# LCAV/LenslessPiCam

Measured on AMD Instinct MI355X. Metric: ADMM iterations/sec at 4056x3040x3, 100 iters, higher is better.
Workload: dtype f32; 1 GPU; C2: one 3040x4056x3 frame per GPU, ADMM-TV 100 iterations per step; n_iter=100, frames_per_gpu=1, parallelism=frames sharded over 1 GPU(s), one all-gather per step

## Files before the change

lenslesspicam_amd/csrc/lpc_abi.cpp:

```cpp
#include "lpc_engine.h"

static thread_local std::string g_last_error;
int fail(const std::string& msg) {
  g_last_error = msg;
  return 1;
}

static std::string parse_all_opts(const char* handle_opts, EngineOpts& o) {
  std::string err = parse_engine_opts(std::getenv("LPC_OPTIONS"), o);
  return err.empty() ? parse_engine_opts(handle_opts, o) : err;
}

extern "C" {

const char* lpc_last_error(void) { return g_last_error.c_str(); }
const char* lpc_backend(void) { return rt::backend_name(); }
const char* lpc_real_name(void) { return LPC_REAL_NAME; }

int lpc_create(const lpc_config* cfg, lpc_handle* out) {
  if (!cfg || !out) return fail("lpc_create: null argument");
  *out = nullptr;
  if (cfg->height < 1 || cfg->width < 1) return fail("lpc_create: bad spatial size");
  if (cfg->channels != 1 && cfg->channels != 3) return fail("PSF must either be rgb (3) or grayscale (1)");
  if (cfg->depth < 1 || cfg->batch < 1) return fail("lpc_create: depth and batch must be >= 1");
  if (cfg->algo < LPC_ALGO_CONV || cfg->algo > LPC_ALGO_FISTA) return fail("lpc_create: unknown algo");
  if (cfg->norm < 0 || cfg->norm > 2) return fail("lpc_create: unknown norm");
  int ndev = 0;
  if (rt::device_count(&ndev) != lpcSuccess || ndev < 1)
    return fail("no HIP device: the engine has no CPU path");
  Engine* e = new Engine();
  e->cfg = *cfg;
  e->cfg.options = nullptr;
  {
    std::string err = parse_all_opts(cfg->options, e->opt);
    if (!err.empty()) { delete e; return fail("lpc_create: " + err); }
  }
  e->gd.tk = cfg->fista_tk; e->gd.nest_mu = cfg->nesterov_mu; e->gd.nest_p = cfg->nesterov_p;
  int rc = setup_geometry(e);
  if (!rc) rc = alloc_common(e);
  if (!rc && cfg->algo == LPC_ALGO_ADMM) rc = admm_alloc(e);
  if (!rc && cfg->algo >= LPC_ALGO_GD) rc = gd_alloc(e);
  if (rc) {
    lpc_destroy(e);
    return rc;
  }
  *out = e;
  return 0;
}

int lpc_plan_module(const lpc_config* cfg, int build, char* key_buf, size_t n) {
  if (!cfg) return fail("lpc_plan_module: null config");
  if (cfg->height < 1 || cfg->width < 1 || cfg->depth < 1 || cfg->batch < 1) return fail("lpc_plan_module: bad size");
  EngineOpts opt;
  std::string err = parse_all_opts(cfg->options, opt);
  if (!err.empty()) return fail("lpc_plan_module: " + err);
  ShapePlan sp;
  LPC_OK(setup_shape(*cfg, opt, plan_cu_count(), &sp));
  const bool any = sp.want_static && sp.plan.spec.any();
  if (key_buf && n) std::snprintf(key_buf, n, "%s", any ? plan_spec_key(sp.plan.spec).c_str() : "");
  if (!any || !build) return 0;
  std::string path;
  if (build_plan_module(sp.plan.spec, opt, &path) != 0) return fail(path);
  return 0;
}

int lpc_destroy(lpc_handle e) {
  if (!e) return 0;
  (void)rt::stream_sync(e->stream);
  for (auto& a : e->allocs) (void)rt::dev_free(a.first);
  release_plan_module(e->mod);
  e->mod = nullptr;
#if !defined(LPC_SIMT_EMU)
  for (auto& v : e->timer.ev)
    for (auto& pr : v) { (void)hipEventDestroy(pr.first); (void)hipEventDestroy(pr.second); }
#endif
  delete e;
  return 0;
}

int lpc_padded_shape(lpc_handle e, int* Hp, int* Wp, int* sh, int* sw) {
  if (!e) return fail("null handle");
  if (Hp) *Hp = e->g.Hp;
  if (Wp) *Wp = e->g.Wp;
  if (sh) *sh = e->g.sh;
  if (sw) *sw = e->g.sw;
  return 0;
}

int lpc_workspace_bytes(lpc_handle e, size_t* bytes) {
  if (!e || !bytes) return fail("null argument");
  *bytes = e->total_bytes;
  return 0;
}

int lpc_set_psf(lpc_handle e, const real* dev_psf, void* stream) {
  if (!e || !dev_psf) return fail("lpc_set_psf: null argument");
  e->stream = (lpcStream_t)stream;
  LPC_OK(set_psf(e, dev_psf));
  if (e->cfg.algo == LPC_ALGO_ADMM) LPC_OK(admm_setup_constants(e));
  if (e->cfg.algo >= LPC_ALGO_GD) LPC_OK(gd_setup_constants(e));
  if (e->cfg.algo != LPC_ALGO_CONV) return lpc_reset(e, stream);
  return 0;
}

static int per_frame_refusal(const Engine* e, const char* who) {
  if (!e->psf_per_frame) return 0;
  return fail(std::string(who) + ": not available with per-frame PSFs (lpc_set_psf_batch): their gradients are not implemented");
}
static int per_frame_gd_check(const Engine* e, const char* who) {
  if (e->cfg.algo < LPC_ALGO_GD || (e->gd.gx0_pinned && e->fista.sched_n > 0)) return 0;
  return fail(std::string(who) + ": per-frame PSFs need a pinned start value (lpc_set_start_value) and a schedule "
              "(lpc_set_fista_schedule) on a gradient-descent handle: plain iterations take their step and start value from one PSF");
}

int lpc_set_psf_batch(lpc_handle e, const real* dev_psfs, void* stream) {
  if (!e || !dev_psfs) return fail("lpc_set_psf_batch: null argument");
  LPC_OK(per_frame_gd_check(e, "lpc_set_psf_batch"));
  if (e->fista_tape.rec_on || e->admm_tape.rec_on)
    return fail("lpc_set_psf_batch: the handle records a tape, and gradients with per-frame PSFs are not implemented");
  e->stream = (lpcStream_t)stream;
  const bool gram = e->cfg.algo == LPC_ALGO_ADMM && !e->psf_set;
  LPC_OK(set_psf_batch(e, dev_psfs));
  e->admm.midc_valid = false;
  e->fista_tape.invalidate();
  e->admm_tape.invalidate();
  if (gram) LPC_OK(admm_setup_constants(e));
  if (e->cfg.algo != LPC_ALGO_CONV) return lpc_reset(e, stream);
  return 0;
}

int lpc_convolve(lpc_handle e, const real* dev_x, real* dev_out, int n, int x_channels, int adjoint, void* stream) {
  if (!e || !dev_x || !dev_out) return fail("lpc_convolve: null argument");
  LPC_OK(check_channels(e, x_channels, "lpc_convolve"));
  if (!e->psf_set) return fail("lpc_convolve: PSF not set");
  if (n < 1 || n > e->cfg.batch) return fail("lpc_convolve: n exceeds the configured batch");
  if (e->cfg.algo != LPC_ALGO_CONV) return fail("lpc_convolve: handle was not created with LPC_ALGO_CONV");
  e->stream = (lpcStream_t)stream;
  return convolve_hwc(e, dev_x, dev_out, n, x_channels, adjoint != 0, false);
}

int lpc_convolve_spectrum(lpc_handle e, const real* dev_x, real* dev_out, int n, int x_channels, int adjoint,
                          void* stream) {
  if (!e || !dev_x || !dev_out) return fail("lpc_convolve_spectrum: null argument");
  LPC_OK(check_channels(e, x_channels, "lpc_convolve_spectrum"));
  if (!e->psf_set) return fail("lpc_convolve_spectrum: PSF not set");
  if (n < 1 || n > e->cfg.batch) return fail("lpc_convolve_spectrum: n exceeds the configured batch");
  if (e->cfg.algo != LPC_ALGO_CONV) return fail("lpc_convolve_spectrum: handle was not created with LPC_ALGO_CONV");
  e->stream = (lpcStream_t)stream;
  return convolve_hwc(e, dev_x, dev_out, n, x_channels, adjoint != 0, true);
}

int lpc_set_data(lpc_handle e, const real* dev_data, int data_channels, void* stream) {
  if (!e || !dev_data) return fail("lpc_set_data: null argument");
  if (e->cfg.algo == LPC_ALGO_CONV) return fail("lpc_set_data: operator-only handle");
  LPC_OK(check_channels(e, data_channels, "lpc_set_data"));
  e->stream = (lpcStream_t)stream;
  const PlaneGeom& g = e->g;
  LPC_OK(hwc_to_planar(e, dev_data, e->Y, e->cfg.batch, g.H, g.W, g.W, g.uplane, data_channels));
  e->data_set = true;
  e->data_channels = data_channels;
  e->fista_tape.invalidate();
  e->admm_tape.invalidate();
  return 0;
}

int lpc_set_initial_estimate(lpc_handle e, const real* dev_est, void* stream) {
  if (!e) return fail("null handle");
  if (e->cfg.algo == LPC_ALGO_CONV) return fail("lpc_set_initial_estimate: operator-only handle");
  e->stream = (lpcStream_t)stream;
  const PlaneGeom& g = e->g;
  if (!dev_est) { e->has_init = false; return 0; }
  const bool admm = e->cfg.algo == LPC_ALGO_ADMM;
  const size_t n = (size_t)(admm ? g.rplane : g.uplane) * e->P;
  if (!e->init_est) LPC_OK(dev_alloc(e, &e->init_est, n));
  const int nimg = e->cfg.batch * e->cfg.depth;
  if (admm) LPC_OK(hwc_to_planar(e, dev_est, e->init_est, nimg, g.Hp, g.Wp, g.rpitch, g.rplane));
  else LPC_OK(hwc_to_planar(e, dev_est, e->init_est, nimg, g.H, g.W, g.W, g.uplane));
  e->has_init = true;
  return 0;
}

int lpc_reset(lpc_handle e, void* stream) {
  if (!e) return fail("null handle");
  if (!e->psf_set) return fail("lpc_reset: PSF not set");
  e->stream = (lpcStream_t)stream;
  if (e->cfg.algo == LPC_ALGO_ADMM) return admm_reset(e);
  if (e->cfg.algo >= LPC_ALGO_GD) return gd_reset(e);
  return 0;
}

int lpc_set_momentum(lpc_handle e, double p, double mu, double tk) {
  if (!e) return fail("null handle");
  e->gd.nest_p = p; e->gd.nest_mu = mu;
  if (tk > 0) e->gd.tk = tk;
  return gd_apply_momentum_reset(e);
}

int lpc_set_start_value(lpc_handle e, const real* dev_start, void* stream) {
  if (!e) return fail("null handle");
  if (e->cfg.algo < LPC_ALGO_GD) return fail("lpc_set_start_value: gradient-descent family only");
  e->stream = (lpcStream_t)stream;
  e->gd.gx0_pinned = dev_start != nullptr;
  if (dev_start) LPC_RT(rt::copy_d2d_async(e->gd.gx0, dev_start, e->cfg.channels * sizeof(real), e->stream));
  return 0;
}

int lpc_set_admm_schedule(lpc_handle e, int n, const double* mu1, const double* mu2, const double* mu3,
                          const double* tau) {
  if (!e) return fail("null handle");
  if (e->cfg.algo != LPC_ALGO_ADMM) return fail("lpc_set_admm_schedule: not an ADMM handle");
  for (auto& v : e->admm.sched) v.clear();
  e->admm_tape.invalidate();
  if (n <= 0) return 0;
  if (!mu1 || !mu2 || !mu3 || !tau) return fail("lpc_set_admm_schedule: null array");
  for (int i = 0; i < n; ++i) {
    if (!(mu1[i] > 0) || !(mu2[i] > 0) || !(mu3[i] > 0)) return fail("lpc_set_admm_schedule: step sizes must be > 0");
    e->admm.sched[0].push_back(mu1[i]); e->admm.sched[1].push_back(mu2[i]);
    e->admm.sched[2].push_back(mu3[i]); e->admm.sched[3].push_back(tau[i]);
  }
  return 0;
}

int lpc_set_fista_schedule(lpc_handle e, int n, const real* alpha, const real* coef, void* stream) {
  if (!e) return fail("null handle");
  if (e->cfg.algo != LPC_ALGO_FISTA) return fail("lpc_set_fista_schedule: not a FISTA handle");
  e->stream = (lpcStream_t)stream;
  return gd_set_schedule(e, n, alpha, coef);
}

int lpc_fista_record(lpc_handle e, int on) {
  if (!e) return fail("null handle");
  if (e->cfg.algo != LPC_ALGO_FISTA) return fail("lpc_fista_record: not a FISTA handle");
  if (on) LPC_OK(per_frame_refusal(e, "lpc_fista_record"));
  return tape_record(e, e->fista_tape, on, gd_tape_alloc);
}

static int tape_refusal(const Engine* e, const Tape& t, long n, const std::string& who, bool counted) {
  if (!counted && (!t.rec_on || !t.buf || t.iters < 0))
    return fail("lpc_" + who + "_backward: nothing recorded (lpc_" + who + "_record(h, 1), then lpc_reset and lpc_iterate)");
  if (counted && !t.complete(n, e->iters_done))
    return fail("lpc_" + who + "_backward: " + std::to_string(e->iters_done) + " iterations since the reset, the schedule has " +
                std::to_string(n));
  return 0;
}

static int fista_backward(lpc_handle e, const real* dev_grad_out, real* dev_grad_data, real* dev_grad_alpha,
                          real* dev_grad_coef, real* dev_grad_init, real* dev_grad_psf, void* stream) {
  if (!e || !dev_grad_out || !dev_grad_alpha || !dev_grad_coef) return fail("lpc_fista_backward: null argument");
  if (e->cfg.algo != LPC_ALGO_FISTA) return fail("lpc_fista_backward: not a FISTA handle");
  LPC_OK(per_frame_refusal(e, "lpc_fista_backward"));
  if (e->fista.sched_n <= 0) return fail("lpc_fista_backward: the handle has no schedule (lpc_set_fista_schedule)");
  LPC_OK(tape_refusal(e, e->fista_tape, e->fista.sched_n, "fista", false));
  if (e->gd.split_pending) return fail("lpc_fista_backward: a split iteration is in flight (lpc_iterate_end missing)");
  LPC_OK(tape_refusal(e, e->fista_tape, e->fista.sched_n, "fista", true));
  if ((e->g.Hp | e->g.Wp) & 1)
    return fail("lpc_fista_backward: padded frame " + std::to_string(e->g.Hp) + " x " + std::to_string(e->g.Wp) +
                " has an odd length: convolve and deconvolve are not each other's adjoints there (not implemented)");
  if (e->cfg.depth > 1) return fail("lpc_fista_backward: depth > 1 is not implemented");
  for (real a : e->fista.alpha)
    if (a == (real)0.) return fail("lpc_fista_backward: a step alpha of the schedule is 0");
  if (dev_grad_data && !e->data_set) return fail("lpc_fista_backward: no data set");
  e->stream = (lpcStream_t)stream;
  return gd_backward(e, dev_grad_out, dev_grad_data, dev_grad_alpha, dev_grad_coef, dev_grad_init, dev_grad_psf);
}
int lpc_fista_backward(lpc_handle e, const real* dev_grad_out, real* dev_grad_data, real* dev_grad_alpha,
                       real* dev_grad_coef, real* dev_grad_init, void* stream) {
  return fista_backward(e, dev_grad_out, dev_grad_data, dev_grad_alpha, dev_grad_coef, dev_grad_init, nullptr, stream);
}
int lpc_fista_backward_psf(lpc_handle e, const real* dev_grad_out, real* dev_grad_data, real* dev_grad_alpha,
                           real* dev_grad_coef, real* dev_grad_init, real* dev_grad_psf, void* stream) {
  return fista_backward(e, dev_grad_out, dev_grad_data, dev_grad_alpha, dev_grad_coef, dev_grad_init, dev_grad_psf, stream);
}

int lpc_admm_record(lpc_handle e, int on) {
  if (!e) return fail("null handle");
  if (e->cfg.algo != LPC_ALGO_ADMM) return fail("lpc_admm_record: not an ADMM handle");
  if (on) LPC_OK(per_frame_refusal(e, "lpc_admm_record"));
  return tape_record(e, e->admm_tape, on, admm_tape_alloc);
}

static int admm_backward_checked(lpc_handle e, const real* dev_grad_out, real* dev_grad_data, real* dev_grad_mu1,
                                 real* dev_grad_mu2, real* dev_grad_mu3, real* dev_grad_tau, real* dev_grad_psf, void* stream) {
  if (!e || !dev_grad_out || !dev_grad_mu1 || !dev_grad_mu2 || !dev_grad_mu3 || !dev_grad_tau)
    return fail("lpc_admm_backward: null argument");
  if (e->cfg.algo != LPC_ALGO_ADMM) return fail("lpc_admm_backward: not an ADMM handle");
  LPC_OK(per_frame_refusal(e, "lpc_admm_backward"));
  const long n = (long)e->admm.sched[0].size();
  if (n <= 0) return fail("lpc_admm_backward: the handle has no schedule (lpc_set_admm_schedule)");
  if (e->cfg.depth > 1) return fail("lpc_admm_backward: depth > 1 is not implemented");
  if ((e->g.Hp | e->g.Wp) & 1)
    return fail("lpc_admm_backward: padded frame " + std::to_string(e->g.Hp) + " x " + std::to_string(e->g.Wp) +
                " has an odd length: the spectral step and the convolve / deconvolve pair are not self-adjoint there "
                "(not implemented)");
  if (e->admm.custom_gram || e->admm.pnp_mode)
    return fail("lpc_admm_backward: a caller's psi and plug-and-play iterations are not differentiated");
  if (e->has_init) return fail("lpc_admm_backward: an initial estimate is set (its gradient is not implemented)");
  LPC_OK(tape_refusal(e, e->admm_tape, n, "admm", false));
  LPC_OK(tape_refusal(e, e->admm_tape, n, "admm", true));
  if (dev_grad_data && !e->data_set) return fail("lpc_admm_backward: no data set");
  if (dev_grad_psf && e->cfg.norm != LPC_NORM_BACKWARD)
    return fail("lpc_admm_backward_psf: the gradient with respect to the PSF is implemented for norm \"backward\" only");
  e->stream = (lpcStream_t)stream;
  return admm_backward(e, dev_grad_out, dev_grad_data, dev_grad_mu1, dev_grad_mu2, dev_grad_mu3, dev_grad_tau, dev_grad_psf);
}
int lpc_admm_backward(lpc_handle e, const real* dev_grad_out, real* dev_grad_data, real* dev_grad_mu1, real* dev_grad_mu2,
                      real* dev_grad_mu3, real* dev_grad_tau, void* stream) {
  return admm_backward_checked(e, dev_grad_out, dev_grad_data, dev_grad_mu1, dev_grad_mu2, dev_grad_mu3, dev_grad_tau, nullptr,
                               stream);
}
int lpc_admm_backward_psf(lpc_handle e, const real* dev_grad_out, real* dev_grad_data, real* dev_grad_mu1, real* dev_grad_mu2,
                          real* dev_grad_mu3, real* dev_grad_tau, real* dev_grad_psf, void* stream) {
  return admm_backward_checked(e, dev_grad_out, dev_grad_data, dev_grad_mu1, dev_grad_mu2, dev_grad_mu3, dev_grad_tau,
                               dev_grad_psf, stream);
}

int lpc_iterate(lpc_handle e, int n_iter, void* stream) {
  if (!e) return fail("null handle");
  if (n_iter < 0) return fail("lpc_iterate: negative iteration count");
  if (!e->psf_set) return fail("lpc_iterate: PSF not set");
  if (!e->data_set) return fail("Must set data with `set_data()`");
  e->stream = (lpcStream_t)stream;
  if (e->gd.split_pending) return fail("lpc_iterate: a split iteration is in flight (lpc_iterate_end missing)");
  if (e->admm.pnp_mode) return fail("lpc_iterate: the handle runs plug-and-play iterations since the last reset");
  if (e->psf_per_frame) LPC_OK(per_frame_gd_check(e, "lpc_iterate"));
  if (e->cfg.algo == LPC_ALGO_ADMM) return admm_iterate(e, n_iter);
  if (e->cfg.algo >= LPC_ALGO_GD) return gd_iterate(e, n_iter);
  return fail("lpc_iterate: operator-only handle");
}

int lpc_iterate_begin(lpc_handle e, void* stream) {
  if (!e) return fail("null handle");
  if (e->cfg.algo < LPC_ALGO_GD) return fail("lpc_iterate_begin: gradient-descent family only");
  if (!e->psf_set) return fail("lpc_iterate_begin: PSF not set");
  if (!e->data_set) return fail("Must set data with `set_data()`");
  if (e->gd.split_pending) return fail("lpc_iterate_begin: the previous split iteration was not finished");
  if (e->psf_per_frame) LPC_OK(per_frame_gd_check(e, "lpc_iterate_begin"));
  if (e->fista_tape.rec_on)
    return fail("lpc_iterate_begin: not available while the handle records a tape (lpc_fista_record)");
  e->stream = (lpcStream_t)stream;
  return gd_iterate(e, 1, 1);
}

int lpc_iterate_end(lpc_handle e, const real* dev_projected, void* stream) {
  if (!e || !dev_projected) return fail("lpc_iterate_end: null argument");
  if (e->cfg.algo < LPC_ALGO_GD) return fail("lpc_iterate_end: gradient-descent family only");
  if (!e->gd.split_pending) return fail("lpc_iterate_end: no split iteration in flight");
  e->stream = (lpcStream_t)stream;
  return gd_finish_split(e, dev_projected);
}

static int pnp_check(lpc_handle e, const char* who) {
  if (!e) return fail("null handle");
  if (e->cfg.algo != LPC_ALGO_ADMM) return fail(std::string(who) + ": ADMM handles only");
  if (!e->psf_set) return fail(std::string(who) + ": PSF not set");
  if (!e->data_set) return fail("Must set data with `set_data()`");
  if (!e->admm.sched[0].empty()) return fail(std::string(who) + ": not available with an unrolled schedule");
  return 0;
}

int lpc_admm_pnp_begin(lpc_handle e, int use_dual, real* dev_denoiser_in, void* stream) {
  LPC_OK(pnp_check(e, "lpc_admm_pnp_begin"));
  if (!dev_denoiser_in) return fail("lpc_admm_pnp_begin: null argument");
  if (e->admm.pnp_pending) return fail("lpc_admm_pnp_begin: the previous split iteration was not finished");
  if (!e->admm.pnp_mode && e->iters_done != 0)
    return fail("lpc_admm_pnp_begin: fused iterations already ran since the last reset");
  e->stream = (lpcStream_t)stream;
  return admm_pnp_begin(e, use_dual, dev_denoiser_in);
}

int lpc_admm_pnp_end(lpc_handle e, int use_dual, const real* dev_U, void* stream) {
  LPC_OK(pnp_check(e, "lpc_admm_pnp_end"));
  if (!dev_U) return fail("lpc_admm_pnp_end: null argument");
  if (!e->admm.pnp_pending) return fail("lpc_admm_pnp_end: no split iteration in flight");
  e->stream = (lpcStream_t)stream;
  return admm_pnp_end(e, use_dual, dev_U);
}

int lpc_set_psi_gram(lpc_handle e, const real* dev_gabs, void* stream) {
  if (!e || !dev_gabs) return fail("lpc_set_psi_gram: null argument");
  if (e->cfg.algo != LPC_ALGO_ADMM) return fail("lpc_set_psi_gram: ADMM handles only");
  e->stream = (lpcStream_t)stream;
  return admm_set_psi_gram(e, dev_gabs);
}

int lpc_admm_psi_step(lpc_handle e, const real* dev_psit, void* stream) {
  LPC_OK(pnp_check(e, "lpc_admm_psi_step"));
  if (!dev_psit) return fail("lpc_admm_psi_step: null argument");
  if (e->admm.pnp_pending) return fail("lpc_admm_psi_step: a plug-and-play iteration is in flight");
  if (!e->admm.pnp_mode && e->iters_done != 0)
    return fail("lpc_admm_psi_step: fused iterations already ran since the last reset");
  e->stream = (lpcStream_t)stream;
  return admm_psi_step(e, dev_psit);
}

int lpc_form_image(lpc_handle e, real* dev_out, void* stream) {
  if (!e || !dev_out) return fail("lpc_form_image: null argument");
  e->stream = (lpcStream_t)stream;
  if (e->cfg.algo == LPC_ALGO_ADMM) return admm_form_image(e, dev_out);
  if (e->cfg.algo >= LPC_ALGO_GD) return gd_form_image(e, dev_out);
  return fail("lpc_form_image: operator-only handle");
}

int lpc_get_state(lpc_handle e, const char* name, real* dev_out, void* stream) {
  if (!e || !name || !dev_out) return fail("lpc_get_state: null argument");
  e->stream = (lpcStream_t)stream;
  if (e->cfg.algo >= LPC_ALGO_GD) return gd_get_state(e, name, dev_out);
  if (e->cfg.algo == LPC_ALGO_ADMM) return admm_get_state(e, name, dev_out);
  return fail("lpc_get_state: operator-only handle");
}

int lpc_profile_enable(lpc_handle e, int on) {
  if (!e) return fail("null handle");
#if !defined(LPC_SIMT_EMU)
  for (int k = 0; k < LPC_K_COUNT; ++k) e->timer.used[k] = 0;
#endif
  e->timer.on = on != 0;
  e->timer.mask = on > 1 ? (unsigned)on >> 1 : ~0u;
  return 0;
}

int lpc_profile_read(lpc_handle e, double* avg_ms, long* launches) {
  if (!e || !avg_ms || !launches) return fail("null argument");
  for (int k = 0; k < LPC_K_COUNT; ++k) { avg_ms[k] = 0.0; launches[k] = 0; }
#if !defined(LPC_SIMT_EMU)
  LPC_RT(hipStreamSynchronize(e->stream));
  for (int k = 0; k < LPC_K_COUNT; ++k) {
    double tot = 0.0;
    for (size_t i = 0; i < e->timer.used[k]; ++i) {
      float ms = 0.f;
      LPC_RT(hipEventElapsedTime(&ms, e->timer.ev[k][i].first, e->timer.ev[k][i].second));
      tot += ms;
    }
    launches[k] = (long)e->timer.used[k];
    avg_ms[k] = e->timer.used[k] ? tot / (double)e->timer.used[k] : 0.0;
  }
#endif
  return 0;
}

int lpc_kernel_bytes(lpc_handle e, int kid, double* bytes) {
  if (!e || !bytes) return fail("null argument");
  if (e->cfg.algo == LPC_ALGO_ADMM) return admm_kernel_bytes(e, kid, bytes);
  if (e->cfg.algo >= LPC_ALGO_GD) return gd_kernel_bytes(e, kid, bytes);
  return fail("lpc_kernel_bytes: operator-only handle");
}

int lpc_plan_info(lpc_handle e, char* buf, size_t n) {
  if (!e || !buf || n == 0) return fail("null argument");
  const PlaneGeom& g = e->g;
  const LaunchPlan& pl = e->plan;
  const PlanSpec& sp = pl.spec;
  std::string s = "padded " + std::to_string(g.Hp) + "x" + std::to_string(g.Wp);
  s += pl.rows_half ? "; rows: half-length " + std::to_string(g.Wp / 2) : "; rows: paired " + std::to_string(g.Wp);
  const bool rows_static = e->mod && sp.row_kind && (pl.rows_half || e->cfg.algo == LPC_ALGO_ADMM);
  if (rows_static) s += " [static " + rad_list(sp.row, ".") + ", " + std::to_string(sp.row.nt) + " threads]";
  if (pl.gd_v2) s += " (fused rows: second form, " + std::to_string(sp.row.n / sp.row.rad[0]) + " lanes)";
  if (pl.admm_rows_v2)
    s += std::string(" (ADMM rows: second form, ") + (pl.admm_rows_v2 == 3 ? "forward + inverse, " : pl.admm_rows_v2 == 2 ? "inverse, " : "forward, ") +
         std::to_string(sp.row.n / sp.row.rad[0]) + " lanes)";
  s += "; columns: " + (pl.N1 > 1 ? std::to_string(pl.N1) + " x " + std::to_string(pl.N2) + " split" : std::string("single pass ") + std::to_string(pl.N2));
  s += ", T = " + std::to_string(pl.T);
  if (e->mod && sp.passA.n) s += ", pass A [static " + rad_list(sp.passA, ".") + ", T = " + std::to_string(sp.passA.T) + "]";
  if (e->cfg.algo == LPC_ALGO_ADMM) {
    s += pl.admm_mid == ADMM_MID_REG24 ? ", middle in registers"
         : pl.admm_mid == ADMM_MID_MODULE ? ", LDS middle [static " + rad_list(sp.mid, ".") + (sp.mid_kind == LPC_MID_SEQ ? ", one spectrum at a time" : "") + (g.slay ? ", pair-line spectra]" : "]")
                                          : ", LDS middle";
    s += pl.k1 == ADMM_K1_ROWS ? "; TV / W half and X half inside the forward rows (three launches per iteration)"
         : pl.k1 == ADMM_K1_TV_W ? "; tiled TV / W kernel + X half inside the forward rows" : "; stand-alone image-domain kernel";
    if (pl.xi_window) s += pl.hv_skip ? " (xi inside the sensor window only, H V row transforms skipped outside it)"
                                      : " (xi inside the sensor window only)";
    if (pl.rho_rsp || pl.xi_half)
      s += std::string("; inside a call: ") + (pl.rho_rsp ? "rho read back from r_sp" : "") +
           (pl.rho_rsp && pl.xi_half ? ", " : "") + (pl.xi_half ? "xi half-applied" : "");
  }
  if (e->cfg.algo == LPC_ALGO_ADMM && e->admm.g_sep) s += "; gram as row + column terms";
  if (e->cfg.algo == LPC_ALGO_FISTA)
    s += e->mod && e->mod->gd_bwd_head ? "; reverse rows: plan module" : pl.rows_half ? "; reverse rows: half-length, run-time plan"
                                                                                     : "; reverse rows: paired, run-time plan";
  s += e->mod ? "; plan module " + plan_spec_key(sp) : "; run-time plans (" + e->mod_note + ")";
  std::snprintf(buf, n, "%s", s.c_str());
  return 0;
}

int lpc_model_bytes(lpc_handle e, double* bytes) {
  if (!e || !bytes) return fail("null argument");
  if (e->cfg.algo == LPC_ALGO_ADMM) *bytes = admm_model_bytes(e);
  else if (e->cfg.algo >= LPC_ALGO_GD) *bytes = gd_model_bytes(e);
  else return fail("lpc_model_bytes: operator-only handle");
  return 0;
}

}
```

lenslesspicam_amd/csrc/lpc_admm.cpp:

```cpp
#include "lpc_engine.h"
#include "lpc_admm_kernels.h"
#include "lpc_layout_kernels.h"
#include "lpc_reduce_kernels.h"

static void admm_params(const Engine* e, long it, double out[4]) {
  const lpc_config& c = e->cfg;
  const double dflt[4] = {c.mu1, c.mu2, c.mu3, c.tau};
  for (int k = 0; k < 4; ++k) {
    const std::vector<double>& v = e->admm.sched[k];
    out[k] = v.empty() ? dflt[k] : v[(size_t)std::min<long>(it, (long)v.size() - 1)];
  }
}

static AdmmScalars admm_scalars(const Engine* e, const double cur[4]) {
  AdmmScalars p;
  p.mu1 = (real)cur[0]; p.mu2 = (real)cur[1]; p.mu3 = (real)cur[2];
  p.thr = (real)(cur[3] / cur[1]);
  p.m_in = (real)1.0 / ((real)1.0 + p.mu1);
  p.m_out = (real)1.0 / ((real)0.0 + p.mu1);
  p.first = e->first ? 1 : 0;
  const double* prev = e->first ? cur : e->admm.last_par;
  p.mu1p = (real)prev[0]; p.mu2p = (real)prev[1]; p.mu3p = (real)prev[2];
  p.thrp = (real)(prev[3] / prev[1]);
  p.m_in_p = (real)1.0 / ((real)1.0 + p.mu1p);
  p.m_out_p = (real)1.0 / ((real)0.0 + p.mu1p);
  p.r_mu2 = (real)(1.0 / (double)p.mu2); p.r_mu3 = (real)(1.0 / (double)p.mu3);
  p.r_mu2p = (real)(1.0 / (double)p.mu2p); p.r_mu3p = (real)(1.0 / (double)p.mu3p);
  p.clamp_cur = e->admm.vw_cur ? 1 : 0;
  p.clamp_old = e->admm.vw_old ? 1 : 0;
  p.xiw = e->plan.xi_window ? 1 : 0;
  p.xi_store = 1;
  p.skipa = p.skiphv = 0;
  p.rev = e->plan.rev_k1 ? 1 : 0;
  p.half_in = p.half_out = 0;
  p.rho_rsp = p.xi_in = p.xi_out = 0;
  return p;
}

int admm_alloc_psf(Engine* e, int nplanes) {
  const PlaneGeom& g = e->g;
  dev_free(e, e->admm.Hs_t); dev_free(e, e->admm.midc); dev_free(e, e->admm.midrd);
  e->admm.Hs_t = nullptr; e->admm.midc = nullptr; e->admm.midrd = nullptr;
  e->admm.midc_valid = false;
  if (!g.slay) return 0;
  LPC_OK(dev_alloc(e, &e->admm.Hs_t, (size_t)g.cplane * nplanes));
  if (e->mod && e->mod->mid_pc) {
    real2* c = nullptr;
    LPC_OK(dev_alloc(e, &c, (size_t)g.cplane * nplanes * (e->mod->mid_pc == 1 ? 2 : 1)));
    e->admm.midc = c;
    LPC_OK(dev_alloc(e, &e->admm.midrd, (size_t)g.cplane * nplanes));
  }
  return 0;
}

static const int kGsepBlocks = 512;
int admm_alloc(Engine* e) {
  const PlaneGeom& g = e->g;
  const size_t rp = (size_t)g.rplane * e->P;
  real* zeroed = nullptr;
  LPC_OK(dev_alloc(e, &zeroed, 8 * rp));
  real** zb[] = {&e->admm.V[0], &e->admm.V[1], &e->admm.HVb[0], &e->admm.HVb[1], &e->admm.xi, &e->admm.eta0[0], &e->admm.eta1[0], &e->admm.rho};
  for (int k = 0; k < 8; ++k) *zb[k] = zeroed + (size_t)k * rp;
  real** bufs[] = {&e->admm.eta0[1], &e->admm.eta1[1], &e->admm.Rsp, &e->admm.Aarr};
  for (real** b : bufs) LPC_OK(dev_alloc(e, b, rp));
  LPC_OK(dev_alloc(e, &e->admm.Gabs, (size_t)g.cplane));
  if (g.slay) LPC_OK(dev_alloc(e, &e->admm.Gabs_t, (size_t)g.cplane));
  LPC_OK(admm_alloc_psf(e, e->Ppsf));
  LPC_OK(dev_alloc(e, &e->admm.Ga, (size_t)g.Hp));
  LPC_OK(dev_alloc(e, &e->admm.Gb, (size_t)g.cpitch));
  LPC_OK(dev_alloc(e, &e->admm.Gpart, (size_t)2 * kGsepBlocks));
  return 0;
}

static int admm_split_gram(Engine* e) {
  const PlaneGeom& g = e->g;
  e->admm.g_sep = 0;
  e->admm.midc_valid = false;
  if (g.slay)
    LPC_OK(launch_k(e, -1, k_to_pair_lines<256, real>, grid1d((long)g.Hp * g.cpitch, 256), 256, 0, (const real*)e->admm.Gabs,
                    e->admm.Gabs_t, g.Hp, g.cpitch, g.cplane));
  if (!e->plan.g_terms) return 0;
  const int n = (int)std::max<long>(g.Hp, g.cpitch);
  LPC_OK(launch_k(e, -1, k_gsep_extract, grid1d((long)n, 256), 256, 0, (const real*)e->admm.Gabs, g.Hp, g.Wc,
                  (long)g.cpitch, e->admm.Ga, e->admm.Gb));
  LPC_OK(launch_k(e, -1, k_gsep_check<256>, dim3(kGsepBlocks), 256, 2 * 256 * sizeof(real), (const real*)e->admm.Gabs, g.Hp,
                  g.Wc, (long)g.cpitch, (const real*)e->admm.Ga, (const real*)e->admm.Gb, e->admm.Gpart));
  std::vector<real> part((size_t)2 * kGsepBlocks);
  LPC_RT(rt::copy_d2h_async(part.data(), e->admm.Gpart, part.size() * sizeof(real), e->stream));
  LPC_RT(rt::stream_sync(e->stream));
  double err = 0., top = 0.;
  for (int b = 0; b < kGsepBlocks; ++b) { err = std::max(err, (double)part[2 * b]); top = std::max(top, -(double)part[2 * b + 1]); }
  const double eps = sizeof(real) == 4 ? 1e-6 : 1e-13;
  e->admm.g_sep = (top > 0. && err <= eps * top) ? 1 : 0;
  return 0;
}

int admm_setup_constants(Engine* e) {
  const PlaneGeom& g = e->g;
  real* stencil = e->admm.Rsp;
  LPC_RT(rt::memset_async(stencil, 0, (size_t)g.rplane * sizeof(real), e->stream));
  std::vector<real> host((size_t)g.rplane, (real)0.);
  host[0] = (real)4.;
  host[(size_t)(1 % g.Wp)] = -(real)1.;
  host[(size_t)(g.Wp - 1)] = -(real)1.;
  host[(size_t)(1 % g.Hp) * g.rpitch] = -(real)1.;
  host[(size_t)(g.Hp - 1) * g.rpitch] = -(real)1.;
  LPC_OK(upload(e, stencil, host.data(), host.size() * sizeof(real)));
  real2* Gs = e->S;
  LPC_OK(fft2_forward_setup(e, src_padded(e, stencil), Gs, 1));
  LPC_OK(launch_k(e, -1, k_abs_complex<256>, grid1d((long)g.cplane, 256), 256, 0, (const real2*)Gs, e->admm.Gabs,
                  (long)g.cplane));
  e->admm.custom_gram = false;
  return admm_split_gram(e);
}

int admm_reset(Engine* e) {
  const PlaneGeom& g = e->g;
  const size_t rb = (size_t)g.rplane * e->P * sizeof(real);
  if (e->has_init) LPC_RT(rt::memset_async(e->admm.V[1], 0, 7 * rb, e->stream));
  else LPC_RT(rt::memset_async(e->admm.V[0], 0, 8 * rb, e->stream));
  e->admm.vcur = 0;
  e->admm.ecur = 0;
  e->admm.hcur = 0;
  e->admm.vw_cur = e->admm.vw_old = false;
  if (e->has_init) {
    LPC_RT(rt::copy_d2d_async(e->admm.V[0], e->init_est, rb, e->stream));
    LPC_OK(convolve_planar(e, e->admm.V[0], e->admm.HVb[0], e->P, true, false));
  }
  e->first = true;
  e->admm.pnp_mode = e->admm.pnp_pending = false;
  e->iters_done = 0;
  return admm_tape_reset(e);
}

static int admm_spectral_step(Engine* e, const AdmmScalars& sc, real* Vout, real* HVout, bool xhalf = false,
                              const K1Rows* k1 = nullptr) {
  if (xhalf) LPC_OK(e->mod->admm_rows_fwd_x(e, &sc, k1));
  else LPC_OK(admm_rows_fwd(e));
  LPC_OK(admm_cols(e, sc));
  return admm_rows_inv(e, Vout, HVout, sc.skiphv != 0);
}
int admm_spectral_plain(Engine* e, const double par[4], real* Vout, real* HVout) {
  return admm_spectral_step(e, admm_scalars(e, par), Vout, HVout);
}


typedef void (*K1Kernel)(PlaneGeom, AdmmScalars, const real*, const real*, const real*, const real*, real*, const real*,
                         const real*, real*, real*, real*, const real*, real*, real*, unsigned);
struct K1Launch { K1Kernel fn; int th, tw; size_t smem; };
static K1Launch k1_launch(AdmmK1 form, bool half_in) {
  constexpr int NT = 256, TW4 = 256;
  auto smem4 = [](int th) { return (size_t)2 * (th + 2) * (TW4 + 8) * sizeof(real); };
  switch (form) {
    case ADMM_K1_TV_W:
      return half_in ? K1Launch{k_admm_spatial_v4<4, NT, false, true>, 4, TW4, smem4(4) / 2}
                     : K1Launch{k_admm_spatial_v4<4, NT, false>, 4, TW4, smem4(4)};
    case ADMM_K1_TILED: return {k_admm_spatial_v4<8, NT>, 8, TW4, smem4(8)};
    default: return {k_admm_spatial<16, 64, NT>, 16, 64, (size_t)(2 * 18 * 66 + 17 * 64 + 16 * 65) * sizeof(real)};
  }
}

int admm_iterate(Engine* e, int n_iter) {
  const PlaneGeom& g = e->g;
  const LaunchPlan& pl = e->plan;
  bool sb_rows_valid = false;
  for (int it = 0; it < n_iter; ++it) {
    real* Vc = e->admm.V[e->admm.vcur];
    real* Vo = e->admm.V[e->admm.vcur ^ 1];
    double par[4];
    admm_params(e, e->iters_done, par);
    AdmmScalars sc = admm_scalars(e, par);
    sc.xi_store = (it + 1 == n_iter || !sc.xiw) ? 1 : 0;
    sc.skipa = (pl.hv_skip && sb_rows_valid && !sc.xi_store) ? 1 : 0;
    sc.skiphv = (pl.hv_skip && it + 3 < n_iter) ? 1 : 0;
    sc.half_in = (pl.k1_half && it > 0) ? 1 : 0;
    sc.half_out = (pl.k1_half && it + 1 < n_iter) ? 1 : 0;
    sc.rho_rsp = (pl.rho_rsp && sc.half_in) ? 1 : 0;
    sc.xi_in = (pl.xi_half && it > 0) ? 1 : 0;
    sc.xi_out = (pl.xi_half && it + 1 < n_iter) ? 1 : 0;
    AdmmState& a = e->admm;
    const K1Rows k1 = {Vc, Vo, a.eta0[a.ecur], a.eta1[a.ecur], a.eta0[a.ecur ^ 1], a.eta1[a.ecur ^ 1], a.rho, pl.k1_xcd_order};
    if (pl.k1 != ADMM_K1_ROWS) {
      const K1Launch k = k1_launch(pl.k1, sc.half_in != 0);
      const unsigned tiles_x = (g.Wp + k.tw - 1) / k.tw, tiles_y = (g.Hp + k.th - 1) / k.th;
      LPC_OK(launch_k(e, LPC_K_SPATIAL, k.fn, dim3(tiles_x * tiles_y, e->P, 1), 256, k.smem, g, sc, (const real*)Vc,
                      (const real*)Vo, (const real*)a.HVb[a.hcur], (const real*)a.HVb[a.hcur ^ 1], a.xi,
                      (const real*)a.eta0[a.ecur], (const real*)a.eta1[a.ecur], a.eta0[a.ecur ^ 1], a.eta1[a.ecur ^ 1],
                      a.rho, (const real*)e->Y, a.Rsp, a.Aarr, tiles_x));
    }
    e->admm.vw_old = e->admm.vw_cur;
    e->admm.vw_cur = false;
    e->admm.ecur ^= 1;
    e->first = false;
    LPC_OK(admm_spectral_step(e, sc, Vo, e->admm.HVb[e->admm.hcur ^ 1], pl.xhalf_rows, pl.k1 == ADMM_K1_ROWS ? &k1 : nullptr));
    e->admm.vcur ^= 1;
    e->admm.hcur ^= 1;
    sb_rows_valid = true;
    for (int k = 0; k < 4; ++k) e->admm.last_par[k] = par[k];
    LPC_OK(admm_tape_push(e, Vo));
    ++e->iters_done;
  }
  return 0;
}

int admm_pnp_begin(Engine* e, int use_dual, real* dev_denoiser_in) {
  e->admm.pnp_mode = true;
  const PlaneGeom& g = e->g;
  const int nimg = e->cfg.batch * e->cfg.depth;
  real* src = e->admm.V[e->admm.vcur];
  if (use_dual) {
    const long n = (long)g.rplane * e->P;
    LPC_OK(launch_k(e, -1, k_pnp_input<256>, grid1d(n, 256), 256, 0, e->admm.Rsp, (const real*)e->admm.eta1[0],
                    (const real*)e->admm.eta0[0], (real)e->cfg.mu2, n));
    src = e->admm.Rsp;
  }
  LPC_OK(planar_to_hwc(e, src, dev_denoiser_in, nimg, g.Hp, g.Wp, g.rpitch, g.rplane, 0, 0, 0));
  e->admm.pnp_pending = true;
  return 0;
}

int admm_pnp_end(Engine* e, int use_dual, const real* dev_U) {
  const PlaneGeom& g = e->g;
  const int nimg = e->cfg.batch * e->cfg.depth;
  real *eta = e->admm.eta0[0], *U = e->admm.eta1[0], *X = e->admm.eta0[1], *W = e->admm.eta1[1];
  LPC_OK(hwc_to_planar(e, dev_U, U, nimg, g.Hp, g.Wp, g.rpitch, g.rplane));
  double par[4];
  admm_params(e, e->iters_done, par);
  const AdmmScalars sc = admm_scalars(e, par);
  const dim3 grid = grid1d((long)g.Hp * g.Wp, 256, e->P);
  real* Vc = e->admm.V[e->admm.vcur];
  real* Vn = e->admm.V[e->admm.vcur ^ 1];
  real* HVn = e->admm.HVb[e->admm.hcur ^ 1];
  LPC_OK(launch_k(e, LPC_K_SPATIAL, k_pnp_pre<256>, grid, 256, 0, g, sc, use_dual ? 1 : 0, (const real*)Vc,
                  (const real*)e->admm.HVb[e->admm.hcur], (const real*)e->admm.xi, (const real*)e->admm.rho, (const real*)U,
                  (const real*)eta, (const real*)e->Y, X, W, e->admm.Rsp, e->admm.Aarr));
  LPC_OK(admm_spectral_step(e, sc, Vn, HVn));
  LPC_OK(launch_k(e, LPC_K_SPATIAL, k_pnp_post<256>, grid, 256, 0, g, sc, use_dual ? 1 : 0, (const real*)Vn,
                  (const real*)HVn, (const real*)X, (const real*)W, (const real*)U, e->admm.xi, eta, e->admm.rho));
  e->admm.vcur ^= 1;
  e->admm.hcur ^= 1;
  e->admm.pnp_pending = false;
  e->first = false;
  ++e->iters_done;
  return 0;
}

int admm_set_psi_gram(Engine* e, const real* dev_gabs) {
  const PlaneGeom& g = e->g;
  LPC_RT(rt::memset_async(e->admm.Gabs, 0, (size_t)g.cplane * sizeof(real), e->stream));
  LPC_OK(launch_k(e, -1, k_permute_spectrum_rows<256>, grid1d((long)g.Hp * g.Wc, 256), 256, 0, dev_gabs, e->admm.Gabs, g.Hp,
                  g.Wc, g.cpitch, e->plan.N1, e->plan.N2));
  e->admm.custom_gram = true;
  return admm_split_gram(e);
}

int admm_psi_step(Engine* e, const real* dev_psit) {
  e->admm.pnp_mode = true;
  const PlaneGeom& g = e->g;
  const int nimg = e->cfg.batch * e->cfg.depth;
  real *T = e->admm.eta1[0], *X = e->admm.eta0[1], *W = e->admm.eta1[1];
  LPC_OK(hwc_to_planar(e, dev_psit, T, nimg, g.Hp, g.Wp, g.rpitch, g.rplane));
  double par[4];
  admm_params(e, e->iters_done, par);
  const AdmmScalars sc = admm_scalars(e, par);
  const dim3 grid = grid1d((long)g.Hp * g.Wp, 256, e->P);
  real* Vc = e->admm.V[e->admm.vcur];
  real* Vn = e->admm.V[e->admm.vcur ^ 1];
  real* HVn = e->admm.HVb[e->admm.hcur ^ 1];
  LPC_OK(launch_k(e, LPC_K_SPATIAL, k_pnp_pre<256>, grid, 256, 0, g, sc, 2, (const real*)Vc,
                  (const real*)e->admm.HVb[e->admm.hcur], (const real*)e->admm.xi, (const real*)e->admm.rho, (const real*)T,
                  (const real*)e->admm.eta0[0], (const real*)e->Y, X, W, e->admm.Rsp, e->admm.Aarr));
  LPC_OK(admm_spectral_step(e, sc, Vn, HVn));
  LPC_OK(launch_k(e, LPC_K_SPATIAL, k_pnp_post<256>, grid, 256, 0, g, sc, 0, (const real*)Vn, (const real*)HVn,
                  (const real*)X, (const real*)W, (const real*)T, e->admm.xi, e->admm.eta0[0], e->admm.rho));
  e->admm.vcur ^= 1;
  e->admm.hcur ^= 1;
  e->first = false;
  ++e->iters_done;
  return 0;
}

int admm_form_image(Engine* e, real* dev_out) {
  const PlaneGeom& g = e->g;
  const int nimg = e->cfg.batch * e->cfg.depth;
  if (e->has_init && e->iters_done == 0 && e->init_est) {
    LPC_OK(launch_k(e, -1, k_clamp_window_inplace<256>, grid1d((long)g.H * g.W, 256, e->P), 256, 0, g, e->init_est));
  }
  if (e->admm.pnp_mode) {
    LPC_OK(planar_to_hwc(e, e->admm.V[e->admm.vcur], dev_out, nimg, g.H, g.W, g.rpitch, g.rplane, g.sh, g.sw, 1));
    return launch_k(e, -1, k_clamp_window_inplace<256>, grid1d((long)g.H * g.W, 256, e->P), 256, 0, g,
                    e->admm.V[e->admm.vcur]);
  }
  LPC_OK(planar_to_hwc(e, e->admm.V[e->admm.vcur], dev_out, nimg, g.H, g.W, g.rpitch, g.rplane, g.sh, g.sw, 1));
  e->admm.vw_cur = true;
  return 0;
}

int admm_get_state(Engine* e, const std::string& nm, real* dev_out) {
  const PlaneGeom& g = e->g;
  const int nimg = e->cfg.batch * e->cfg.depth;
  auto out_padded = [&](real* src) {
    return planar_to_hwc(e, src, dev_out, nimg, g.Hp, g.Wp, g.rpitch, g.rplane, 0, 0, 0);
  };
  if (e->admm.pnp_mode) {
    if (nm == "image_est") return out_padded(e->admm.V[e->admm.vcur]);
    if (nm == "forward_out") return out_padded(e->admm.HVb[e->admm.hcur]);
    if (nm == "xi") return out_padded(e->admm.xi);
    if (nm == "rho") return out_padded(e->admm.rho);
    if (nm == "eta") return out_padded(e->admm.eta0[0]);
    if (nm == "U") return out_padded(e->admm.eta1[0]);
    if (nm == "X") return out_padded(e->admm.eta0[1]);
    if (nm == "W") return out_padded(e->admm.eta1[1]);
    return fail("lpc_get_state: unknown name '" + nm + "'");
  }
  if (nm == "image_est")
    return planar_to_hwc(e, e->admm.V[e->admm.vcur], dev_out, nimg, g.Hp, g.Wp, g.rpitch, g.rplane, 0, 0,
                         e->admm.vw_cur ? 2 : 0);
  if (nm == "forward_out") return out_padded(e->admm.HVb[e->admm.hcur]);
  int w0 = -1, w1 = -1;
  if (nm == "xi") w0 = 0;
  else if (nm == "rho") w0 = 3;
  else if (nm == "W") w0 = 6;
  else if (nm == "X") w0 = 7;
  else if (nm == "eta") { w0 = 1; w1 = 2; }
  else if (nm == "U") { w0 = 4; w1 = 5; }
  else return fail("lpc_get_state: unknown name '" + nm + "'");
  double par[4];
  admm_params(e, e->iters_done, par);
  AdmmScalars sc = admm_scalars(e, par);
  sc.clamp_old = e->admm.vw_old ? 1 : 0;
  const AdmmState& a = e->admm;
  LPC_OK(launch_k(e, -1, k_admm_flush<256>, grid1d((long)g.Hp * g.Wp, 256, e->P), 256, 0, g, sc,
                  (const real*)a.V[a.vcur], (const real*)a.V[a.vcur ^ 1], (const real*)a.HVb[a.hcur],
                  (const real*)a.HVb[a.hcur ^ 1], (const real*)e->Y, (const real*)a.xi, (const real*)a.eta0[a.ecur],
                  (const real*)a.eta1[a.ecur], (const real*)a.rho, a.Rsp, w1 >= 0 ? a.Aarr : (real*)nullptr, w0,
                  w1 >= 0 ? w1 : 0));
  if (w1 < 0) return out_padded(e->admm.Rsp);
  return planar2_to_hwc2(e, e->admm.Rsp, e->admm.Aarr, dev_out, nimg);
}

int admm_kernel_bytes(Engine* e, int kid, double* bytes) {
  const PlaneGeom& g = e->g;
  const LaunchPlan& pl = e->plan;
  const double eb = (double)sizeof(real);
  const double R = eb * g.Hp * g.Wp * e->P;
  const double S = 2 * eb * g.Hp * g.Wc * e->P;
  const double R0 = eb * g.H * g.W * e->Pdata;
  const double Sc = 2 * eb * g.Hp * g.Wc * e->Ppsf;
  const bool split = pl.N1 > 1, k1_rows = pl.k1 == ADMM_K1_ROWS;
  const double fr = (double)g.H / (double)g.Hp;
  const double nxw = pl.xi_half ? 2.0 : 3.0;
  double b = 0.0;
  switch (kid) {
    case LPC_K_SPATIAL: b = k1_rows ? 0.0 : pl.xhalf_rows ? (pl.rho_rsp ? 7.0 : pl.k1_half ? 8.0 : 9.0) * R : 15.0 * R + R0; break;
    case LPC_K_ROW_FWD: b = (pl.hv_skip ? (1.0 + fr) * R + nxw * eb * g.H * g.W * e->P + R0 + (1.0 + fr) * S
                                : pl.xi_window ? 2.0 * R + nxw * eb * g.H * g.W * e->P + R0 + 2.0 * S
                                : pl.xhalf_rows ? (2.0 + nxw) * R + R0 + 2.0 * S : 2.0 * R + 2.0 * S)
                               + (k1_rows ? (pl.k1_half ? 6.0 : 7.0) * R : 0.0); break;
    case LPC_K_COL_A_FWD: b = split ? 4.0 * S : 0.0; break;
    case LPC_K_COL_MID: b = 4.0 * S + Sc + (e->admm.g_sep ? 0. : eb * g.Hp * g.Wc); break;
    case LPC_K_COL_A_INV: b = split ? 4.0 * S : 0.0; break;
    case LPC_K_ROW_INV: b = pl.hv_skip ? (1.0 + fr) * (S + R) : 2.0 * S + 2.0 * R; break;
    default: return fail("bad kernel id");
  }
  *bytes = b;
  return 0;
}

double admm_model_bytes(const Engine* e) {
  const PlaneGeom& g = e->g;
  const double eb = (double)sizeof(real);
  const double R = eb * g.Hp * g.Wp * e->P, S = 2 * eb * g.Hp * g.Wc * e->P;
  const double Sc = e->psf_per_frame ? 2 * eb * g.Hp * g.Wc * e->Ppsf : 0.0;
  return 19.0 * R + eb * g.H * g.W * e->Pdata + 13.5 * S + Sc;
}
```

lenslesspicam_amd/csrc/lpc_admm_v2_kernels.h:

```cpp
#pragma once
#include "lpc_gd_v2_kernels.h"
#include "lpc_admm_kernels.h"

#ifndef LPC_DOUBLE

template <int NT, int SK, class PL>
__global__ __launch_bounds__(NT, 4) void k_rinv_half_v2(PlaneGeom g, PL plan, const real2* LPC_RESTRICT twW,
                                                        const real2* LPC_RESTRICT SA, const real2* LPC_RESTRICT SB,
                                                        real* LPC_RESTRICT A, real* LPC_RESTRICT B, int skip_b_outside) {
  using P = typename PL::plan;
  constexpr int R = GdV2<P>::R, NB = GdV2<P>::NB, L = GdV2<P>::L;
  static_assert(GdV2<P>::ok && NT == NB, "k_rinv_half_v2: one butterfly per lane and stage");
  LPC_DYN_SMEM(smem);
  real2* s = (real2*)smem;
  const int j = LPC_TID(NT);
  const unsigned bx = LPC_BX(g);
  int row = bx >> 1, arr = (bx ^ (bx >> 3)) & 1;
  const long pl = LPC_BY(g);
  if (skip_b_outside) {
    if ((int)bx < 2 * g.H) row += g.sh;
    else {
      const int q = (int)bx - 2 * g.H;
      row = q < g.sh ? q : q + g.H;
      arr = 0;
    }
  }
  real2 wb[4];
  v2_tw_load<P, 1>(plan.tws, j, wb);
  v2_load_tangle_first<P, SK, false>(s, (arr ? SB : SA) + pl * g.cplane + (long)row * g.cpitch, twW, j);
  v2_barrier();
  v2_mid_chain<P, SK, true>(s, plan.tws, j, wb, std::make_integer_sequence<int, L - 2>{});
  real2 v[R];
  v2_final_stage<P, SK, true, false>(s, plan.tws, j, wb, v);
  real2* o2 = (real2*)((arr ? B : A) + pl * g.rplane + (long)row * g.rpitch);
#pragma unroll
  for (int m = 0; m < R; ++m) o2[j + NB * m] = v[m];
}

template <int NT, int SK, class PL>
__global__ __launch_bounds__(NT, 4) void k_rfwd_half_x_v2(PlaneGeom g, AdmmScalars pin, PL plan, const real2* LPC_RESTRICT twW,
                                                          const real* LPC_RESTRICT Rsp, const real* LPC_RESTRICT HV,
                                                          real* LPC_RESTRICT xi, const real* LPC_RESTRICT Y,
                                                          real2* LPC_RESTRICT SA, real2* LPC_RESTRICT SB, FastDiv fdc,
                                                          FastDiv fc) {
  using P = typename PL::plan;
  constexpr int R = GdV2<P>::R, NB = GdV2<P>::NB, L = GdV2<P>::L, H = R / 2;
  static_assert(GdV2<P>::ok && NT == NB, "k_rfwd_half_x_v2: one butterfly per lane and stage");
  LPC_DYN_SMEM(smem);
  real2* s = (real2*)smem;
  const int j = LPC_TID(NT);
  const unsigned bx = LPC_BX(g);
  const int gr = (int)(bx >> 1), arr = (int)(bx & 1);
  const unsigned pl = LPC_BY(g);
  const long o_row = (long)pl * g.rplane + (long)gr * g.rpitch;
  const bool row_in = (gr >= g.sh) && (gr < g.sh + g.H);
  if (arr == 1 && pin.skipa && !row_in) return;
  real2 r[R], v[R];
  if (arr == 0) {
    const real2* a2 = (const real2*)(Rsp + o_row);
#pragma unroll
    for (int m = 0; m < R; ++m) r[m] = a2[j + NB * m];
  } else {
    AdmmScalars p = pin;
    p.first = 0; p.xi_in = 1; p.xi_out = 1;
    const int x0 = p.xiw ? g.sw & ~3 : 0, x1 = p.xiw ? (g.sw + g.W + 3) & ~3 : g.Wp;
    const lpc_rsrc xr = lpc_make_rsrc(xi + o_row + x0, (p.xiw && !row_in) ? 0u : (unsigned)(x1 - x0) * (unsigned)sizeof(real));
    const lpc_rsrc yr = lpc_make_rsrc(Y + (long)v2_data_plane(pl, fdc, fc, g.C) * g.uplane + (long)(gr - g.sh) * g.W,
                                      row_in ? (unsigned)g.W * (unsigned)sizeof(real) : 0u);
    const real2* hv2 = (const real2*)(HV + o_row);
    const real ho = lpc_opaque_f((real)0.);
    auto xoff = [&](int m) { return lpc_opaque((2 * (j + NB * m) - x0) * (int)sizeof(real)); };
    auto yoff = [&](int m) { return lpc_opaque((2 * (j + NB * m) - g.sw) * (int)sizeof(real)); };
    auto loads = [&](int m0, real2* hh, real2* xx, real2* yy) {
#pragma unroll
      for (int m = 0; m < H; ++m) hh[m] = hv2[j + NB * (m0 + m)];
#pragma unroll
      for (int m = 0; m < H; ++m) xx[m] = lpc_buf_load2(xr, xoff(m0 + m));
#pragma unroll
      for (int m = 0; m < H; ++m) yy[m] = lpc_buf_load2(yr, yoff(m0 + m));
    };
    auto apply = [&](int m0, const real2* hh, const real2* xx, const real2* yy) {
#pragma unroll
      for (int m = 0; m < H; ++m) {
        const bool in = row_in && (unsigned)(2 * (j + NB * (m0 + m)) - g.sw) < (unsigned)g.W;
        real2 xn;
        xhalf_apply2(p, hh[m], xx[m], yy[m], in, ho, xn, r[m0 + m]);
        lpc_buf_store2(xr, xoff(m0 + m), xn);
      }
    };
    real2 h0[H], x0v[H], y0[H], h1[H], x1v[H], y1[H];
    loads(0, h0, x0v, y0);
    loads(H, h1, x1v, y1);
    LPC_SCHED_FENCE();
    apply(0, h0, x0v, y0);
    apply(H, h1, x1v, y1);
  }
  real2 wb[4];
  v2_tw_load<P, 1>(plan.tws, j, wb);
  v2_first_fwd<P, SK>(s, j, r);
  v2_mid_chain<P, SK, false>(s, plan.tws, j, wb, std::make_integer_sequence<int, L - 2>{});
  v2_final_stage<P, SK, false, false>(s, plan.tws, j, wb, v);
  v2_barrier();
  v2_untangle_store<P, SK, false>(s, twW, j, v, (arr ? SB : SA) + (long)pl * g.cplane + (long)gr * g.cpitch);
}

#endif
```

lenslesspicam_amd/csrc/lpc_engine.h:

```cpp
#pragma once
#include "lpc_args.h"
#include "lpc.h"
#include "lpc_plan.h"

#ifndef LPC_SRC_FP
#define LPC_SRC_FP "dev"
#endif

#include <algorithm>
#include <climits>
#include <string>
#include <type_traits>
#include <unordered_set>
#include <vector>

int fail(const std::string& msg);
#define LPC_RT(expr)                                                                      \
  do {                                                                                    \
    lpcError_t e_ = (expr);                                                               \
    if (e_ != lpcSuccess)                                                                 \
      return fail(std::string(#expr) + " failed: " + rt::err_string(e_));                 \
  } while (0)
#define LPC_OK(expr)          \
  do {                        \
    int r_ = (expr);          \
    if (r_) return r_;        \
  } while (0)


static constexpr int kMaxTilePoints = (int)(131072 / sizeof(real2));
template <class F>
static inline int dispatch_cfg(int nelem, F&& f) {
  using std::integral_constant;
  if (nelem <= 1024) return f(integral_constant<int, 256>{}, integral_constant<int, 4>{});
  if (nelem <= 2048) return f(integral_constant<int, 256>{}, integral_constant<int, 8>{});
  if (nelem <= 4096) return f(integral_constant<int, 256>{}, integral_constant<int, 16>{});
  if (nelem <= 8192) return f(integral_constant<int, 512>{}, integral_constant<int, 16>{});
  if (nelem <= kMaxTilePoints) return f(integral_constant<int, 1024>{}, integral_constant<int, 16>{});
  return fail("FFT tile of " + std::to_string(nelem) + " points exceeds the LDS budget (" +
              std::to_string(kMaxTilePoints) + ")");
}

template <class F>
static inline int dispatch_row(int Wp, int skew, bool r2, F&& f) {
  using std::integral_constant;
  return dispatch_cfg(Wp, [&](auto NT, auto EM) {
    if (skew && r2) return f(NT, EM, integral_constant<bool, true>{}, integral_constant<bool, true>{});
    if (skew) return f(NT, EM, integral_constant<bool, true>{}, integral_constant<bool, false>{});
    if (r2) return f(NT, EM, integral_constant<bool, false>{}, integral_constant<bool, true>{});
    return f(NT, EM, integral_constant<bool, false>{}, integral_constant<bool, false>{});
  });
}

struct KernelTimer {
#if !defined(LPC_SIMT_EMU)
  std::vector<std::pair<hipEvent_t, hipEvent_t>> ev[LPC_K_COUNT];
  size_t used[LPC_K_COUNT] = {0};
#endif
  bool on = false;
  unsigned mask = ~0u;
};

enum AdmmK1 { ADMM_K1_ROWS, ADMM_K1_TV_W, ADMM_K1_TILED, ADMM_K1_SCALAR };
enum AdmmMid { ADMM_MID_REG24, ADMM_MID_MODULE, ADMM_MID_RT_512X18, ADMM_MID_RT_LDS };

struct LaunchPlan {
  PlanSpec spec;
  int N1 = 1, N2 = 1;
  int T = 16;
  bool rows_half = false;
  bool xhalf_rows = false;
  bool xi_window = false;
  bool hv_skip = false;
  AdmmK1 k1 = ADMM_K1_SCALAR;
  bool k1_half = false;
  bool rho_rsp = false;
  bool xi_half = false;
  int admm_rows_v2 = 0;
  int k1_xcd_order = 0;
  AdmmMid admm_mid = ADMM_MID_RT_LDS;
  int conv_mid_reg = 0;
  bool gd_fuse_fwd = false;
  bool gd_v2 = false;
  bool rev_k1 = false, rev_passa_fwd = false, rev_passa_inv = false, rev_mid = false;
  bool gd_rev_resid = false, gd_rev_update = false, gd_rev_mid = false;
  int mid_swz = 0;
  bool g_terms = false;
};

struct LaunchCtx {
  KernelTimer timer;
  lpcStream_t stream = nullptr;
};

struct AdmmState {
  real2* Hs_t = nullptr;
  real* Gabs_t = nullptr;
  void* midc = nullptr;
  real* midrd = nullptr;
  double midc_par[3] = {0, 0, 0};
  bool midc_valid = false;
  real* Gabs = nullptr;
  real* Ga = nullptr;
  real* Gb = nullptr;
  real* Gpart = nullptr;
  int g_sep = 0;
  std::vector<double> sched[4];
  double last_par[4] = {0, 0, 0, 0};
  real *V[2] = {nullptr, nullptr}, *HVb[2] = {nullptr, nullptr}, *xi = nullptr, *rho = nullptr,
        *Rsp = nullptr, *Aarr = nullptr;
  real *eta0[2] = {nullptr, nullptr}, *eta1[2] = {nullptr, nullptr};
  int vcur = 0, ecur = 0, hcur = 0;
  bool vw_cur = false, vw_old = false;
  bool pnp_mode = false, pnp_pending = false;
  bool custom_gram = false;
};

struct GdState {
  real *gx = nullptr, *gaux = nullptr;
  real* galpha = nullptr;
  real* gx0 = nullptr;
  bool gx0_pinned = false;
  real2* S2 = nullptr;
  double tk = 1.0, nest_mu = 0.9, nest_p = 0.0;
  bool fwd_done = false;
  bool split_pending = false;
};

struct FistaSchedule {
  std::vector<real> coef;
  real* galpha_sched = nullptr;
  size_t sched_cap = 0;
  int sched_n = 0;
  std::vector<real> alpha;
};

struct Tape {
  bool rec_on = false;
  real* buf = nullptr;
  size_t slot = 0;
  double* part = nullptr;
  int n = 0;
  long iters = -1;
  real* psf_ws = nullptr;
  real* at(long k) const { return buf + (size_t)k * slot; }
  void begin() { iters = 0; }
  void invalidate() { iters = -1; }
  bool wants(long iters_done) const { return iters >= 0 && iters == iters_done && iters_done < n; }
  void advance() { ++iters; }
  bool complete(long sched_n, long iters_done) const { return iters_done == sched_n && iters == sched_n && n == sched_n; }
};

struct lpc_engine : LaunchCtx {
  lpc_config cfg{};
  PlaneGeom g{};
  Fft1dPlan planW{}, planA{}, planB{};
  Fft1dPlan planWi{};
  Fft1dPlan planWh{};
  EngineOpts opt;
  LaunchPlan plan;
  const struct LpcModule* mod = nullptr;
  std::string mod_note;
  bool rows_r2 = false;
  ColPass passA{}, passB{};
  int P = 0, Ppsf = 0, Pdata = 0;
  int psf_cap = 0;
  bool psf_per_frame = false;
  std::vector<std::pair<void*, size_t>> allocs;
  size_t total_bytes = 0;

  real2* Hs = nullptr;
  real2* phr = nullptr;
  real2* phc = nullptr;
  real2* twH = nullptr;
  real2* tws_row = nullptr;
  real2* S = nullptr;
  real* Y = nullptr;
  int data_channels = 0;
  real* init_est = nullptr;
  real* psf_planar = nullptr;
  real *conv_in = nullptr, *conv_out = nullptr;
  bool has_init = false, psf_set = false, data_set = false, first = true;
  long iters_done = 0;
  AdmmState admm;
  GdState gd;
  FistaSchedule fista;
  Tape fista_tape, admm_tape;
};
typedef lpc_engine Engine;

template <class Tp>
static inline int dev_alloc(Engine* e, Tp** out, size_t count) {
  void* p = nullptr;
  size_t bytes = count * sizeof(Tp);
  LPC_RT(rt::dev_malloc(&p, bytes));
  e->allocs.push_back({p, bytes});
  e->total_bytes += bytes;
  *out = (Tp*)p;
  return 0;
}
static inline void dev_free(Engine* e, void* p) {
  if (!p) return;
  (void)rt::stream_sync(e->stream);
  for (auto it = e->allocs.begin(); it != e->allocs.end(); ++it)
    if (it->first == p) {
      e->total_bytes -= it->second;
      e->allocs.erase(it);
      break;
    }
  (void)rt::dev_free(p);
}

static inline void tape_free(Engine* e, Tape& t) {
  dev_free(e, t.psf_ws);
  dev_free(e, t.buf);
  dev_free(e, t.part);
  t.psf_ws = nullptr; t.buf = nullptr; t.part = nullptr; t.n = 0;
  t.invalidate();
}
static inline int tape_alloc(Engine* e, Tape& t, int n, size_t nslots, size_t slot, size_t nparts) {
  if (t.buf && t.n == n) return 0;
  tape_free(e, t);
  LPC_OK(dev_alloc(e, &t.buf, nslots * slot));
  if (dev_alloc(e, &t.part, nparts)) {
    tape_free(e, t);
    return 1;
  }
  t.n = n; t.slot = slot;
  return 0;
}
static inline int tape_record(Engine* e, Tape& t, int on, int (*alloc)(Engine*)) {
  t.rec_on = on > 0;
  t.invalidate();
  if (on < 0) return 0;
  if (!t.rec_on) { tape_free(e, t); return 0; }
  return alloc(e);
}

int big_smem_once(const void* fn, size_t smem);

template <class K, class... A>
static inline int launch_k(LaunchCtx* e, int kid, K kernel, dim3 grid, int nt, size_t smem, A... args) {
  if (smem > 48 * 1024) LPC_OK(big_smem_once((const void*)kernel, smem));
#if !defined(LPC_SIMT_EMU)
  const bool timed = e->timer.on && kid >= 0 && ((e->timer.mask >> kid) & 1u);
  size_t slot = 0;
  if (timed) {
    auto& v = e->timer.ev[kid];
    slot = e->timer.used[kid]++;
    if (slot >= v.size()) {
      hipEvent_t a, b;
      LPC_RT(hipEventCreate(&a));
      LPC_RT(hipEventCreate(&b));
      v.push_back({a, b});
    }
    LPC_RT(hipEventRecord(v[slot].first, e->stream));
  }
  hipLaunchKernelGGL(kernel, grid, dim3(nt), smem, e->stream, args...);
  if (timed) LPC_RT(hipEventRecord(e->timer.ev[kid][slot].second, e->stream));
#else
  (void)kid;
  lpc_emu::launch(grid, dim3(nt), smem, [=]() { kernel(args...); });
#endif
  LPC_RT(rt::last_error());
  return 0;
}

static inline dim3 grid1d(long n, int nt, long planes = 1) {
  long b = (n + nt - 1) / nt;
  if (b > 4096) b = 4096;
  if (b < 1) b = 1;
  return dim3((unsigned)b, (unsigned)planes, 1);
}

static inline RealSrc src_unpadded(const Engine* e, const real* base) {
  const PlaneGeom& g = e->g;
  RealSrc s;
  s.base = base; s.plane_stride = g.uplane; s.pitch = g.W; s.nrows = g.H; s.ncols = g.W; s.col0 = g.sw;
  s.out_row0 = g.sh;
  return s;
}
static inline RealSrc src_padded(const Engine* e, const real* base) {
  const PlaneGeom& g = e->g;
  RealSrc s;
  s.base = base; s.plane_stride = g.rplane; s.pitch = g.rpitch; s.nrows = g.Hp; s.ncols = g.Wp; s.col0 = 0;
  s.out_row0 = 0;
  return s;
}
static inline RealDst dst_padded(const Engine* e, real* base) {
  const PlaneGeom& g = e->g;
  RealDst d;
  d.base = base; d.plane_stride = g.rplane; d.pitch = g.rpitch; d.nrows = g.Hp; d.row0 = 0; d.col0 = 0;
  d.ncols = g.Wp;
  return d;
}
static inline RealDst dst_cropped(const Engine* e, real* base) {
  const PlaneGeom& g = e->g;
  RealDst d;
  d.base = base; d.plane_stride = g.uplane; d.pitch = g.W; d.nrows = g.H; d.row0 = g.sh; d.col0 = g.sw;
  d.ncols = g.W;
  return d;
}

struct GdScalars;
struct GdBwd;
struct LpcModule {
  int (*rows_fwd_single)(Engine*, const RealSrc*, real2* S, int nplanes, int kid);
  int (*rows_inv_single)(Engine*, const real2* S, const RealDst*, int nplanes, int kid);
  int (*admm_rows_fwd)(Engine*);
  int (*admm_rows_fwd_x)(Engine*, const AdmmScalars*, const K1Rows* k1);
  int (*admm_rows_inv)(Engine*, real* Vout, real* HVout, int skip_hv_outside);
  int (*gd_rows_mid)(Engine*, const real2* Sin, real2* Sout);
  int (*gd_rows_update)(Engine*, const GdScalars*, const real* alpha);
  int (*gd_rows_update_fwd)(Engine*, const GdScalars*, const real* alpha);
  int (*gd_bwd_head)(Engine*, const GdBwd*);
  int (*gd_bwd_mid)(Engine*, const GdBwd*);
  int (*gd_bwd_update)(Engine*, const GdBwd*);
  int (*gd_bwd_acc)(Engine*, const GdBwd*, const real2* Sin);
  int (*cols_passA)(Engine*, const ColPass*, real2* S, int nplanes, int inverse, int kid);
  int (*admm_mid)(Engine*, const ColPass*, const AdmmScalars*, real sb_outside_scale);
  int k1_rows;
  int mid_pc;
  int slay;
  int gd_v2;
  int admm_rows_v2;
};
const LpcModule* get_plan_module(const PlanSpec& spec, const EngineOpts& opt, bool allow_compile, std::string* why);
void release_plan_module(const LpcModule* mod);
int build_plan_module(const PlanSpec& spec, const EngineOpts& opt, std::string* path_or_error);

struct ShapePlan {
  PlaneGeom g{};
  int P = 0, Ppsf = 0, Pdata = 0;
  LaunchPlan plan;
  bool want_static = false;
};
int plan_cu_count();
bool plan_radices(int n, std::vector<int>& rad);
int setup_shape(const lpc_config& c, const EngineOpts& o, int cu, ShapePlan* out);
void choose_plan(const lpc_config& c, const EngineOpts& o, const PlaneGeom& g, int P, bool allow_static, int cu, LaunchPlan* pl);
void finish_plan(const lpc_config& c, const EngineOpts& o, const PlaneGeom& g, int P, const LpcModule* mod, bool lane_twiddles,
                 int cu, LaunchPlan* pl);
int upload(Engine* e, void* dst, const void* src, size_t bytes);
int setup_geometry(Engine* e);
int alloc_common(Engine* e);
int set_psf(Engine* e, const real* dev_psf);
int set_psf_batch(Engine* e, const real* dev_psfs);
int fft2_forward_setup(Engine* e, const RealSrc& src, real2* S, int nplanes);
int cols_fwd_full(Engine* e, real2* S, int nplanes, int zr0, int zr1);
int convolve_planar(Engine* e, const real* xin, real* xout, int nplanes, bool padded_io, bool adjoint);
int convolve_hwc(Engine* e, const real* dev_x, real* dev_out, int n, int x_channels, bool adjoint, bool spectrum);
int hwc_to_planar(Engine* e, const real* src, real* dst, int nimg, int rows, int cols, int pitch, long dplane,
                  int src_channels = 0);
int planar_to_hwc(Engine* e, real* src, real* dst, int nimg, int rows, int cols, int pitch, long splane, int row0, int col0,
                  int clamp);
int planar2_to_hwc2(Engine* e, const real* a0, const real* a1, real* dst, int nimg);
int check_channels(const Engine* e, int ch, const char* who);
int fill_planar(Engine* e, real* p, long n, real v);
int plane_minmax(Engine* e, const real2* Hs, const real* plane, int nblk, int nplanes, real* partial);
int admm_alloc(Engine* e);
int admm_alloc_psf(Engine* e, int nplanes);
int admm_setup_constants(Engine* e);
int admm_reset(Engine* e);
int admm_iterate(Engine* e, int n_iter);
int admm_pnp_begin(Engine* e, int use_dual, real* dev_denoiser_in);
int admm_pnp_end(Engine* e, int use_dual, const real* dev_U);
int admm_set_psi_gram(Engine* e, const real* dev_gabs);
int admm_psi_step(Engine* e, const real* dev_psit);
int admm_form_image(Engine* e, real* dev_out);
int admm_get_state(Engine* e, const std::string& nm, real* dev_out);
int admm_kernel_bytes(Engine* e, int kid, double* bytes);
double admm_model_bytes(const Engine* e);
int admm_spectral_plain(Engine* e, const double par[4], real* Vout, real* HVout);
int admm_tape_alloc(Engine* e);
int admm_tape_reset(Engine* e);
int admm_tape_push(Engine* e, const real* Vnew);
int admm_backward(Engine* e, const real* grad_out, real* grad_data, real* grad_mu1, real* grad_mu2, real* grad_mu3,
                  real* grad_tau, real* grad_psf = nullptr);
int gd_alloc(Engine* e);
int gd_setup_constants(Engine* e);
int gd_apply_momentum_reset(Engine* e);
int gd_set_schedule(Engine* e, int n, const real* alpha, const real* coef);
int gd_reset(Engine* e);
int gd_iterate(Engine* e, int n_iter, int split = 0);
int gd_finish_split(Engine* e, const real* dev_projected);
int gd_form_image(Engine* e, real* dev_out);
int gd_get_state(Engine* e, const std::string& nm, real* dev_out);
int gd_kernel_bytes(Engine* e, int kid, double* bytes);
double gd_model_bytes(const Engine* e);
int rows_fwd_single(Engine* e, const RealSrc& src, real2* S, int nplanes, int kid);
int rows_inv_single(Engine* e, const real2* S, const RealDst& dst, int nplanes, int kid);
int admm_rows_fwd(Engine* e);
int admm_rows_inv(Engine* e, real* Vout, real* HVout, bool skip_hv_outside = false);
int cols_passA(Engine* e, real2* S, int nplanes, bool inverse, int zr0, int zr1, int kid, bool crop_rows_only = false,
               real sb_outside_scale = (real)0.);
int cols_passB_fwd(Engine* e, real2* S, int nplanes, int zr0, int zr1);
int conv_middle(Engine* e, real2* S, int nplanes, bool adjoint, int zr0, int zr1, bool crop_rows_only = false,
                const real2* mult = nullptr, int mult_planes = 0);
int admm_cols(Engine* e, const AdmmScalars& sc);
int gd_rows_mid(Engine* e, const real2* Sin, real2* Sout);
int gd_rows_update(Engine* e, const GdScalars& sc, const real* alpha);
int gd_tape_alloc(Engine* e);
int gd_tape_reset(Engine* e);
int gd_tape_push(Engine* e);
int gd_backward(Engine* e, const real* grad_out, real* grad_data, real* grad_alpha, real* grad_coef, real* grad_init,
                real* grad_psf = nullptr);
int gd_bwd_rows(Engine* e, int mode, const GdBwd& a, const real2* Sin = nullptr);
int gd_bwd_psf_sum(Engine* e, const real* acc, real* grad_psf);
int gd_bwd_gdata(Engine* e, const real* gb, real* grad_data);
```

lenslesspicam_amd/csrc/lpc_launch.h:

```cpp
#pragma once
#include "lpc_engine.h"
#include "lpc_row_kernels.h"
#include "lpc_col_kernels.h"

static inline real2* spec_b(const Engine* e) { return e->S + (size_t)e->P * e->g.cplane; }
static inline real inv_points(const PlaneGeom& g) { return (real)1.0 / ((real)g.Hp * (real)g.Wp); }
static inline PlaneGeom geom_rev(const Engine* e, bool rev) {
  PlaneGeom g = e->g;
  g.rev = rev ? 1 : 0;
  return g;
}

template <int NT, int EM, int SK, class PA>
static inline int launch_rows_fwd_half(Engine* e, const PA& pa, const RealSrc& src, real2* S, int nplanes, int kid) {
  return launch_k(e, kid, k_rfwd_rows_half<NT, EM, SK, PA>, dim3(src.nrows, nplanes), NT,
                  LPC_ROW_SMEM_BYTES(e->g.Wp / 2, SK), e->g, pa, e->planW.tw, src, S);
}
template <int NT, int EM, int SK, class PA>
static inline int launch_rows_inv_half(Engine* e, const PA& pa, const real2* S, const RealDst& dst, int nplanes, int kid) {
  return launch_k(e, kid, k_rinv_rows_half<NT, EM, SK, PA>, dim3(dst.nrows, nplanes), NT,
                  LPC_ROW_SMEM_BYTES(e->g.Wp / 2, SK), e->g, pa, e->planW.tw, S, dst);
}
template <int NT, int EM, int SK, class PA>
static inline int launch_admm_rows_fwd_half(Engine* e, const PA& pa) {
  return launch_k(e, LPC_K_ROW_FWD, k_rfwd_half<NT, EM, SK, PA>, dim3(2 * e->g.Hp, e->P), NT,
                  LPC_ROW_SMEM_BYTES(e->g.Wp / 2, SK), e->g, pa, e->planW.tw, (const real*)e->admm.Rsp, (const real*)e->admm.Aarr,
                  e->S, spec_b(e));
}
template <int NT, int EM, int SK, class PA>
static inline int launch_admm_rows_inv_half(Engine* e, const PA& pa, real* Vout, real* HVout, bool skip_hv) {
  const PlaneGeom& g = e->g;
  return launch_k(e, LPC_K_ROW_INV, k_rinv_half<NT, EM, SK, PA>, dim3(skip_hv ? g.Hp + g.H : 2 * g.Hp, e->P), NT,
                  LPC_ROW_SMEM_BYTES(g.Wp / 2, SK), g, pa, e->planW.tw, (const real2*)e->S, (const real2*)spec_b(e),
                  Vout, HVout, skip_hv ? 1 : 0);
}

template <int NT, int EM, int SK, bool R2, int SL, class PA>
static inline int launch_admm_rows_fwd_paired(Engine* e, const PA& pa) {
  return launch_k(e, LPC_K_ROW_FWD, k_rfwd_arrays<NT, EM, SK, R2, PA, SL>, dim3(paired_rows_grid(e->g, false), e->P), NT,
                  LPC_ROW_SMEM_BYTES(e->g.Wp, SK), e->g, pa, (const real*)e->admm.Rsp, (const real*)e->admm.Aarr, e->S, spec_b(e));
}
template <int NT, int EM, int SK, bool R2, int SL, class PA>
static inline int launch_admm_rows_inv_paired(Engine* e, const PA& pa, real* Vout, real* HVout, bool skip_hv) {
  return launch_k(e, LPC_K_ROW_INV, k_rinv_arrays<NT, EM, SK, R2, PA, SL>, dim3(paired_rows_grid(e->g, skip_hv), e->P), NT,
                  LPC_ROW_SMEM_BYTES(e->g.Wp, SK), e->g, pa, (const real2*)e->S, (const real2*)spec_b(e), Vout, HVout,
                  skip_hv ? 1 : 0);
}

template <int NT, int EM, int SBT, bool TWLDS, class PA>
static inline int launch_cols(Engine* e, const PA& pa, const ColPass& cp, real2* S, int nplanes, bool inverse, int kid) {
  const dim3 grid(cp.G * cp.ntile_c, nplanes);
  const size_t smem = (size_t)cp.N * (cp.T + (TWLDS ? 2 : 0)) * sizeof(real2);
  if (inverse) return launch_k(e, kid, k_cols<NT, EM, true, PA, SBT, TWLDS>, grid, NT, smem, e->g, pa, cp, S);
  return launch_k(e, kid, k_cols<NT, EM, false, PA, SBT, TWLDS>, grid, NT, smem, e->g, pa, cp, S);
}
template <int NT, int EM, int SBT2, bool TWLDS, int SL, class PA>
static inline int launch_admm_mid(Engine* e, const PA& pa, const ColPass& cp, const AdmmScalars& sc, real sb_outside_scale) {
  return launch_k(e, LPC_K_COL_MID, k_cols_mid_admm<NT, EM, PA, SBT2, TWLDS, SL>, dim3(cp.G * cp.ntile_c, e->P), NT,
                  (size_t)cp.N * (2 * cp.T + (TWLDS ? 1 : 0)) * sizeof(real2), e->g, pa, cp, e->S, spec_b(e),
                  (const real2*)(SL ? e->admm.Hs_t : e->Hs), (const real*)(SL ? e->admm.Gabs_t : e->admm.Gabs), (const real2*)e->phr,
                  (const real2*)e->phc, make_fastdiv((unsigned)(2 * cp.T)), sc.mu1, sc.mu2, sc.mu3, inv_points(e->g),
                  sb_outside_scale);
}
```

lenslesspicam_amd/csrc/lpc_module.cpp:

```cpp
#include "lpc_gd_launch.h"
#include "lpc_gd_bwd_launch.h"
#include "lpc_admm_row_kernels.h"
#include "lpc_gd_v2_kernels.h"
#include "lpc_admm_v2_kernels.h"

#ifndef LPC_MOD_MID_PRE
#define LPC_MOD_MID_PRE 0
#endif
#ifndef LPC_MOD_SLAY
#define LPC_MOD_SLAY 0
#endif
#ifndef LPC_MOD_MID_PC
#define LPC_MOD_MID_PC 0
#endif
#ifndef LPC_MOD_FAMILY
#error "lpc_module.cpp is compiled with the flags of plan_spec_defines() (lpc_plan.h)"
#endif

#if LPC_MOD_ROW_KIND != 0
typedef SPlan<LPC_MOD_ROW_RAD> RowP;
#ifndef LPC_MOD_TW_LANE
#define LPC_MOD_TW_LANE 1
#endif
typedef SPlanArg<RowP, LPC_MOD_TW_LANE != 0> RowPA;
static constexpr int RNT = LPC_MOD_ROW_NT, REM = LPC_MOD_ROW_EM;
static constexpr int RSK = LPC_MOD_ROW_SK;
static_assert(RSK != LPC_LAY_SKEW8 || RowP::skew_ok(), "this row plan does not keep the LDS skew affine");
static const size_t kRowSmem = LPC_ROW_SMEM_BYTES(RowP::n, RSK);
#endif

#if LPC_MOD_ROW_KIND == LPC_ROWS_HALF
static RowPA row_arg(const Engine* e) { return splan_arg<RowP, LPC_MOD_TW_LANE != 0>(e->planWh, e->tws_row); }

static int m_rows_fwd_single(Engine* e, const RealSrc* src, real2* S, int nplanes, int kid) {
  return launch_rows_fwd_half<RNT, REM, RSK>(e, row_arg(e), *src, S, nplanes, kid);
}
static int m_rows_inv_single(Engine* e, const real2* S, const RealDst* dst, int nplanes, int kid) {
  return launch_rows_inv_half<RNT, REM, RSK>(e, row_arg(e), S, *dst, nplanes, kid);
}
#if LPC_MOD_FAMILY == LPC_FAM_ADMM
#ifndef LPC_MOD_V2_SK
#define LPC_MOD_V2_SK LPC_LAY_NONE
#endif
static constexpr int V2SK = LPC_MOD_V2_SK;
static const size_t kV2Smem = LPC_ROW_SMEM_BYTES(RowP::n, V2SK);
static int m_admm_rows_fwd(Engine* e) { return launch_admm_rows_fwd_half<RNT, REM, RSK>(e, row_arg(e)); }
static int m_admm_rows_inv(Engine* e, real* Vout, real* HVout, int skip_hv_outside) {
#ifndef LPC_DOUBLE
  if constexpr (GdV2<RowP>::ok) {
    if (e->plan.admm_rows_v2 & 2) {
      const PlaneGeom& g = e->g;
      constexpr int NB = GdV2<RowP>::NB;
      return launch_k(e, LPC_K_ROW_INV, k_rinv_half_v2<NB, V2SK, RowPA>, dim3(skip_hv_outside ? g.Hp + g.H : 2 * g.Hp, e->P), NB,
                      kV2Smem, g, row_arg(e), (const real2*)e->planW.tw, (const real2*)e->S, (const real2*)spec_b(e), Vout,
                      HVout, skip_hv_outside ? 1 : 0);
    }
  }
#endif
  return launch_admm_rows_inv_half<RNT, REM, RSK>(e, row_arg(e), Vout, HVout, skip_hv_outside != 0);
}
#if LPC_MOD_ROW_X
static int m_admm_rows_fwd_x(Engine* e, const AdmmScalars* sc, const K1Rows* k1) {
  if (k1) return fail("internal: half-length rows do not hold the TV / W half");
#ifndef LPC_DOUBLE
  if constexpr (GdV2<RowP>::ok) {
    if ((e->plan.admm_rows_v2 & 1) && !sc->first && sc->xi_in && sc->xi_out && !(sc->xiw && sc->xi_store)) {
      constexpr int NB = GdV2<RowP>::NB;
      return launch_k(e, LPC_K_ROW_FWD, k_rfwd_half_x_v2<NB, V2SK, RowPA>, dim3(2 * e->g.Hp, e->P), NB, kV2Smem, e->g, *sc,
                      row_arg(e), (const real2*)e->planW.tw, (const real*)e->admm.Rsp, (const real*)e->admm.HVb[e->admm.hcur],
                      e->admm.xi, (const real*)e->Y, e->S, spec_b(e), make_fastdiv((unsigned)e->g.DC),
                      make_fastdiv((unsigned)e->g.C));
    }
  }
#endif
  return launch_k(e, LPC_K_ROW_FWD, k_rfwd_half_x<RNT, REM, RSK, RowPA>, dim3(2 * e->g.Hp, e->P), RNT, kRowSmem,
                  e->g, *sc,
                  row_arg(e), (const real2*)e->planW.tw, (const real*)e->admm.Rsp, (const real*)e->admm.HVb[e->admm.hcur],
                  (const real*)e->admm.HVb[e->admm.hcur ^ 1], e->admm.xi, (const real*)e->Y, e->S, spec_b(e));
}
#endif
#else
#ifndef LPC_MOD_V2_SK
#define LPC_MOD_V2_SK LPC_LAY_NONE
#endif
static constexpr int V2SK = LPC_MOD_V2_SK;
static const size_t kV2Smem = LPC_ROW_SMEM_BYTES(RowP::n, V2SK);
static int m_gd_rows_mid(Engine* e, const real2* Sin, real2* Sout) {
  const PlaneGeom& g = e->g;
#ifndef LPC_DOUBLE
  if constexpr (GdV2<RowP>::ok) {
    if (e->plan.gd_v2)
      return launch_k(e, LPC_K_ROW_INV, k_gd_resid_v2<GdV2<RowP>::NB, V2SK, RowPA>, dim3(g.H, e->P), GdV2<RowP>::NB, kV2Smem,
                      geom_rev(e, e->plan.gd_rev_resid), row_arg(e), e->planW.tw, Sin, Sout,
                      (const real*)e->Y, make_fastdiv((unsigned)g.DC), make_fastdiv((unsigned)g.C));
  }
#endif
  return launch_gd_rows_mid_half<RNT, REM, RSK>(e, row_arg(e), Sin, Sout);
}
static int m_gd_rows_update(Engine* e, const GdScalars* sc, const real* alpha) {
  return launch_gd_rows_update_half<RNT, REM, RSK>(e, row_arg(e), *sc, alpha);
}
static int m_gd_rows_update_fwd(Engine* e, const GdScalars* sc, const real* alpha) {
  const PlaneGeom& g = e->g;
#ifndef LPC_DOUBLE
  if constexpr (GdV2<RowP>::ok) {
    if (e->plan.gd_v2) {
      auto go = [&](auto kernel) {
        return launch_k(e, LPC_K_SPATIAL, kernel, dim3(g.H, e->P), GdV2<RowP>::NB, kV2Smem, geom_rev(e, e->plan.gd_rev_update),
                        row_arg(e), e->planW.tw, (const real2*)e->gd.S2, e->S, e->gd.gx, e->gd.gaux, alpha, *sc,
                        make_fastdiv((unsigned)g.C));
      };
      constexpr int NB = GdV2<RowP>::NB;
      if (sc->kind == 2) return sc->first ? go(k_gd_update_fwd_v2<NB, V2SK, RowPA, 2, 1>) : go(k_gd_update_fwd_v2<NB, V2SK, RowPA, 2, 0>);
      if (sc->kind == 1) return go(k_gd_update_fwd_v2<NB, V2SK, RowPA, 1, 0>);
      return go(k_gd_update_fwd_v2<NB, V2SK, RowPA, 0, 0>);
    }
  }
#endif
  return launch_k(e, LPC_K_SPATIAL, k_rinv_gd_update_fwd_half<RNT, REM, RSK, RowPA>, dim3(g.H, e->P), RNT, kRowSmem,
                  geom_rev(e, e->plan.gd_rev_update),
                  row_arg(e), e->planW.tw, (const real2*)e->gd.S2, e->S, e->gd.gx, e->gd.gaux, alpha, *sc);
}
static int m_gd_bwd_head(Engine* e, const GdBwd* a) { return launch_gd_bwd_half<0, RNT, REM, RSK>(e, row_arg(e), *a); }
static int m_gd_bwd_mid(Engine* e, const GdBwd* a) { return launch_gd_bwd_half<1, RNT, REM, RSK>(e, row_arg(e), *a); }
static int m_gd_bwd_update(Engine* e, const GdBwd* a) { return launch_gd_bwd_half<2, RNT, REM, RSK>(e, row_arg(e), *a); }
static int m_gd_bwd_acc(Engine* e, const GdBwd* a, const real2* Sin) {
  return launch_gd_bwd_half<3, RNT, REM, RSK>(e, row_arg(e), *a, Sin);
}
#endif
#endif

#if LPC_MOD_ROW_KIND == LPC_ROWS_PAIRED
static RowPA row_arg(const Engine* e) { return splan_arg<RowP, LPC_MOD_TW_LANE != 0>(e->planW, e->tws_row); }

static int m_admm_rows_fwd(Engine* e) {
  return launch_admm_rows_fwd_paired<RNT, REM, RSK, false, LPC_MOD_SLAY>(e, row_arg(e));
}
static int m_admm_rows_inv(Engine* e, real* Vout, real* HVout, int skip_hv_outside) {
  return launch_admm_rows_inv_paired<RNT, REM, RSK, false, LPC_MOD_SLAY>(e, row_arg(e), Vout, HVout, skip_hv_outside != 0);
}
#if LPC_MOD_ROW_X
constexpr int kK1Quads = (RowP::n >> 2) <= RNT ? 1 : ((RowP::n >> 2) <= 2 * RNT ? 2 : 0);
constexpr bool kK1Rows = kK1Quads != 0;
static int m_admm_rows_fwd_x(Engine* e, const AdmmScalars* sc, const K1Rows* k1) {
  real2 *SA = e->S, *SB = spec_b(e);
  const int xrows = paired_rows_grid(e->g, sc->skipa != 0);
  if (k1) {
    if constexpr (kK1Rows)
      return launch_k(e, LPC_K_ROW_FWD, k_rfwd_arrays_x<RNT, REM, RSK, RowPA, true, LPC_MOD_SLAY>, dim3(xrows, e->P), RNT, kRowSmem,
                      e->g, *sc,
                      row_arg(e), (const real*)e->admm.Rsp, (const real*)e->admm.HVb[e->admm.hcur], (const real*)e->admm.HVb[e->admm.hcur ^ 1],
                      e->admm.xi, (const real*)e->Y, SA, SB, *k1);
    return fail("internal: this module's rows do not hold the TV / W half");
  }
  return launch_k(e, LPC_K_ROW_FWD, k_rfwd_arrays_x<RNT, REM, RSK, RowPA, false, LPC_MOD_SLAY>, dim3(xrows, e->P), RNT, kRowSmem,
                  e->g, *sc,
                  row_arg(e), (const real*)e->admm.Rsp, (const real*)e->admm.HVb[e->admm.hcur], (const real*)e->admm.HVb[e->admm.hcur ^ 1],
                  e->admm.xi, (const real*)e->Y, SA, SB, K1Rows{});
}
#endif
#endif

#if LPC_MOD_PASSA
typedef SPlan<LPC_MOD_PASSA_RAD> PassAP;
static int m_cols_passA(Engine* e, const ColPass* cp, real2* S, int nplanes, int inverse, int kid) {
  return launch_cols<LPC_MOD_PASSA_NT, LPC_MOD_PASSA_EM, LPC_MOD_PASSA_T, true>(e, splan_arg<PassAP>(e->planA), *cp, S,
                                                                                nplanes, inverse != 0, kid);
}
#endif

#if LPC_MOD_MID_KIND != 0
typedef SPlan<LPC_MOD_MID_RAD> MidP;
typedef SPlanArg<MidP> MidPA;
static int m_admm_mid(Engine* e, const ColPass* cp, const AdmmScalars* sc, real sb_outside_scale) {
  constexpr int NT = LPC_MOD_MID_NT, EM = LPC_MOD_MID_EM, T = LPC_MOD_MID_T;
  const MidPA pa = splan_arg<MidP>(e->planB);
#if LPC_MOD_MID_KIND == LPC_MID_SEQ
  constexpr int PC = LPC_MOD_SLAY != 0 ? LPC_MOD_MID_PC : 0;
  return launch_k(e, LPC_K_COL_MID, k_cols_mid_admm_seq<NT, EM, MidPA, T, LPC_MOD_MID_MINW, LPC_MOD_MID_PRE != 0, LPC_MOD_SLAY, PC>,
                  dim3(cp->ntile_c * e->P), NT, (size_t)MidP::n * (T + 1) * sizeof(real2), e->g, pa, *cp, e->S, spec_b(e),
                  PC ? (const real2*)e->admm.midc : (const real2*)(LPC_MOD_SLAY ? e->admm.Hs_t : e->Hs),
                  PC ? (const real*)e->admm.midrd : (const real*)(LPC_MOD_SLAY ? e->admm.Gabs_t : e->admm.Gabs), (const real2*)e->phr, (const real2*)e->phc, sc->mu1,
                  sc->mu2, sc->mu3, inv_points(e->g), sb_outside_scale);
#else
  return launch_admm_mid<NT, EM, 2 * T, true, LPC_MOD_SLAY>(e, pa, *cp, *sc, sb_outside_scale);
#endif
}
#endif

#if defined(LPC_STAMP)
extern "C" int lpc_module_stamps(unsigned long long* dst, size_t bytes) {
  if (bytes > sizeof(lpc_stamp_buf)) bytes = sizeof(lpc_stamp_buf);
  if (hipDeviceSynchronize() != hipSuccess) return 1;
  return hipMemcpyFromSymbol(dst, HIP_SYMBOL(lpc_stamp_buf), bytes, 0, hipMemcpyDeviceToHost) == hipSuccess ? 0 : 1;
}
#endif
extern "C" int lpc_module_init(LpcModule* m, size_t engine_size, const char* src_fp) {
  if (!m || engine_size != sizeof(Engine) || !src_fp || std::strcmp(src_fp, LPC_SRC_FP) != 0) return 1;
  std::memset((void*)m, 0, sizeof(*m));
#if LPC_MOD_ROW_KIND == LPC_ROWS_HALF
  m->rows_fwd_single = m_rows_fwd_single;
  m->rows_inv_single = m_rows_inv_single;
#endif
#if LPC_MOD_ROW_KIND != 0 && LPC_MOD_FAMILY == LPC_FAM_ADMM
  m->admm_rows_fwd = m_admm_rows_fwd;
  m->admm_rows_inv = m_admm_rows_inv;
#if LPC_MOD_ROW_KIND == LPC_ROWS_HALF && !defined(LPC_DOUBLE)
  m->admm_rows_v2 = GdV2<RowP>::ok ? 1 : 0;
#endif
#if LPC_MOD_ROW_X
  m->admm_rows_fwd_x = m_admm_rows_fwd_x;
#if LPC_MOD_ROW_KIND == LPC_ROWS_PAIRED
  m->k1_rows = kK1Quads;
#endif
#endif
#endif
#if LPC_MOD_ROW_KIND == LPC_ROWS_HALF && LPC_MOD_FAMILY == LPC_FAM_GD
#ifndef LPC_DOUBLE
  m->gd_v2 = GdV2<RowP>::ok ? 1 : 0;
#endif
  m->gd_rows_mid = m_gd_rows_mid;
  m->gd_rows_update = m_gd_rows_update;
  m->gd_rows_update_fwd = m_gd_rows_update_fwd;
  m->gd_bwd_head = m_gd_bwd_head;
  m->gd_bwd_mid = m_gd_bwd_mid;
  m->gd_bwd_update = m_gd_bwd_update;
  m->gd_bwd_acc = m_gd_bwd_acc;
#endif
#if LPC_MOD_PASSA
  m->cols_passA = m_cols_passA;
#endif
#if LPC_MOD_MID_KIND != 0
  m->admm_mid = m_admm_mid;
#endif
  m->slay = LPC_MOD_SLAY;
#if LPC_MOD_MID_KIND == LPC_MID_SEQ
  m->mid_pc = LPC_MOD_SLAY != 0 ? LPC_MOD_MID_PC : 0;
#endif
  return 0;
}
```

lenslesspicam_amd/csrc/lpc_plan.h:

```cpp
#pragma once
#include <cctype>
#include <cstdio>
#include <cstdlib>
#include <cstring>
#include <string>
#include <vector>

#define LPC_SPEC_MAX_ST 8

struct StaticFft {
  int n = 0;
  int nst = 0;
  int rad[LPC_SPEC_MAX_ST] = {0};
  int nt = 0, em = 0;
  int T = 1;
};

#define LPC_FAM_ADMM 1
#define LPC_FAM_GD 2
#define LPC_ROWS_RUNTIME 0
#define LPC_ROWS_HALF 1
#define LPC_ROWS_PAIRED 2
#define LPC_MID_RUNTIME 0
#define LPC_MID_PAIR 1
#define LPC_MID_SEQ 2

struct PlanSpec {
  int family = 0;
  int f64 = 0;
  int row_kind = LPC_ROWS_RUNTIME;
  StaticFft row;
  int row_sk = 0;
  int row_x = 0;
  StaticFft passA;
  int mid_kind = LPC_MID_RUNTIME;
  StaticFft mid;
  int mid_minw = 1;
  int mid_pre = 0;
  int mid_pc = 0;
  int slay = 0;
  bool any() const { return row_kind != LPC_ROWS_RUNTIME || passA.n || mid_kind != LPC_MID_RUNTIME; }
};

static inline std::string fft_key(const StaticFft& f) {
  std::string s = std::to_string(f.n) + "r";
  for (int i = 0; i < f.nst; ++i) s += (i ? "." : "") + std::to_string(f.rad[i]);
  s += "t" + std::to_string(f.T) + "w" + std::to_string(f.nt) + "x" + std::to_string(f.em);
  return s;
}
static inline std::string plan_spec_key(const PlanSpec& s) {
  std::string k = s.f64 ? "f64" : "f32";
  k += s.family == LPC_FAM_ADMM ? "_admm" : "_gd";
  if (s.row_kind) k += std::string(s.row_kind == LPC_ROWS_HALF ? "_rh" : "_rp") + fft_key(s.row) + (s.row_sk == 1 ? "s" : "") + (s.row_x ? "x" : "");
  if (s.passA.n) k += "_a" + fft_key(s.passA);
  if (s.mid_kind) k += std::string(s.mid_kind == LPC_MID_PAIR ? "_mp" : "_ms") + fft_key(s.mid) + "m" + std::to_string(s.mid_minw) + (s.mid_pre ? "p" : "") + (s.slay ? "L" : "") + (s.mid_pc == 1 ? "c" : (s.mid_pc == 2 ? "r" : ""));
  return k;
}
static inline std::string rad_list(const StaticFft& f, const char* sep = ",") {
  std::string s;
  for (int i = 0; i < f.nst; ++i) s += (i ? sep : "") + std::to_string(f.rad[i]);
  return s;
}
static inline std::vector<std::string> plan_spec_defines(const PlanSpec& s) {
  std::vector<std::string> d;
  auto def = [&](const std::string& k, const std::string& v) { d.push_back("-D" + k + "=" + v); };
  auto defi = [&](const std::string& k, int v) { def(k, std::to_string(v)); };
  if (s.f64) d.push_back("-DLPC_DOUBLE");
  defi("LPC_MOD_FAMILY", s.family);
  defi("LPC_MOD_ROW_KIND", s.row_kind);
  if (s.row_kind) {
    def("LPC_MOD_ROW_RAD", rad_list(s.row));
    defi("LPC_MOD_ROW_NT", s.row.nt); defi("LPC_MOD_ROW_EM", s.row.em);
    defi("LPC_MOD_ROW_SK", s.row_sk); defi("LPC_MOD_ROW_X", s.row_x);
  }
  defi("LPC_MOD_PASSA", s.passA.n ? 1 : 0);
  if (s.passA.n) {
    def("LPC_MOD_PASSA_RAD", rad_list(s.passA));
    defi("LPC_MOD_PASSA_NT", s.passA.nt); defi("LPC_MOD_PASSA_EM", s.passA.em); defi("LPC_MOD_PASSA_T", s.passA.T);
  }
  defi("LPC_MOD_MID_KIND", s.mid_kind);
  if (s.mid_kind) {
    def("LPC_MOD_MID_RAD", rad_list(s.mid));
    defi("LPC_MOD_MID_NT", s.mid.nt); defi("LPC_MOD_MID_EM", s.mid.em); defi("LPC_MOD_MID_T", s.mid.T);
    defi("LPC_MOD_MID_MINW", s.mid_minw);
    defi("LPC_MOD_MID_PRE", s.mid_pre);
  }
  defi("LPC_MOD_SLAY", s.slay);
  defi("LPC_MOD_MID_PC", s.mid_pc);
  return d;
}

struct EngineOpts {
  int no_static = 0;
  int jit = 1;
  long jit_min_points = 1L << 16;
  std::string module_dir;
  std::string compiler;
  int module_max = 256;
  int module_loaded_max = 64;
  int rows_half = -1;
  int tile_budget = 0;
  int split_n2 = 0;
  int col_t = 0;
  int passa_t = 0;
  int mid_seq = -1;
  int mid_pre = -1;
  int prow_nt128 = -1;
  int g_plane = -1;
  int mid_swz = -1;
  int spec_lay = -1;
  std::string row_rad;
  int hv_full = 0;
  int xi_full = 0;
  int k1_rows = 1;
  int k1_group = 16;
  int mid_pc = 1;
  int k1_half = 1;
  int rho_rsp = 1;
  int xi_half = 1;
  int admm_rows_v2 = 1;
  int rev_order = 9;
  int gd_rev = -1;
  int gd_no_fuse_fwd = 0;
  int gd_v2 = 1;
};

static inline std::string unescape_opt_path(const std::string& v) {
  std::string r;
  for (size_t i = 0; i < v.size(); ++i) {
    if (v[i] == '%' && i + 2 < v.size() && std::isxdigit((unsigned char)v[i + 1]) && std::isxdigit((unsigned char)v[i + 2])) {
      r += (char)std::strtol(v.substr(i + 1, 2).c_str(), nullptr, 16);
      i += 2;
    } else {
      r += v[i];
    }
  }
  return r;
}

static inline std::string parse_engine_opts(const char* str, EngineOpts& o) {
  if (!str) return "";
  std::string s(str);
  size_t i = 0;
  while (i < s.size()) {
    size_t j = s.find_first_of(",; \t\n", i);
    if (j == std::string::npos) j = s.size();
    if (j > i) {
      const std::string tok = s.substr(i, j - i);
      const size_t eq = tok.find('=');
      const std::string k = tok.substr(0, eq), v = eq == std::string::npos ? "1" : tok.substr(eq + 1);
      const long iv = std::atol(v.c_str());
      if (k == "no_static") o.no_static = (int)iv;
      else if (k == "jit") o.jit = (int)iv;
      else if (k == "jit_min_points") o.jit_min_points = iv;
      else if (k == "module_dir") o.module_dir = unescape_opt_path(v);
      else if (k == "compiler") o.compiler = unescape_opt_path(v);
      else if (k == "module_max") o.module_max = (int)iv;
      else if (k == "module_loaded_max") o.module_loaded_max = (int)iv;
      else if (k == "rows_half") o.rows_half = (int)iv;
      else if (k == "tile_budget") o.tile_budget = (int)iv;
      else if (k == "split_n2") o.split_n2 = (int)iv;
      else if (k == "col_t") o.col_t = (int)iv;
      else if (k == "passa_t") o.passa_t = (int)iv;
      else if (k == "mid_seq") o.mid_seq = (int)iv;
      else if (k == "mid_pre") o.mid_pre = (int)iv;
      else if (k == "prow_nt128") o.prow_nt128 = (int)iv;
      else if (k == "g_plane") o.g_plane = (int)iv;
      else if (k == "mid_swz") o.mid_swz = (int)iv;
      else if (k == "spec_lay") o.spec_lay = (int)iv;
      else if (k == "row_rad") o.row_rad = v;
      else if (k == "hv_full") o.hv_full = (int)iv;
      else if (k == "xi_full") o.xi_full = (int)iv;
      else if (k == "k1_rows") o.k1_rows = (int)iv;
      else if (k == "k1_group") o.k1_group = (int)iv;
      else if (k == "k1_half") o.k1_half = (int)iv;
      else if (k == "rho_rsp") o.rho_rsp = (int)iv;
      else if (k == "xi_half") o.xi_half = (int)iv;
      else if (k == "admm_rows_v2") o.admm_rows_v2 = (int)iv;
      else if (k == "mid_pc") o.mid_pc = (int)iv;
      else if (k == "rev_order") o.rev_order = (int)iv;
      else if (k == "gd_rev") o.gd_rev = (int)iv;
      else if (k == "gd_no_fuse_fwd") o.gd_no_fuse_fwd = (int)iv;
      else if (k == "gd_v2") o.gd_v2 = (int)iv;
      else return "unknown engine option '" + k + "'";
    }
    i = j + 1;
  }
  return "";
}
```

lenslesspicam_amd/csrc/lpc_planner.cpp:

```cpp
#include "lpc_engine.h"

static int next_5smooth(int n) {
  int m = n < 1 ? 1 : n;
  for (;; ++m) {
    int r = m;
    while (r % 2 == 0) r /= 2;
    while (r % 3 == 0) r /= 3;
    while (r % 5 == 0) r /= 5;
    if (r == 1) return m;
  }
}
bool plan_radices(int n, std::vector<int>& rad) {
  rad.clear();
  int r = n, a = 0, b3 = 0;
  while (r % 2 == 0) { r /= 2; ++a; }
  while (r % 3 == 0) { r /= 3; ++b3; }
  int c5 = 0;
  { int t = r; while (t % 5 == 0) { t /= 5; ++c5; } }
  int best_k6 = 0, best_cnt = 1 << 30;
  for (int k6 = 0; k6 <= std::min(a, b3); ++k6) {
    const int a2 = a - k6;
    const int cnt = k6 + a2 / 3 + (a2 % 3 ? 1 : 0) + (b3 - k6) + c5;
    if (cnt < best_cnt) { best_cnt = cnt; best_k6 = k6; }
  }
  a -= best_k6;
  for (int i = 0; i < a / 3; ++i) rad.push_back(8);
  a %= 3;
  for (int i = 0; i < best_k6; ++i) rad.push_back(6);
  b3 -= best_k6;
  if (a == 2) rad.push_back(4);
  if (a == 1) rad.push_back(2);
  while (r % 5 == 0) { r /= 5; rad.push_back(5); }
  for (int i = 0; i < b3; ++i) rad.push_back(3);
  return r == 1;
}
static bool radices_skew_ok(int n, const std::vector<int>& rad) {
  int ns = 1;
  for (int r : rad) {
    if ((n / r) % 8 != 0) return false;
    if (!(ns % 8 == 0 || (ns == 1 && r % 8 == 0))) return false;
    ns *= r;
  }
  return true;
}

static int row_layout(int n, const std::vector<int>& rad) { return radices_skew_ok(n, rad) ? 1 : 0; }

static void choose_split(const EngineOpts& opt, int Hp, int Wc, int* N1, int* N2, int* T, bool prefer24 = false,
                         bool admm_f32 = false) {
  int t = 16;
  if (opt.col_t > 0) t = opt.col_t;
  while (t > 1 && t / 2 >= Wc) t /= 2;
  int budget = kMaxTilePoints;
  if (opt.tile_budget > 0) budget = std::max(64, opt.tile_budget);
  for (int tt = t; tt >= (t >= 8 ? 8 : t); tt /= 2) {
    if ((long)Hp * 2 * tt <= budget) { *N1 = 1; *N2 = Hp; *T = tt; return; }
    if (tt == 1) break;
  }
  int best1 = 1, best2 = Hp, bestcost = 1 << 30;
  for (int d = 1; d <= Hp; ++d) {
    if (Hp % d) continue;
    const int n2 = d, n1 = Hp / d;
    if ((long)n2 * 2 * t > budget / 2 || (long)n1 * t > budget / 2) continue;
    const int cost = std::max(n1, 2 * n2);
    if (cost < bestcost || (admm_f32 && cost == bestcost && n2 > best2)) { bestcost = cost; best1 = n1; best2 = n2; }
  }
  if (prefer24 && Hp % 24 == 0 && Hp / 24 <= (admm_f32 ? 96 : 128) && Hp / 24 >= 2 && (long)(Hp / 24) * t <= budget / 2) {
    best2 = 24; best1 = Hp / 24;
  }
  if (opt.split_n2 > 0) {
    const int n2 = opt.split_n2;
    if (n2 > 0 && Hp % n2 == 0 && (long)n2 * 2 * t <= budget && (long)(Hp / n2) * t <= budget) { best2 = n2; best1 = Hp / n2; }
  }
  *N1 = best1; *N2 = best2; *T = t;
}
static void set_static_fft(StaticFft& f, int n, const std::vector<int>& rad, int T, int nt, int em) {
  f = StaticFft{};
  if ((int)rad.size() > LPC_SPEC_MAX_ST) return;
  f.n = n; f.nst = (int)rad.size();
  for (int i = 0; i < f.nst; ++i) f.rad[i] = rad[(size_t)i];
  f.T = T; f.nt = nt; f.em = em;
}
static inline int round_up64(int v) { return (v + 63) / 64 * 64; }
static void override_radices(const std::string& opt, int n, std::vector<int>& rad) {
  if (opt.empty()) return;
  std::vector<int> r;
  long prod = 1;
  size_t i = 0;
  while (i < opt.size()) {
    size_t j = opt.find('.', i);
    if (j == std::string::npos) j = opt.size();
    const int v = std::atoi(opt.substr(i, j - i).c_str());
    static const int ok[] = {2, 3, 4, 5, 6, 8, 9, 10, 12, 15, 16, 18, 20, 24, 30};
    if (std::find(std::begin(ok), std::end(ok), v) == std::end(ok)) return;
    r.push_back(v);
    prod *= v;
    i = j + 1;
  }
  if (prod == n && (int)r.size() <= LPC_SPEC_MAX_ST) rad = r;
}

int plan_cu_count() {
#if defined(LPC_SIMT_EMU)
  return 256;
#endif
  int n = 0;
  if (rt::device_count(&n) != lpcSuccess || n <= 0) return 256;
  return rt::cu_count();
}

void choose_plan(const lpc_config& c, const EngineOpts& o, const PlaneGeom& g, int P, bool allow_static, int cu, LaunchPlan* out) {
  const bool admm = c.algo == LPC_ALGO_ADMM, f32 = sizeof(real) == 4;
  LaunchPlan& pl = *out;
  pl = LaunchPlan{};
  pl.spec.family = admm ? LPC_FAM_ADMM : LPC_FAM_GD;
  pl.spec.f64 = f32 ? 0 : 1;
  choose_split(o, g.Hp, g.Wc, &pl.N1, &pl.N2, &pl.T, !admm || f32, admm && f32);
  const long col_step = (long)(pl.N1 > 1 ? pl.N2 : 1) * g.cpitch * (long)sizeof(real2);
  const bool st_cols = allow_static && col_step < (1L << 24) && g.Hp < (1 << 24) &&
                       (unsigned long long)g.Hp * g.cpitch * sizeof(real2) < (1ULL << 32);
  const bool seq = admm && f32 && st_cols && pl.N1 == 1 && pl.T == 8 && g.Wc > 8 && (long)g.Hp * 16 <= kMaxTilePoints &&
                   o.col_t == 0 && o.mid_seq != 0 && ((long)P * ((g.Wc + 15) / 16) >= 512 || o.mid_seq == 1);
  const bool half_ok = g.Wp % 2 == 0 && g.Wp >= 4;
  const bool admm_wide = (allow_static && g.Wp % 4 == 0 && o.k1_rows != 0) ? g.Wp > 4096
                                                                            : 5 * LPC_ROW_SMEM_BYTES(g.Wp, 1) > 160 * 1024;
  const bool wide = admm ? admm_wide : (g.Wp >= 2048 || (allow_static && g.Wp >= 128));
  pl.rows_half = half_ok && wide;
  if (o.rows_half == 0) pl.rows_half = false;
  if (o.rows_half == 1 && half_ok) pl.rows_half = true;
  if (!allow_static) return;

  PlanSpec& sp = pl.spec;
  std::vector<int> rad;
  const bool xhalf = admm && g.Wp % 4 == 0;
  if (pl.rows_half) {
    const int n = g.Wp / 2;
    plan_radices(n, rad);
    if (n == 4096) rad = {16, 16, 16};
    if (n == 2048 && admm) rad = {16, 16, 8};
    if (n == 1920 && admm) rad = {16, 8, 15};
    override_radices(o.row_rad, n, rad);
    int nt = std::min(1024, std::max(64, round_up64(n / rad[0])));
    if (n == 2048 && admm && rad[0] == 16) nt = 256;
    if (n == 4096 && rad[0] == 16) nt = 512;
    if (n == 1024 && !admm) nt = 256;
    set_static_fft(sp.row, n, rad, 1, nt, (n + nt - 1) / nt);
    if (sp.row.n && sp.row.em <= 16) {
      sp.row_kind = LPC_ROWS_HALF;
      sp.row_sk = row_layout(n, rad);
      sp.row_x = xhalf;
    }
  } else if (admm) {
    const int n = g.Wp;
    plan_radices(n, rad);
    if (rad.size() >= 2 && rad.back() == 2) {
      for (size_t i = rad.size() - 1; i-- > 0;)
        if (rad[i] == 8) { rad[i] = 4; rad.back() = 4; std::stable_sort(rad.begin(), rad.end(), [](int a, int b) { return (a == 8) > (b == 8); }); break; }
    }
    override_radices(o.row_rad, n, rad);
    int nt = std::min(1024, std::max(64, round_up64(n / rad[0])));
    if (nt < 256 && n >= 512) {
      const bool batch = (long)P * g.Hp >= 8192;
      const bool k1r = xhalf && o.k1_rows != 0 && n % 4 == 0 && n / 4 <= 256;
      if (o.prow_nt128 == 0 || (o.prow_nt128 < 0 && (!batch || k1r))) nt = 256;
    }
    set_static_fft(sp.row, n, rad, 1, nt, (n + nt - 1) / nt);
    if (sp.row.n && sp.row.em <= 16) {
      sp.row_kind = LPC_ROWS_PAIRED;
      sp.row_sk = row_layout(n, rad);
      sp.row_x = xhalf;
    }
  }
  if (st_cols && pl.N1 > 1) {
    int T = pl.T;
    if (pl.T == 16 && g.Wc >= 256 && o.col_t == 0) T = 32;
    if (o.passa_t > 0) T = o.passa_t;
    while (T > 1 && (long)pl.N1 * T > kMaxTilePoints) T /= 2;
    plan_radices(pl.N1, rad);
    if (pl.N1 == 90) rad = {10, 9};
    const int pts = pl.N1 * T;
    int nt = T >= 32 ? 512 : 256;
    while (nt < 1024 && (pts + nt - 1) / nt > 16) nt *= 2;
    set_static_fft(sp.passA, pl.N1, rad, T, nt, (pts + nt - 1) / nt);
    if (sp.passA.em > 16) sp.passA = StaticFft{};
  }
  const bool reg_mid = pl.N1 > 1 && f32 && pl.N2 == 24;
  if (admm && st_cols && !reg_mid) {
    const int n = pl.N2, T = pl.T;
    plan_radices(n, rad);
    if (n == 540) rad = seq ? std::vector<int>{10, 6, 9} : std::vector<int>{30, 18};
    const bool one_wave_of_tiles = !seq && pl.N1 == 1 && (long)P * ((g.Wc + T - 1) / T) <= cu && n * 2 * T > 8192;
    if (one_wave_of_tiles && n == 540) rad = {6, 10, 9};
    const int pts = n * (seq ? T : 2 * T);
    int nt = pts <= 4096 ? 256 : (pts <= 9216 ? 512 : 1024);
    if (seq) nt = pts <= 9 * 256 ? 256 : (pts <= 18 * 512 ? 512 : 1024);
    if (one_wave_of_tiles) nt = 1024;
    set_static_fft(sp.mid, n, rad, T, nt, (pts + nt - 1) / nt);
    if (sp.mid.n && sp.mid.em <= 18) {
      sp.mid_kind = seq ? LPC_MID_SEQ : LPC_MID_PAIR;
      if (seq) {
        sp.mid_pre = o.mid_pre >= 0 ? (o.mid_pre ? 1 : 0) : 1;
        const size_t lds = (size_t)n * (T + 1) * sizeof(real2);
        const int wgs = (int)std::max<size_t>(1, std::min<size_t>(8, (160 * 1024) / lds));
        sp.mid_minw = std::min(8, std::max(1, (wgs * nt + 255) / 256));
      }
    } else {
      sp.mid = StaticFft{};
    }
  }
  sp.slay = (admm && f32 && sp.row_kind == LPC_ROWS_PAIRED && sp.mid_kind != LPC_MID_RUNTIME && pl.N1 == 1 && sp.mid.T == 8 &&
             o.spec_lay != 0) ? 1 : 0;
  sp.mid_pc = (sp.slay && sp.mid_kind == LPC_MID_SEQ && o.mid_pc != 0) ? ((g.Hp % 2 == 0 && g.Wp % 2 == 0) ? 2 : 1) : 0;
}

void finish_plan(const lpc_config& c, const EngineOpts& o, const PlaneGeom& g, int P, const LpcModule* mod, bool lane_twiddles,
                 int cu, LaunchPlan* out) {
  LaunchPlan& pl = *out;
  const bool admm = c.algo == LPC_ALGO_ADMM, gd = c.algo >= LPC_ALGO_GD, split = pl.N1 > 1;
  pl.xhalf_rows = admm && mod && mod->admm_rows_fwd_x;
  const bool k1_rows = pl.xhalf_rows && g.Wp % 4 == 0 && mod->k1_rows != 0 && o.k1_rows != 0;
  pl.k1 = k1_rows ? ADMM_K1_ROWS : pl.xhalf_rows ? ADMM_K1_TV_W : g.Wp % 4 == 0 ? ADMM_K1_TILED : ADMM_K1_SCALAR;
  pl.k1_half = pl.xhalf_rows && o.k1_half != 0;
  pl.rho_rsp = pl.k1_half && pl.k1 == ADMM_K1_TV_W && o.rho_rsp != 0;
  pl.xi_half = pl.k1_half && o.xi_half != 0;
  pl.admm_rows_v2 = (admm && pl.rows_half && mod && mod->admm_rows_v2 && lane_twiddles && ((g.sw | g.W) & 1) == 0 && g.W >= 2)
                        ? (o.admm_rows_v2 & 3) : 0;
  pl.k1_xcd_order = cu != 256 ? 0 : (long)paired_rows_grid(g, false) * P <= 8192 ? -1 : std::max(0, o.k1_group);
  pl.xi_window = pl.xhalf_rows && !o.xi_full;
  pl.hv_skip = pl.xi_window && !o.hv_full && mod->admm_rows_inv && (split || mod->admm_mid);
  const long mid_pts = (long)pl.N2 * pl.T * 2;
  pl.admm_mid = split && sizeof(real) == 4 && pl.N2 == 24 ? ADMM_MID_REG24
                : mod && mod->admm_mid ? ADMM_MID_MODULE
                : mid_pts > 8192 && mid_pts <= 9216 ? ADMM_MID_RT_512X18 : ADMM_MID_RT_LDS;
  static const int kRegMid[] = {48, 40, 36, 32, 30, 24};
  pl.conv_mid_reg = split && std::find(std::begin(kRegMid), std::end(kRegMid), pl.N2) != std::end(kRegMid) ? pl.N2 : 0;
  pl.gd_fuse_fwd = gd && mod && mod->gd_rows_update_fwd && !o.gd_no_fuse_fwd;
  pl.gd_v2 = gd && mod && mod->gd_v2 && lane_twiddles && o.gd_v2 != 0 && ((g.sw | g.W) & 1) == 0 && g.W >= 2;
  pl.rev_k1 = o.rev_order & 1;
  pl.rev_passa_fwd = o.rev_order & 2;
  pl.rev_passa_inv = o.rev_order & 4;
  pl.rev_mid = o.rev_order & 8;
  const int gd_rev = o.gd_rev >= 0 ? o.gd_rev : ((size_t)g.cplane * P * sizeof(real2) > ((size_t)200 << 20)) ? 7 : 0;
  const bool mod_gd_rows = mod && mod->gd_rows_mid;
  pl.gd_rev_resid = mod_gd_rows && (gd_rev & 1);
  pl.gd_rev_update = mod_gd_rows && (gd_rev & 2);
  pl.gd_rev_mid = gd_rev & 4;
  pl.mid_swz = o.mid_swz >= 0 ? o.mid_swz : ((size_t)pl.T * sizeof(real2) < 128 && !g.slay ? 1 : 0);
  pl.g_terms = o.g_plane >= 0 ? !o.g_plane : ((size_t)g.cplane * sizeof(real) > ((size_t)8 << 20));
}

int setup_shape(const lpc_config& c, const EngineOpts& o, int cu, ShapePlan* out) {
  PlaneGeom& g = out->g;
  g.H = c.height; g.W = c.width;
  g.Hp = next_5smooth(2 * g.H - 1);
  g.Wp = next_5smooth(2 * g.W - 1);
  g.Wc = g.Wp / 2 + 1;
  g.sh = (g.Hp - g.H) / 2;
  g.sw = (g.Wp - g.W) / 2;
  g.rpitch = (g.Wp + 3) / 4 * 4;
  g.cpitch = (g.Wc + 15) / 16 * 16;
  g.rplane = (long)g.Hp * g.rpitch;
  g.cplane = (long)((g.Hp + 1) & ~1) * g.cpitch;
  g.slay = 0;
  g.uplane = (long)g.H * g.W;
  g.DC = c.depth * c.channels;
  g.C = c.channels;
  g.PM = g.DC;
  g.rev = 0;
  out->Ppsf = g.DC;
  out->P = c.batch * g.DC;
  out->Pdata = c.batch * c.channels;
  if (g.Wp > kMaxTilePoints)
    return fail("padded width " + std::to_string(g.Wp) + " > " + std::to_string(kMaxTilePoints) + " is not supported");
  out->want_static = !o.no_static && (long)g.Hp * g.Wp >= o.jit_min_points;
  choose_plan(c, o, g, out->P, out->want_static, cu, &out->plan);
  return 0;
}
```

lenslesspicam_amd/csrc/lpc_row_kernels.h:

```cpp
#pragma once
#include "lpc_args.h"

template <int NT, int SK, int SL = 0>
static __device__ __forceinline__ void untangle_store(const real2* s, int Wp, int Wc, real2* outA,
                                                       real2* outB, bool validB, int tid, bool validA = true) {
  for (int k = tid; k < Wc; k += NT) {
    real2 zk = s[lds_slot<SK>(k)];
    real2 zn = s[lds_slot<SK>(k == 0 ? 0 : Wp - k)];
    if (validA) outA[spec_col<SL>(k)] = make_real2((real)0.5 * (zk.x + zn.x), (real)0.5 * (zk.y - zn.y));
    if (validB) outB[spec_col<SL>(k)] = make_real2((real)0.5 * (zk.y + zn.y), -(real)0.5 * (zk.x - zn.x));
  }
}

template <int NT, int EMAX, int SK, int SL = 0>
static __device__ __forceinline__ void tangle_load(real2* s, int Wp, int Wc, const real2* inA,
                                                    const real2* inB, bool validB, int tid, bool validA = true) {
  constexpr int EH = EMAX / 2 + 1;
  if constexpr (SL == 1) {
    constexpr int EP = (EH + 1) / 2;
    real4 a4[EP], b4[EP];
    const real4 z4 = make_real4((real)0., (real)0., (real)0., (real)0.);
#pragma unroll
    for (int q = 0; q < EP; ++q) {
      const int k = 2 * (tid + q * NT);
      a4[q] = b4[q] = z4;
      if (k < Wc) {
        if (validA) a4[q] = ld4((const real*)(inA + spec_col<SL>(k)));
        if (validB) b4[q] = ld4((const real*)(inB + spec_col<SL>(k)));
      }
    }
#pragma unroll
    for (int q = 0; q < EP; ++q) {
#pragma unroll
      for (int u = 0; u < 2; ++u) {
        const int k = 2 * (tid + q * NT) + u;
        if (k < Wc) {
          real2 av = u ? make_real2(a4[q].z, a4[q].w) : make_real2(a4[q].x, a4[q].y);
          real2 bv = u ? make_real2(b4[q].z, b4[q].w) : make_real2(b4[q].x, b4[q].y);
          const bool selfconj = (k == 0) || (2 * k == Wp);
          if (selfconj) { av.y = (real)0.; bv.y = (real)0.; }
          s[lds_slot<SK>(k)] = make_real2(av.x - bv.y, av.y + bv.x);
          if (!selfconj) s[lds_slot<SK>(Wp - k)] = make_real2(av.x + bv.y, bv.x - av.y);
        }
      }
    }
    return;
  }
  real2 a[EH], b[EH];
#pragma unroll
  for (int q = 0; q < EH; ++q) {
    const int k = tid + q * NT;
    a[q] = make_real2((real)0., (real)0.);
    b[q] = make_real2((real)0., (real)0.);
    if (k < Wc) {
      if (validA) a[q] = inA[spec_col<SL>(k)];
      if (validB) b[q] = inB[spec_col<SL>(k)];
    }
  }
#pragma unroll
  for (int q = 0; q < EH; ++q) {
    const int k = tid + q * NT;
    if (k < Wc) {
      real2 av = a[q], bv = b[q];
      const bool selfconj = (k == 0) || (2 * k == Wp);
      if (selfconj) { av.y = (real)0.; bv.y = (real)0.; }
      s[lds_slot<SK>(k)] = make_real2(av.x - bv.y, av.y + bv.x);
      if (!selfconj) s[lds_slot<SK>(Wp - k)] = make_real2(av.x + bv.y, bv.x - av.y);
    }
  }
}

template <int NT, int SK>
static __device__ __forceinline__ void untangle_r2_store(const real2* s, int Wp, const real2* LPC_RESTRICT tw,
                                                          real2* outA, real2* outB, bool validB, int tid) {
  const int nb = Wp >> 1;
  auto emit = [&](int k, real2 zk, real2 zn) {
    outA[k] = make_real2((real)0.5 * (zk.x + zn.x), (real)0.5 * (zk.y - zn.y));
    if (validB) outB[k] = make_real2((real)0.5 * (zk.y + zn.y), (real)-0.5 * (zk.x - zn.x));
  };
  for (int j = tid; j <= nb / 2; j += NT) {
    const int jm = nb - j;
    const real2 u0 = s[lds_slot<SK>(j)];
    const real2 v0 = j ? cmul(s[lds_slot<SK>(j + nb)], tw[j]) : s[lds_slot<SK>(nb)];
    const real2 zj = cadd(u0, v0), zjn = csub(u0, v0);
    if (j == 0) {
      emit(0, zj, zj);
      emit(nb, zjn, zjn);
    } else if (j == jm) {
      emit(j, zj, zjn);
    } else {
      const real2 u1 = s[lds_slot<SK>(jm)];
      const real2 v1 = cmul(s[lds_slot<SK>(jm + nb)], tw[jm]);
      const real2 zm = cadd(u1, v1), zmn = csub(u1, v1);
      emit(j, zj, zmn);
      emit(jm, zm, zjn);
    }
  }
}

template <int NT>
static __device__ __forceinline__ void tangle_r2_load(real2* s, int Wp, const real2* inA, const real2* inB,
                                                       bool validB, int tid) {
  const int nb = Wp >> 1;
  const real2 zero = make_real2((real)0, (real)0);
  for (int j = tid; j <= nb / 2; j += NT) {
    const int jm = nb - j;
    real2 a0 = inA[j], b0 = validB ? inB[j] : zero;
    real2 a1 = inA[jm], b1 = validB ? inB[jm] : zero;
    if (j == 0) { a0.y = (real)0; b0.y = (real)0; a1.y = (real)0; b1.y = (real)0; }
    const real2 zj = make_real2(a0.x - b0.y, a0.y + b0.x);
    const real2 zm = make_real2(a1.x - b1.y, a1.y + b1.x);
    const real2 zjn = make_real2(a1.x + b1.y, b1.x - a1.y);
    const real2 zmn = make_real2(a0.x + b0.y, b0.x - a0.y);
    if (j == 0) {
      s[0] = cadd(zj, zm);
      s[1] = csub(zj, zm);
    } else {
      s[2 * j] = cadd(zj, zjn);
      s[2 * j + 1] = csub(zj, zjn);
      if (j != jm) {
        s[2 * jm] = cadd(zm, zmn);
        s[2 * jm + 1] = csub(zm, zmn);
      }
    }
  }
}

static __device__ __forceinline__ PairedRows paired_rows_of(const PlaneGeom& g, unsigned bx, bool window_b) {
  const int nB = window_b ? paired_rows_window(g) : (g.Hp + 1) >> 1;
  PairedRows r;
  int idx;
  if ((int)bx < 2 * nB) { r.arr = (int)((bx ^ (bx >> 3)) & 1u); idx = (int)(bx >> 1); }
  else { r.arr = 0; idx = (int)bx - nB; }
  r.first = true;
  if (r.arr == 1 && window_b) {
    r.r0 = (g.slay ? g.sh & ~1 : g.sh) + 2 * idx;
    r.first = r.r0 >= g.sh;
    r.second = r.r0 + 1 < g.sh + g.H;
  }
  else { r.r0 = 2 * idx; r.second = r.r0 + 1 < g.Hp; }
  return r;
}

template <int NT, int EMAX, int SK, bool R2, class PL = Fft1dPlan, int SL = 0>
__global__ __launch_bounds__(NT) void k_rfwd_arrays(PlaneGeom g, PL plan,
                                                     const real* LPC_RESTRICT A,
                                                     const real* LPC_RESTRICT B,
                                                     real2* LPC_RESTRICT SA,
                                                     real2* LPC_RESTRICT SB) {
  LPC_DYN_SMEM(smem);
  real2* s = (real2*)smem;
  const int tid = LPC_TID(NT);
  const long pl = blockIdx.y;
  const PairedRows pr = paired_rows_of(g, blockIdx.x, false);
  const real* a = (pr.arr ? B : A) + pl * g.rplane + (long)pr.r0 * g.rpitch;
  const real* b = a + g.rpitch;
  const bool v1 = pr.second;
  auto src = [&](int i, int) { return make_real2(a[i], v1 ? b[i] : (real)0.); };
  if constexpr (is_static_plan<PL>::value)
    fft_tile<NT, EMAX, false, SK, false, true>(s, plan, 1, make_fastdiv_dev1(), tid, src, LdsNatural{});
  else
    fft_tile<NT, EMAX, false, SK, false, true>(s, plan, 1, make_fastdiv_dev1(), tid, src, LdsNatural{}, NoFix{}, 0,
                                               R2 ? 1 : 0);
  real2* oa = (pr.arr ? SB : SA) + pl * g.cplane + (long)pr.r0 * g.cpitch;
  real2* ob = oa + (SL ? 8 : g.cpitch);
  static_assert(!(R2 && SL), "pair-line spectra: compile-time plans only");
  if (R2) untangle_r2_store<NT, SK>(s, g.Wp, plan.tw, oa, ob, v1, tid);
  else untangle_store<NT, SK, SL>(s, g.Wp, g.Wc, oa, ob, v1, tid);
}

template <int NT, int SK>
static __device__ __forceinline__ void untangle_half_store(const real2* s, int M, const real2* LPC_RESTRICT twW,
                                                            real2* LPC_RESTRICT o, int tid) {
  for (int k = tid; k <= M / 2; k += NT) {
    const int km = M - k;
    const real2 zk = s[lds_slot<SK>(k)];
    const real2 zm = s[lds_slot<SK>(k == 0 ? 0 : km)];
    const real ex = (real)0.5 * (zk.x + zm.x), ey = (real)0.5 * (zk.y - zm.y);
    const real2 od = make_real2((real)0.5 * (zk.y + zm.y), (real)-0.5 * (zk.x - zm.x));
    const real2 wo = cmul(twW[k], od);
    o[k] = make_real2(ex + wo.x, ey + wo.y);
    if (k != km) o[km] = make_real2(ex - wo.x, wo.y - ey);
  }
}

template <int NT, int EMAX, int SK, class PL = Fft1dPlan>
__global__ __launch_bounds__(NT) void k_rfwd_half(PlaneGeom g, PL plan, const real2* LPC_RESTRICT twW,
                                                   const real* LPC_RESTRICT A, const real* LPC_RESTRICT B,
                                                   real2* LPC_RESTRICT SA, real2* LPC_RESTRICT SB) {
  LPC_DYN_SMEM(smem);
  real2* s = (real2*)smem;
  const int tid = LPC_TID(NT), row = blockIdx.x >> 1, arr = blockIdx.x & 1;
  const long pl = blockIdx.y;
  const real2* a2 = (const real2*)((arr ? B : A) + pl * g.rplane + (long)row * g.rpitch);
  auto src = [&](int i, int) { return a2[i]; };
  fft_tile<NT, EMAX, false, SK, false, true>(s, plan, 1, make_fastdiv_dev1(), tid, src, LdsNatural{});
  untangle_half_store<NT, SK>(s, g.Wp >> 1, twW, (arr ? SB : SA) + pl * g.cplane + (long)row * g.cpitch, tid);
}

template <int NT, int EMAX, int SK>
static __device__ __forceinline__ void tangle_half_load(real2* s, int M, const real2* LPC_RESTRICT twW,
                                                         const real2* LPC_RESTRICT in, int tid) {
  constexpr int EH = EMAX / 2 + 1;
  real2 xk[EH], xm[EH];
#pragma unroll
  for (int q = 0; q < EH; ++q) {
    const int k = tid + q * NT;
    xk[q] = make_real2((real)0., (real)0.);
    xm[q] = xk[q];
    if (k <= M / 2) { xk[q] = in[k]; xm[q] = in[M - k]; }
  }
#pragma unroll
  for (int q = 0; q < EH; ++q) {
    const int k = tid + q * NT;
    if (k <= M / 2) {
      real2 a = xk[q], b = xm[q];
      if (k == 0) { a.y = (real)0.; b.y = (real)0.; }
      const real2 e = make_real2(a.x + b.x, a.y - b.y);
      const real2 d = make_real2(a.x - b.x, a.y + b.y);
      const real2 od = cmul_conj(d, twW[k]);
      s[lds_slot<SK>(k)] = make_real2(e.x - od.y, e.y + od.x);
      if (k != 0 && k != M - k) s[lds_slot<SK>(M - k)] = make_real2(e.x + od.y, od.x - e.y);
    }
  }
}

template <int NT, int EMAX, int SK, class PL = Fft1dPlan>
__global__ __launch_bounds__(NT) void k_rinv_half(PlaneGeom g, PL plan, const real2* LPC_RESTRICT twW,
                                                   const real2* LPC_RESTRICT SA, const real2* LPC_RESTRICT SB,
                                                   real* LPC_RESTRICT A, real* LPC_RESTRICT B, int skip_b_outside) {
  LPC_DYN_SMEM(smem);
  real2* s = (real2*)smem;
  const int tid = LPC_TID(NT);
  const unsigned bx = LPC_BX(g);
  int row = bx >> 1, arr = (bx ^ (bx >> 3)) & 1;
  const long pl = LPC_BY(g);
  if (skip_b_outside) {
    if ((int)bx < 2 * g.H) row += g.sh;
    else {
      const int q = (int)bx - 2 * g.H;
      row = q < g.sh ? q : q + g.H;
      arr = 0;
    }
  }
  tangle_half_load<NT, EMAX, SK>(s, g.Wp >> 1, twW, (arr ? SB : SA) + pl * g.cplane + (long)row * g.cpitch, tid);
  __syncthreads();
  real2* o2 = (real2*)((arr ? B : A) + pl * g.rplane + (long)row * g.rpitch);
  auto out = [&](int i, int, real2 v) { o2[i] = v; };
  fft_tile<NT, EMAX, true, SK, true, false, true>(s, plan, 1, make_fastdiv_dev1(), tid, LdsNatural{}, out);
}

template <int NT, int EMAX, int SK, bool R2>
__global__ __launch_bounds__(NT) void k_rfwd_rows(PlaneGeom g, Fft1dPlan plan, RealSrc src,
                                                   real2* LPC_RESTRICT S) {
  LPC_DYN_SMEM(smem);
  real2* s = (real2*)smem;
  const int tid = LPC_TID(NT);
  const int r0 = 2 * blockIdx.x, r1 = r0 + 1;
  const long pl = blockIdx.y;
  const bool v1 = r1 < src.nrows;
  const real* a = src.base + pl * src.plane_stride + (long)r0 * src.pitch;
  const real* b = src.base + pl * src.plane_stride + (long)r1 * src.pitch;
  auto in = [&](int i, int) {
    const int c = i - src.col0;
    const bool ok = (c >= 0) && (c < src.ncols);
    return make_real2(ok ? a[c] : (real)0., (ok && v1) ? b[c] : (real)0.);
  };
  fft_tile<NT, EMAX, false, SK, false, true>(s, plan, 1, make_fastdiv_dev1(), tid, in, LdsNatural{}, NoFix{}, 0,
                                             R2 ? 1 : 0);
  real2* o = S + pl * g.cplane + (long)(src.out_row0 + r0) * g.cpitch;
  if (R2) untangle_r2_store<NT, SK>(s, g.Wp, plan.tw, o, o + g.cpitch, v1, tid);
  else untangle_store<NT, SK>(s, g.Wp, g.Wc, o, o + g.cpitch, v1, tid);
}

template <int NT, int EMAX, int SK, class PL = Fft1dPlan>
__global__ __launch_bounds__(NT) void k_rfwd_rows_half(PlaneGeom g, PL plan, const real2* LPC_RESTRICT twW,
                                                        RealSrc src, real2* LPC_RESTRICT S) {
  LPC_DYN_SMEM(smem);
  real2* s = (real2*)smem;
  const int tid = LPC_TID(NT), r = blockIdx.x;
  const long pl = blockIdx.y;
  const real* a = src.base + pl * src.plane_stride + (long)r * src.pitch;
  auto in = [&](int i, int) {
    const int c = 2 * i - src.col0;
    return make_real2((c >= 0 && c < src.ncols) ? a[c] : (real)0.,
                      (c + 1 >= 0 && c + 1 < src.ncols) ? a[c + 1] : (real)0.);
  };
  fft_tile<NT, EMAX, false, SK, false, true>(s, plan, 1, make_fastdiv_dev1(), tid, in, LdsNatural{});
  untangle_half_store<NT, SK>(s, g.Wp >> 1, twW, S + pl * g.cplane + (long)(src.out_row0 + r) * g.cpitch, tid);
}

template <int NT, int EMAX, int SK, bool R2, class PL = Fft1dPlan, int SL = 0>
__global__ __launch_bounds__(NT) void k_rinv_arrays(PlaneGeom g, PL plan,
                                                     const real2* LPC_RESTRICT SA,
                                                     const real2* LPC_RESTRICT SB,
                                                     real* LPC_RESTRICT A, real* LPC_RESTRICT B, int window_only) {
  LPC_DYN_SMEM(smem);
  real2* s = (real2*)smem;
  const int tid = LPC_TID(NT);
  LPC_STAMP_BEGIN(3);
  const long pl = LPC_BY(g);
  const PairedRows pr = paired_rows_of(g, LPC_BX(g), window_only != 0);
  const bool va = pr.first, vb = pr.second;
  const real2* ia = (pr.arr ? SB : SA) + pl * g.cplane + (long)pr.r0 * g.cpitch;
  const real2* ib = ia + (SL ? 8 : g.cpitch);
  static_assert(!(R2 && SL), "pair-line spectra: compile-time plans only");
  if (R2) tangle_r2_load<NT>(s, g.Wp, ia, ib, vb, tid);
  else tangle_load<NT, EMAX, SK, SL>(s, g.Wp, g.Wc, ia, ib, vb, tid, va);
  __syncthreads();
  real* a = (pr.arr ? B : A) + pl * g.rplane + (long)pr.r0 * g.rpitch;
  real* b = a + g.rpitch;
  auto out = [&](int i, int, real2 v) { if (va) a[i] = v.x; if (vb) b[i] = v.y; };
  if constexpr (is_static_plan<PL>::value)
    fft_tile<NT, EMAX, true, SK, true, false, true>(s, plan, 1, make_fastdiv_dev1(), tid, LdsNatural{}, out);
  else
    fft_tile<NT, EMAX, true, SK, true, false, true>(s, plan, 1, make_fastdiv_dev1(), tid, LdsNatural{}, out, NoFix{},
                                                    R2 ? 1 : 0, 0);
  LPC_STAMP_END();
}

static __device__ __forceinline__ int shifted_col(int i, int hw, int col0, int Wp) {
  int c = i - hw - col0;
  if (c < 0) c += Wp;
  if (c < 0) c += Wp;
  return c;
}

template <int NT, int EMAX, int SK, bool R2>
__global__ __launch_bounds__(NT) void k_rinv_rows(PlaneGeom g, Fft1dPlan plan,
                                                   const real2* LPC_RESTRICT S, RealDst dst) {
  LPC_DYN_SMEM(smem);
  real2* s = (real2*)smem;
  const int tid = LPC_TID(NT);
  const int r0 = 2 * blockIdx.x, r1 = r0 + 1;
  const long pl = blockIdx.y;
  const bool v1 = r1 < dst.nrows;
  const int hh = g.Hp / 2, hw = g.Wp / 2;
  const int sr0 = wrap_add(dst.row0 + r0, hh, g.Hp);
  const int sr1 = wrap_add(dst.row0 + (v1 ? r1 : r0), hh, g.Hp);
  if (R2) tangle_r2_load<NT>(s, g.Wp, S + pl * g.cplane + (long)sr0 * g.cpitch,
                             S + pl * g.cplane + (long)sr1 * g.cpitch, v1, tid);
  else tangle_load<NT, EMAX, SK>(s, g.Wp, g.Wc, S + pl * g.cplane + (long)sr0 * g.cpitch,
                                 S + pl * g.cplane + (long)sr1 * g.cpitch, v1, tid);
  __syncthreads();
  real* a = dst.base + pl * dst.plane_stride + (long)r0 * dst.pitch;
  real* b = dst.base + pl * dst.plane_stride + (long)r1 * dst.pitch;
  auto out = [&](int i, int, real2 v) {
    const int c = shifted_col(i, hw, dst.col0, g.Wp);
    if (c < dst.ncols) {
      a[c] = v.x;
      if (v1) b[c] = v.y;
    }
  };
  fft_tile<NT, EMAX, true, SK, true, false, true>(s, plan, 1, make_fastdiv_dev1(), tid, LdsNatural{}, out, NoFix{},
                                                  R2 ? 1 : 0, 0);
}

template <int NT, int EMAX, int SK, class PL = Fft1dPlan>
__global__ __launch_bounds__(NT) void k_rinv_rows_half(PlaneGeom g, PL plan, const real2* LPC_RESTRICT twW,
                                                        const real2* LPC_RESTRICT S, RealDst dst) {
  LPC_DYN_SMEM(smem);
  real2* s = (real2*)smem;
  const int tid = LPC_TID(NT), r = blockIdx.x;
  const long pl = blockIdx.y;
  const int hh = g.Hp / 2, hw = g.Wp / 2;
  const int sr = wrap_add(dst.row0 + r, hh, g.Hp);
  tangle_half_load<NT, EMAX, SK>(s, g.Wp >> 1, twW, S + pl * g.cplane + (long)sr * g.cpitch, tid);
  __syncthreads();
  real* a = dst.base + pl * dst.plane_stride + (long)r * dst.pitch;
  auto out = [&](int i, int, real2 v) {
    const int c0 = shifted_col(2 * i, hw, dst.col0, g.Wp);
    if (c0 < dst.ncols) a[c0] = v.x;
    const int c1 = shifted_col(2 * i + 1, hw, dst.col0, g.Wp);
    if (c1 < dst.ncols) a[c1] = v.y;
  };
  fft_tile<NT, EMAX, true, SK, true, false, true>(s, plan, 1, make_fastdiv_dev1(), tid, LdsNatural{}, out);
}
```

lenslesspicam_amd/csrc/lpc_rows.cpp:

```cpp
#include "lpc_launch.h"

int rows_fwd_single(Engine* e, const RealSrc& src, real2* S, int nplanes, int kid) {
  const PlaneGeom& g = e->g;
  if (e->mod && e->mod->rows_fwd_single) return e->mod->rows_fwd_single(e, &src, S, nplanes, kid);
  if (e->plan.rows_half)
    return dispatch_row(g.Wp / 2, e->planWh.skew_ok, false, [&](auto NT, auto EM, auto SK, auto) {
      return launch_rows_fwd_half<NT.value, EM.value, SK.value>(e, e->planWh, src, S, nplanes, kid);
    });
  const int nblk = (src.nrows + 1) / 2;
  return dispatch_row(g.Wp, e->planW.skew_ok, e->rows_r2, [&](auto NT, auto EM, auto SK, auto R2) {
    constexpr int nt = decltype(NT)::value, em = decltype(EM)::value;
    constexpr bool sk = decltype(SK)::value, r2 = decltype(R2)::value;
    return launch_k(e, kid, k_rfwd_rows<nt, em, sk, r2>, dim3(nblk, nplanes), nt, LPC_ROW_SMEM_BYTES(g.Wp, sk), g,
                    e->planW, src, S);
  });
}

int rows_inv_single(Engine* e, const real2* S, const RealDst& dst, int nplanes, int kid) {
  const PlaneGeom& g = e->g;
  if (e->mod && e->mod->rows_inv_single) return e->mod->rows_inv_single(e, S, &dst, nplanes, kid);
  if (e->plan.rows_half)
    return dispatch_row(g.Wp / 2, e->planWh.skew_ok, false, [&](auto NT, auto EM, auto SK, auto) {
      return launch_rows_inv_half<NT.value, EM.value, SK.value>(e, e->planWh, S, dst, nplanes, kid);
    });
  const int nblk = (dst.nrows + 1) / 2;
  const Fft1dPlan& pinv = e->rows_r2 ? e->planWi : e->planW;
  return dispatch_row(g.Wp, pinv.skew_ok, e->rows_r2, [&](auto NT, auto EM, auto SK, auto R2) {
    constexpr int nt = decltype(NT)::value, em = decltype(EM)::value;
    constexpr bool sk = decltype(SK)::value, r2 = decltype(R2)::value;
    return launch_k(e, kid, k_rinv_rows<nt, em, sk, r2>, dim3(nblk, nplanes), nt, LPC_ROW_SMEM_BYTES(g.Wp, sk), g,
                    pinv, S, dst);
  });
}

int admm_rows_fwd(Engine* e) {
  const PlaneGeom& g = e->g;
  if (e->mod && e->mod->admm_rows_fwd) return e->mod->admm_rows_fwd(e);
  if (e->plan.rows_half)
    return dispatch_row(g.Wp / 2, e->planWh.skew_ok, false, [&](auto NT, auto EM, auto SK, auto) {
      return launch_admm_rows_fwd_half<NT.value, EM.value, SK.value>(e, e->planWh);
    });
  return dispatch_row(g.Wp, e->planW.skew_ok, e->rows_r2, [&](auto NT, auto EM, auto SK, auto R2) {
    return launch_admm_rows_fwd_paired<NT.value, EM.value, SK.value, R2.value, 0>(e, e->planW);
  });
}

int admm_rows_inv(Engine* e, real* Vout, real* HVout, bool skip_hv_outside) {
  if (e->mod && e->mod->admm_rows_inv) return e->mod->admm_rows_inv(e, Vout, HVout, skip_hv_outside ? 1 : 0);
  if (skip_hv_outside) return fail("internal: skipping H V rows needs the plan module's row kernels");
  const PlaneGeom& g = e->g;
  const Fft1dPlan& pinv = e->rows_r2 ? e->planWi : e->planW;
  if (e->plan.rows_half)
    return dispatch_row(g.Wp / 2, e->planWh.skew_ok, false, [&](auto NT, auto EM, auto SK, auto) {
      return launch_admm_rows_inv_half<NT.value, EM.value, SK.value>(e, e->planWh, Vout, HVout, false);
    });
  return dispatch_row(g.Wp, pinv.skew_ok, e->rows_r2, [&](auto NT, auto EM, auto SK, auto R2) {
    return launch_admm_rows_inv_paired<NT.value, EM.value, SK.value, R2.value, 0>(e, pinv, Vout, HVout, false);
  });
}
```

lenslesspicam_amd/csrc/lpc_rt.h:

```cpp
#pragma once

#include <cstddef>
#include <cstdint>
#include <cstdio>
#include <cstdlib>
#include <cstring>
#include <cmath>

#if defined(LPC_SIMT_EMU)

#include <functional>

struct dim3 {
  unsigned x, y, z;
  dim3(unsigned x_ = 1, unsigned y_ = 1, unsigned z_ = 1) : x(x_), y(y_), z(z_) {}
};
struct float2 { float x, y; };
struct float4 { float x, y, z, w; };
struct double2 { double x, y; };
static inline double2 make_double2(double x, double y) { double2 r; r.x = x; r.y = y; return r; }
static inline float2 make_float2(float x, float y) { float2 r; r.x = x; r.y = y; return r; }
static inline float4 make_float4(float x, float y, float z, float w) { float4 r; r.x = x; r.y = y; r.z = z; r.w = w; return r; }

namespace lpc_emu {
struct ThreadCtx { dim3 tid, bid, bdim, gdim; char* smem; };
ThreadCtx& ctx();
void barrier();
void launch(dim3 grid, dim3 block, size_t smem_bytes, const std::function<void()>& body);
}

#define __global__
#define __device__
#define __host__
#define __forceinline__ inline
#define __launch_bounds__(...)
#define LPC_RESTRICT
#define threadIdx (lpc_emu::ctx().tid)
#define blockIdx (lpc_emu::ctx().bid)
#define blockDim (lpc_emu::ctx().bdim)
#define gridDim (lpc_emu::ctx().gdim)
#define __syncthreads() lpc_emu::barrier()
#define LPC_DYN_SMEM(name) char* name = lpc_emu::ctx().smem
#define LPC_TID(nt) ((int)threadIdx.x)
static inline unsigned __umulhi(unsigned a, unsigned b) { return (unsigned)(((uint64_t)a * (uint64_t)b) >> 32); }
struct lpc_rsrc { char* base; unsigned bytes; };
static inline lpc_rsrc lpc_make_rsrc(const void* base, unsigned bytes) { lpc_rsrc r; r.base = (char*)base; r.bytes = bytes; return r; }
static inline int lpc_opaque(int x) { return x; }
static inline float lpc_opaque_f(float x) { return x; }
#define LPC_SCHED_FENCE() ((void)0)

typedef void* lpcStream_t;
typedef int lpcError_t;
#define lpcSuccess 0

namespace rt {
static inline const char* err_string(lpcError_t) { return "emu"; }
static inline lpcError_t dev_malloc(void** p, size_t n) { *p = std::malloc(n ? n : 1); return *p ? 0 : 1; }
static inline lpcError_t dev_free(void* p) { std::free(p); return 0; }
static inline lpcError_t dev_malloc_async(void** p, size_t n, lpcStream_t) { return dev_malloc(p, n); }
static inline lpcError_t dev_free_async(void* p, lpcStream_t) { std::free(p); return 0; }
static inline lpcError_t memset_async(void* p, int v, size_t n, lpcStream_t) { std::memset(p, v, n); return 0; }
static inline lpcError_t copy_d2d_async(void* d, const void* s, size_t n, lpcStream_t) { std::memmove(d, s, n); return 0; }
static inline lpcError_t copy_h2d_async(void* d, const void* s, size_t n, lpcStream_t) { std::memcpy(d, s, n); return 0; }
static inline lpcError_t copy_d2h_async(void* d, const void* s, size_t n, lpcStream_t) { std::memcpy(d, s, n); return 0; }
static inline lpcError_t stream_sync(lpcStream_t) { return 0; }
static inline lpcError_t last_error() { return 0; }
static inline lpcError_t device_count(int* n) { *n = 1; return 0; }
static inline lpcError_t current_device(int* d) { *d = 0; return 0; }
static inline lpcError_t set_max_dyn_smem(const void*, size_t) { return 0; }
static inline const char* backend_name() { return "simt-emu(test-only)"; }
static inline int cu_count() { return 2; }
}

#define LPC_LAUNCH(kernel, grid, block, smem, stream, ...) \
  lpc_emu::launch((grid), (block), (smem), [=]() { kernel(__VA_ARGS__); })

#else

#include <hip/hip_runtime.h>

#define LPC_RESTRICT __restrict__
#define LPC_DYN_SMEM(name)                                              \
  extern __shared__ __attribute__((aligned(16))) char lpc_dyn_smem_[];  \
  char* name = lpc_dyn_smem_
static __device__ __forceinline__ int lpc_tid_below(unsigned nt) {
  const unsigned t = threadIdx.x;
  __builtin_assume(t < nt);
  return (int)t;
}
#define LPC_TID(nt) lpc_tid_below((unsigned)(nt))

#if defined(LPC_STAMP)
#define LPC_STAMP_KERNELS 4
#define LPC_STAMP_WGS 4096
#define LPC_STAMP_SLOTS 32
static __device__ unsigned long long lpc_stamp_buf[LPC_STAMP_KERNELS * LPC_STAMP_WGS * LPC_STAMP_SLOTS];
__shared__ unsigned lpc_stamp_lds[2];
static __device__ __forceinline__ void lpc_stamp_put() {
  if (threadIdx.x == 0) {
    const unsigned wg = blockIdx.x + gridDim.x * blockIdx.y, n = lpc_stamp_lds[1];
    if (wg < LPC_STAMP_WGS && n < LPC_STAMP_SLOTS - 1)
      lpc_stamp_buf[((size_t)lpc_stamp_lds[0] * LPC_STAMP_WGS + wg) * LPC_STAMP_SLOTS + 1 + n] = __builtin_amdgcn_s_memrealtime();
    lpc_stamp_lds[1] = n + 1;
  }
}
static __device__ __forceinline__ void lpc_stamp_begin(unsigned kid) {
  if (threadIdx.x == 0) { lpc_stamp_lds[0] = kid; lpc_stamp_lds[1] = 0; }
  lpc_stamp_put();
}
static __device__ __forceinline__ void lpc_stamp_end() {
  asm volatile("s_waitcnt vmcnt(0) lgkmcnt(0)" ::: "memory");
  lpc_stamp_put();
  if (threadIdx.x == 0) {
    const unsigned wg = blockIdx.x + gridDim.x * blockIdx.y;
    if (wg < LPC_STAMP_WGS) lpc_stamp_buf[((size_t)lpc_stamp_lds[0] * LPC_STAMP_WGS + wg) * LPC_STAMP_SLOTS] = lpc_stamp_lds[1];
  }
}
static __device__ __forceinline__ void lpc_sync_stamped() { __syncthreads(); lpc_stamp_put(); }
#define __syncthreads() lpc_sync_stamped()
#define LPC_STAMP_BEGIN(kid) lpc_stamp_begin(kid)
#define LPC_STAMP_END() lpc_stamp_end()
#endif

typedef __amdgpu_buffer_rsrc_t lpc_rsrc;
static __device__ __forceinline__ lpc_rsrc lpc_make_rsrc(const void* base, unsigned bytes) {
  return __builtin_amdgcn_make_buffer_rsrc((void*)base, 0, (int)bytes, 0x00020000);
}
static __device__ __forceinline__ int lpc_opaque(int x) { asm volatile("" : "+v"(x)); return x; }
static __device__ __forceinline__ float lpc_opaque_f(float x) { asm volatile("" : "+s"(x)); return x; }
#define LPC_SCHED_FENCE() __builtin_amdgcn_sched_barrier(0)
typedef hipStream_t lpcStream_t;
typedef hipError_t lpcError_t;
#define lpcSuccess hipSuccess

namespace rt {
static inline const char* err_string(lpcError_t e) { return hipGetErrorString(e); }
static inline lpcError_t dev_malloc(void** p, size_t n) { return hipMalloc(p, n ? n : 1); }
static inline lpcError_t dev_free(void* p) { return hipFree(p); }
static inline lpcError_t dev_malloc_async(void** p, size_t n, lpcStream_t s) { return hipMallocAsync(p, n ? n : 1, s); }
static inline lpcError_t dev_free_async(void* p, lpcStream_t s) { return hipFreeAsync(p, s); }
static inline lpcError_t memset_async(void* p, int v, size_t n, lpcStream_t s) { return hipMemsetAsync(p, v, n, s); }
static inline lpcError_t copy_d2d_async(void* d, const void* s, size_t n, lpcStream_t st) { return hipMemcpyAsync(d, s, n, hipMemcpyDeviceToDevice, st); }
static inline lpcError_t copy_h2d_async(void* d, const void* s, size_t n, lpcStream_t st) { return hipMemcpyAsync(d, s, n, hipMemcpyHostToDevice, st); }
static inline lpcError_t copy_d2h_async(void* d, const void* s, size_t n, lpcStream_t st) { return hipMemcpyAsync(d, s, n, hipMemcpyDeviceToHost, st); }
static inline lpcError_t stream_sync(lpcStream_t s) { return hipStreamSynchronize(s); }
static inline lpcError_t last_error() { return hipGetLastError(); }
static inline lpcError_t device_count(int* n) { return hipGetDeviceCount(n); }
static inline lpcError_t current_device(int* d) { return hipGetDevice(d); }
static inline lpcError_t set_max_dyn_smem(const void* fn, size_t bytes) {
  return hipFuncSetAttribute(fn, hipFuncAttributeMaxDynamicSharedMemorySize, (int)bytes);
}
static inline const char* backend_name() { return "hip-gfx950"; }
static inline int cu_count() {
  int dev = 0, n = 0;
  if (hipGetDevice(&dev) != hipSuccess || hipDeviceGetAttribute(&n, hipDeviceAttributeMultiprocessorCount, dev) != hipSuccess || n <= 0) return 256;
  return n;
}
}

#define LPC_LAUNCH(kernel, grid, block, smem, stream, ...) \
  hipLaunchKernelGGL(kernel, (grid), (block), (smem), (stream), __VA_ARGS__)

#endif

#ifdef LPC_DOUBLE
typedef double real;
typedef double2 real2;
struct real4_t { double x, y, z, w; };
#define make_real2 make_double2
#define LPC_REAL_NAME "float64"
static __host__ __device__ __forceinline__ real rmax(real a, real b) { return fmax(a, b); }
static __host__ __device__ __forceinline__ real rmin(real a, real b) { return fmin(a, b); }
static __host__ __device__ __forceinline__ real rabs(real a) { return fabs(a); }
static __host__ __device__ __forceinline__ real rsqrt_of(real a) { return sqrt(a); }
#else
typedef float real;
typedef float2 real2;
typedef float4 real4_t;
#define make_real2 make_float2
#define LPC_REAL_NAME "float32"
static __host__ __device__ __forceinline__ real rmax(real a, real b) { return fmaxf(a, b); }
static __host__ __device__ __forceinline__ real rmin(real a, real b) { return fminf(a, b); }
static __host__ __device__ __forceinline__ real rabs(real a) { return fabsf(a); }
static __host__ __device__ __forceinline__ real rsqrt_of(real a) { return sqrtf(a); }
#endif

#if defined(LPC_SIMT_EMU)
static inline real2 lpc_buf_load2(lpc_rsrc r, int off) {
  return (unsigned)off + 2 * sizeof(real) <= r.bytes && (unsigned)off < r.bytes ? *(const real2*)(r.base + off) : make_real2((real)0., (real)0.);
}
static inline void lpc_buf_store2(lpc_rsrc r, int off, real2 v) {
  if ((unsigned)off + 2 * sizeof(real) <= r.bytes && (unsigned)off < r.bytes) *(real2*)(r.base + off) = v;
}
#elif !defined(LPC_DOUBLE)
static __device__ __forceinline__ real2 lpc_buf_load2(lpc_rsrc r, int off) {
  typedef unsigned lpc_u2 __attribute__((ext_vector_type(2)));
  typedef float lpc_f2 __attribute__((ext_vector_type(2)));
  const lpc_f2 f = __builtin_bit_cast(lpc_f2, (lpc_u2)__builtin_amdgcn_raw_buffer_load_b64(r, off, 0, 0));
  return make_real2(f.x, f.y);
}
static __device__ __forceinline__ void lpc_buf_store2(lpc_rsrc r, int off, real2 v) {
  typedef unsigned lpc_u2 __attribute__((ext_vector_type(2)));
  typedef float lpc_f2 __attribute__((ext_vector_type(2)));
  lpc_f2 f;
  f.x = v.x;
  f.y = v.y;
  __builtin_amdgcn_raw_buffer_store_b64(__builtin_bit_cast(lpc_u2, f), r, off, 0, 0);
}
#endif

#if defined(LPC_SIMT_EMU)
struct v2f { float x, y; };
static inline v2f mk2(float a, float b) { v2f r; r.x = a; r.y = b; return r; }
static inline v2f operator+(v2f a, v2f b) { return mk2(a.x + b.x, a.y + b.y); }
static inline v2f operator-(v2f a, v2f b) { return mk2(a.x - b.x, a.y - b.y); }
static inline v2f operator*(v2f a, v2f b) { return mk2(a.x * b.x, a.y * b.y); }
static inline v2f operator*(float a, v2f b) { return mk2(a * b.x, a * b.y); }
static inline v2f fma2(v2f a, v2f b, v2f c) { return mk2(std::fma(a.x, b.x, c.x), std::fma(a.y, b.y, c.y)); }
#else
typedef float v2f __attribute__((ext_vector_type(2)));
static __device__ __forceinline__ v2f mk2(float a, float b) { v2f r; r.x = a; r.y = b; return r; }
static __device__ __forceinline__ v2f fma2(v2f a, v2f b, v2f c) { return __builtin_elementwise_fma(a, b, c); }
#endif

#if defined(LPC_SIMT_EMU)
static inline unsigned mul24(unsigned a, unsigned b) { return a * b; }
#else
static __device__ __forceinline__ unsigned mul24(unsigned a, unsigned b) { return __umul24(a, b); }
#endif

#if defined(__HIP_DEVICE_COMPILE__) && !defined(LPC_DOUBLE) && !defined(LPC_SIMT_EMU) && !defined(LPC_NO_PK_COMPLEX)
#define LPC_PK_COMPLEX 1
static __device__ __forceinline__ v2f c2v(real2 a) { return mk2(a.x, a.y); }
static __device__ __forceinline__ real2 v2c(v2f a) { return make_real2(a.x, a.y); }
static __device__ __forceinline__ v2f swap2(v2f a) { return __builtin_shufflevector(a, a, 1, 0); }
#endif
static __host__ __device__ __forceinline__ real2 cmul(real2 a, real2 b) {
#ifdef LPC_PK_COMPLEX
  const v2f A = c2v(a);
  return v2c(fma2(swap2(A), mk2(-b.y, b.y), A * mk2(b.x, b.x)));
#else
  return make_real2(a.x * b.x - a.y * b.y, a.x * b.y + a.y * b.x);
#endif
}
static __host__ __device__ __forceinline__ real2 cmul_conj(real2 a, real2 b) {
#ifdef LPC_PK_COMPLEX
  const v2f A = c2v(a);
  return v2c(fma2(swap2(A), mk2(b.y, -b.y), A * mk2(b.x, b.x)));
#else
  return make_real2(a.x * b.x + a.y * b.y, a.y * b.x - a.x * b.y);
#endif
}
static __host__ __device__ __forceinline__ real2 cadd(real2 a, real2 b) {
#ifdef LPC_PK_COMPLEX
  return v2c(c2v(a) + c2v(b));
#else
  return make_real2(a.x + b.x, a.y + b.y);
#endif
}
static __host__ __device__ __forceinline__ real2 csub(real2 a, real2 b) {
#ifdef LPC_PK_COMPLEX
  return v2c(c2v(a) - c2v(b));
#else
  return make_real2(a.x - b.x, a.y - b.y);
#endif
}
static __host__ __device__ __forceinline__ real2 cconj(real2 a) { return make_real2(a.x, -a.y); }
static __host__ __device__ __forceinline__ real2 cscale(real2 a, real s) {
#ifdef LPC_PK_COMPLEX
  return v2c(c2v(a) * mk2(s, s));
#else
  return make_real2(a.x * s, a.y * s);
#endif
}
static __host__ __device__ __forceinline__ real2 caxpy(real2 a, real s, real2 b) {
#ifdef LPC_PK_COMPLEX
  return v2c(fma2(c2v(a), mk2(s, s), c2v(b)));
#else
  return make_real2(a.x * s + b.x, a.y * s + b.y);
#endif
}
static __host__ __device__ __forceinline__ real2 cmul_mi(real2 a) {
#ifdef LPC_PK_COMPLEX
  const v2f A = c2v(a);
  return v2c(__builtin_shufflevector(A, -A, 1, 2));
#else
  return make_real2(a.y, -a.x);
#endif
}
static __host__ __device__ __forceinline__ real2 cmul_pi(real2 a) {
#ifdef LPC_PK_COMPLEX
  const v2f A = c2v(a);
  return v2c(__builtin_shufflevector(-A, A, 1, 2));
#else
  return make_real2(-a.y, a.x);
#endif
}

struct FastDiv {
  unsigned d, m;
};
static inline FastDiv make_fastdiv(unsigned d) {
  FastDiv f; f.d = d; f.m = d > 1 ? (unsigned)((0x100000000ull / d) + 1ull) : 0u; return f;
}
static __host__ __device__ __forceinline__ FastDiv make_fastdiv_dev1() {
  FastDiv f; f.d = 1; f.m = 0; return f;
}
static __device__ __forceinline__ unsigned fd_div(unsigned n, FastDiv f) {
  return f.d == 1 ? n : __umulhi(n, f.m);
}

#ifndef LPC_STAMP_BEGIN
#define LPC_STAMP_BEGIN(kid) ((void)0)
#define LPC_STAMP_END() ((void)0)
#endif
```

Measured before the change: 334.3 iterations/s.

## Fuse H·V inverse rows with next iteration's xi update and forward rows

Adds a kernel that, for the sensor-window rows, runs the inverse row FFT of H·V, applies the next iteration's xi half-update in registers, and runs the forward row FFT back into the spectrum buffer. This replaces writing HV to memory and reading it again in the next forward-row kernel. The next forward-row launch then only transforms the rho/Rsp array, and the inverse-row launch only produces V rows. It needs the next iteration's scalars computed ahead of time and adds a kernel launch plus cross-iteration state (a_done), and the timer now spans several launches.

```diff
diff --git a/lenslesspicam_amd/csrc/lpc_abi.cpp b/lenslesspicam_amd/csrc/lpc_abi.cpp
--- a/lenslesspicam_amd/csrc/lpc_abi.cpp
+++ b/lenslesspicam_amd/csrc/lpc_abi.cpp
@@ -471,7 +471,8 @@
                                       : " (xi inside the sensor window only)";
     if (pl.rho_rsp || pl.xi_half)
       s += std::string("; inside a call: ") + (pl.rho_rsp ? "rho read back from r_sp" : "") +
-           (pl.rho_rsp && pl.xi_half ? ", " : "") + (pl.xi_half ? "xi half-applied" : "");
+           (pl.rho_rsp && pl.xi_half ? ", " : "") + (pl.xi_half ? "xi half-applied" : "") +
+           (pl.hv_fuse ? (pl.hv_fuse == 2 ? ", H V rows on chip (behind the rows of V)" : ", H V rows on chip") : "");
   }
   if (e->cfg.algo == LPC_ALGO_ADMM && e->admm.g_sep) s += "; gram as row + column terms";
   if (e->cfg.algo == LPC_ALGO_FISTA)
diff --git a/lenslesspicam_amd/csrc/lpc_admm.cpp b/lenslesspicam_amd/csrc/lpc_admm.cpp
--- a/lenslesspicam_amd/csrc/lpc_admm.cpp
+++ b/lenslesspicam_amd/csrc/lpc_admm.cpp
@@ -12,14 +12,14 @@
   }
 }
 
-static AdmmScalars admm_scalars(const Engine* e, const double cur[4]) {
+static AdmmScalars admm_scalars(const Engine* e, const double cur[4], const double* prev_par = nullptr) {
   AdmmScalars p;
   p.mu1 = (real)cur[0]; p.mu2 = (real)cur[1]; p.mu3 = (real)cur[2];
   p.thr = (real)(cur[3] / cur[1]);
   p.m_in = (real)1.0 / ((real)1.0 + p.mu1);
   p.m_out = (real)1.0 / ((real)0.0 + p.mu1);
-  p.first = e->first ? 1 : 0;
-  const double* prev = e->first ? cur : e->admm.last_par;
+  p.first = (e->first && !prev_par) ? 1 : 0;
+  const double* prev = prev_par ? prev_par : e->first ? cur : e->admm.last_par;
   p.mu1p = (real)prev[0]; p.mu2p = (real)prev[1]; p.mu3p = (real)prev[2];
   p.thrp = (real)(prev[3] / prev[1]);
   p.m_in_p = (real)1.0 / ((real)1.0 + p.mu1p);
@@ -134,11 +134,17 @@
 }
 
 static int admm_spectral_step(Engine* e, const AdmmScalars& sc, real* Vout, real* HVout, bool xhalf = false,
-                              const K1Rows* k1 = nullptr) {
-  if (xhalf) LPC_OK(e->mod->admm_rows_fwd_x(e, &sc, k1));
+                              const K1Rows* k1 = nullptr, bool a_done = false, const AdmmScalars* next = nullptr) {
+  if (xhalf) LPC_OK(e->mod->admm_rows_fwd_x(e, &sc, k1, a_done ? 1 : 0));
   else LPC_OK(admm_rows_fwd(e));
   LPC_OK(admm_cols(e, sc));
-  return admm_rows_inv(e, Vout, HVout, sc.skiphv != 0);
+  if (!next) return admm_rows_inv(e, Vout, HVout, sc.skiphv ? ADMM_HV_ROWS_WINDOW : ADMM_HV_ROWS_ALL);
+  size_t slot = 0;
+  LPC_OK(timer_span_begin(e, LPC_K_ROW_INV, &slot));
+  if (e->plan.hv_fuse == 2) LPC_OK(admm_rows_inv(e, Vout, HVout, ADMM_HV_ROWS_NONE));
+  LPC_OK(e->mod->admm_rows_hv(e, next));
+  if (e->plan.hv_fuse != 2) LPC_OK(admm_rows_inv(e, Vout, HVout, ADMM_HV_ROWS_NONE));
+  return timer_span_end(e, LPC_K_ROW_INV, slot);
 }
 int admm_spectral_plain(Engine* e, const double par[4], real* Vout, real* HVout) {
   return admm_spectral_step(e, admm_scalars(e, par), Vout, HVout);
@@ -164,6 +170,7 @@
   const PlaneGeom& g = e->g;
   const LaunchPlan& pl = e->plan;
   bool sb_rows_valid = false;
+  bool a_done = false;
   for (int it = 0; it < n_iter; ++it) {
     real* Vc = e->admm.V[e->admm.vcur];
     real* Vo = e->admm.V[e->admm.vcur ^ 1];
@@ -192,7 +199,16 @@
     e->admm.vw_cur = false;
     e->admm.ecur ^= 1;
     e->first = false;
-    LPC_OK(admm_spectral_step(e, sc, Vo, e->admm.HVb[e->admm.hcur ^ 1], pl.xhalf_rows, pl.k1 == ADMM_K1_ROWS ? &k1 : nullptr));
+    const bool fuse = pl.hv_fuse && sc.skiphv && pl.xi_half && sc.xiw;
+    AdmmScalars scn{};
+    if (fuse) {
+      double parn[4];
+      admm_params(e, e->iters_done + 1, parn);
+      scn = admm_scalars(e, parn, par);
+    }
+    LPC_OK(admm_spectral_step(e, sc, Vo, e->admm.HVb[e->admm.hcur ^ 1], pl.xhalf_rows, pl.k1 == ADMM_K1_ROWS ? &k1 : nullptr,
+                              a_done, fuse ? &scn : nullptr));
+    a_done = fuse;
     e->admm.vcur ^= 1;
     e->admm.hcur ^= 1;
     sb_rows_valid = true;
@@ -348,19 +364,20 @@
   const double R0 = eb * g.H * g.W * e->Pdata;
   const double Sc = 2 * eb * g.Hp * g.Wc * e->Ppsf;
   const bool split = pl.N1 > 1, k1_rows = pl.k1 == ADMM_K1_ROWS;
-  const double fr = (double)g.H / (double)g.Hp;
+  const double Rh = eb * g.H * g.Wp * e->P, Sh = 2 * eb * g.H * g.Wc * e->P;
   const double nxw = pl.xi_half ? 2.0 : 3.0;
   double b = 0.0;
   switch (kid) {
     case LPC_K_SPATIAL: b = k1_rows ? 0.0 : pl.xhalf_rows ? (pl.rho_rsp ? 7.0 : pl.k1_half ? 8.0 : 9.0) * R : 15.0 * R + R0; break;
-    case LPC_K_ROW_FWD: b = (pl.hv_skip ? (1.0 + fr) * R + nxw * eb * g.H * g.W * e->P + R0 + (1.0 + fr) * S
+    case LPC_K_ROW_FWD: b = (pl.hv_fuse ? R + S : pl.hv_skip ? R + Rh + nxw * eb * g.H * g.W * e->P + R0 + S + Sh
                                 : pl.xi_window ? 2.0 * R + nxw * eb * g.H * g.W * e->P + R0 + 2.0 * S
                                 : pl.xhalf_rows ? (2.0 + nxw) * R + R0 + 2.0 * S : 2.0 * R + 2.0 * S)
                                + (k1_rows ? (pl.k1_half ? 6.0 : 7.0) * R : 0.0); break;
     case LPC_K_COL_A_FWD: b = split ? 4.0 * S : 0.0; break;
     case LPC_K_COL_MID: b = 4.0 * S + Sc + (e->admm.g_sep ? 0. : eb * g.Hp * g.Wc); break;
     case LPC_K_COL_A_INV: b = split ? 4.0 * S : 0.0; break;
-    case LPC_K_ROW_INV: b = pl.hv_skip ? (1.0 + fr) * (S + R) : 2.0 * S + 2.0 * R; break;
+    case LPC_K_ROW_INV: b = pl.hv_fuse ? S + R + 2.0 * Sh + 2.0 * eb * g.H * g.W * e->P + R0
+                               : pl.hv_skip ? S + Sh + R + Rh : 2.0 * S + 2.0 * R; break;
     default: return fail("bad kernel id");
   }
   *bytes = b;
diff --git a/lenslesspicam_amd/csrc/lpc_admm_v2_kernels.h b/lenslesspicam_amd/csrc/lpc_admm_v2_kernels.h
--- a/lenslesspicam_amd/csrc/lpc_admm_v2_kernels.h
+++ b/lenslesspicam_amd/csrc/lpc_admm_v2_kernels.h
@@ -17,7 +17,10 @@
   const unsigned bx = LPC_BX(g);
   int row = bx >> 1, arr = (bx ^ (bx >> 3)) & 1;
   const long pl = LPC_BY(g);
-  if (skip_b_outside) {
+  if (skip_b_outside == 2) {
+    row = (int)bx;
+    arr = 0;
+  } else if (skip_b_outside) {
     if ((int)bx < 2 * g.H) row += g.sh;
     else {
       const int q = (int)bx - 2 * g.H;
@@ -37,7 +40,7 @@
   for (int m = 0; m < R; ++m) o2[j + NB * m] = v[m];
 }
 
-template <int NT, int SK, class PL>
+template <int NT, int SK, class PL, bool RSP_ONLY = false>
 __global__ __launch_bounds__(NT, 4) void k_rfwd_half_x_v2(PlaneGeom g, AdmmScalars pin, PL plan, const real2* LPC_RESTRICT twW,
                                                           const real* LPC_RESTRICT Rsp, const real* LPC_RESTRICT HV,
                                                           real* LPC_RESTRICT xi, const real* LPC_RESTRICT Y,
@@ -50,7 +53,7 @@
   real2* s = (real2*)smem;
   const int j = LPC_TID(NT);
   const unsigned bx = LPC_BX(g);
-  const int gr = (int)(bx >> 1), arr = (int)(bx & 1);
+  const int gr = RSP_ONLY ? (int)bx : (int)(bx >> 1), arr = RSP_ONLY ? 0 : (int)(bx & 1);
   const unsigned pl = LPC_BY(g);
   const long o_row = (long)pl * g.rplane + (long)gr * g.rpitch;
   const bool row_in = (gr >= g.sh) && (gr < g.sh + g.H);
@@ -104,4 +107,68 @@
   v2_untangle_store<P, SK, false>(s, twW, j, v, (arr ? SB : SA) + (long)pl * g.cplane + (long)gr * g.cpitch);
 }
 
+template <int NT, int SK, class PL>
+__global__ __launch_bounds__(NT, 4) void k_hv_rows_v2(PlaneGeom g, AdmmScalars pin, PL plan, const real2* LPC_RESTRICT twW,
+                                                      real2* SB, real* LPC_RESTRICT xi, const real* LPC_RESTRICT Y,
+                                                      FastDiv fdc, FastDiv fc) {
+  using P = typename PL::plan;
+  constexpr int R = GdV2<P>::R, NB = GdV2<P>::NB, L = GdV2<P>::L, H = R / 2;
+  static_assert(GdV2<P>::ok && NT == NB, "k_hv_rows_v2: one butterfly per lane and stage");
+  LPC_DYN_SMEM(smem);
+  real2* s = (real2*)smem;
+  const int j = LPC_TID(NT), u = (int)LPC_BX(g);
+  const unsigned pl = LPC_BY(g);
+  const int gr = g.sh + u;
+  real2* row = SB + (long)pl * g.cplane + (long)gr * g.cpitch;
+  real2 wb[4];
+  v2_tw_load<P, 1>(plan.tws, j, wb);
+  v2_load_tangle_first<P, SK, false>(s, row, twW, j);
+  v2_barrier();
+  v2_mid_chain<P, SK, true>(s, plan.tws, j, wb, std::make_integer_sequence<int, L - 2>{});
+  AdmmScalars p = pin;
+  p.first = 0; p.xi_in = 1; p.xi_out = 1;
+  const long o_row = (long)pl * g.rplane + (long)gr * g.rpitch;
+  const int x0 = p.xiw ? g.sw & ~3 : 0, x1 = p.xiw ? (g.sw + g.W + 3) & ~3 : g.Wp;
+  const lpc_rsrc xr = lpc_make_rsrc(xi + o_row + x0, (unsigned)(x1 - x0) * (unsigned)sizeof(real));
+  const lpc_rsrc yr = lpc_make_rsrc(Y + (long)v2_data_plane(pl, fdc, fc, g.C) * g.uplane + (long)u * g.W,
+                                    (unsigned)g.W * (unsigned)sizeof(real));
+  const real ho = lpc_opaque_f((real)0.);
+  auto xoff = [&](int m) { return lpc_opaque((2 * (j + NB * m) - x0) * (int)sizeof(real)); };
+  auto yoff = [&](int m) { return lpc_opaque((2 * (j + NB * m) - g.sw) * (int)sizeof(real)); };
+  auto loads = [&](int m0, real2* xx, real2* yy) {
+#pragma unroll
+    for (int m = 0; m < H; ++m) xx[m] = lpc_buf_load2(xr, xoff(m0 + m));
+#pragma unroll
+    for (int m = 0; m < H; ++m) yy[m] = lpc_buf_load2(yr, yoff(m0 + m));
+  };
+  real2 v[R], r[R];
+  auto apply = [&](int m0, const real2* xx, const real2* yy) {
+#pragma unroll
+    for (int m = 0; m < H; ++m) {
+      const bool in = (unsigned)(2 * (j + NB * (m0 + m)) - g.sw) < (unsigned)g.W;
+      const real2 hv = lpc_opaque_v2(v[m0 + m]);
+      real2 xn;
+      xhalf_apply2(p, hv, xx[m], yy[m], in, ho, xn, r[m0 + m]);
+      lpc_buf_store2(xr, xoff(m0 + m), xn);
+    }
+  };
+  real2 xa[H], ya[H], xb[H], yb[H];
+  loads(0, xa, ya);
+  v2_final_stage<P, SK, true, false>(s, plan.tws, j, wb, v);
+  LPC_SCHED_FENCE();
+  apply(0, xa, ya);
+  LPC_SCHED_FENCE();
+  loads(H, xb, yb);
+  LPC_SCHED_FENCE();
+  apply(H, xb, yb);
+  LPC_SCHED_FENCE();
+  v2_tw_load<P, 1>(plan.tws, j, wb);
+  v2_barrier();
+  v2_first_fwd<P, SK>(s, j, r);
+  v2_mid_chain<P, SK, false>(s, plan.tws, j, wb, std::make_integer_sequence<int, L - 2>{});
+  v2_final_stage<P, SK, false, false>(s, plan.tws, j, wb, v);
+  v2_barrier();
+  v2_untangle_store<P, SK, false>(s, twW, j, v, row);
+}
+
 #endif
diff --git a/lenslesspicam_amd/csrc/lpc_engine.h b/lenslesspicam_amd/csrc/lpc_engine.h
--- a/lenslesspicam_amd/csrc/lpc_engine.h
+++ b/lenslesspicam_amd/csrc/lpc_engine.h
@@ -59,9 +59,11 @@
 #endif
   bool on = false;
   unsigned mask = ~0u;
+  int span = -1;
 };
 
 enum AdmmK1 { ADMM_K1_ROWS, ADMM_K1_TV_W, ADMM_K1_TILED, ADMM_K1_SCALAR };
+enum AdmmHvRows { ADMM_HV_ROWS_ALL = 0, ADMM_HV_ROWS_WINDOW = 1, ADMM_HV_ROWS_NONE = 2 };
 enum AdmmMid { ADMM_MID_REG24, ADMM_MID_MODULE, ADMM_MID_RT_512X18, ADMM_MID_RT_LDS };
 
 struct LaunchPlan {
@@ -77,6 +79,7 @@
   bool rho_rsp = false;
   bool xi_half = false;
   int admm_rows_v2 = 0;
+  int hv_fuse = 0;
   int k1_xcd_order = 0;
   AdmmMid admm_mid = ADMM_MID_RT_LDS;
   int conv_mid_reg = 0;
@@ -239,23 +242,49 @@
 
 int big_smem_once(const void* fn, size_t smem);
 
+#if !defined(LPC_SIMT_EMU)
+static inline bool timer_wants(const LaunchCtx* e, int kid) { return e->timer.on && kid >= 0 && ((e->timer.mask >> kid) & 1u); }
+static inline int timer_open(LaunchCtx* e, int kid, size_t* slot) {
+  auto& v = e->timer.ev[kid];
+  *slot = e->timer.used[kid]++;
+  if (*slot >= v.size()) {
+    hipEvent_t a, b;
+    LPC_RT(hipEventCreate(&a));
+    LPC_RT(hipEventCreate(&b));
+    v.push_back({a, b});
+  }
+  LPC_RT(hipEventRecord(v[*slot].first, e->stream));
+  return 0;
+}
+#endif
+static inline int timer_span_begin(LaunchCtx* e, int kid, size_t* slot) {
+#if !defined(LPC_SIMT_EMU)
+  if (!timer_wants(e, kid)) return 0;
+  LPC_OK(timer_open(e, kid, slot));
+  e->timer.span = kid;
+#else
+  (void)e; (void)kid; (void)slot;
+#endif
+  return 0;
+}
+static inline int timer_span_end(LaunchCtx* e, int kid, size_t slot) {
+#if !defined(LPC_SIMT_EMU)
+  if (e->timer.span != kid) return 0;
+  e->timer.span = -1;
+  LPC_RT(hipEventRecord(e->timer.ev[kid][slot].second, e->stream));
+#else
+  (void)e; (void)kid; (void)slot;
+#endif
+  return 0;
+}
+
 template <class K, class... A>
 static inline int launch_k(LaunchCtx* e, int kid, K kernel, dim3 grid, int nt, size_t smem, A... args) {
   if (smem > 48 * 1024) LPC_OK(big_smem_once((const void*)kernel, smem));
 #if !defined(LPC_SIMT_EMU)
-  const bool timed = e->timer.on && kid >= 0 && ((e->timer.mask >> kid) & 1u);
+  const bool timed = timer_wants(e, kid) && kid != e->timer.span;
   size_t slot = 0;
-  if (timed) {
-    auto& v = e->timer.ev[kid];
-    slot = e->timer.used[kid]++;
-    if (slot >= v.size()) {
-      hipEvent_t a, b;
-      LPC_RT(hipEventCreate(&a));
-      LPC_RT(hipEventCreate(&b));
-      v.push_back({a, b});
-    }
-    LPC_RT(hipEventRecord(v[slot].first, e->stream));
-  }
+  if (timed) LPC_OK(timer_open(e, kid, &slot));
   hipLaunchKernelGGL(kernel, grid, dim3(nt), smem, e->stream, args...);
   if (timed) LPC_RT(hipEventRecord(e->timer.ev[kid][slot].second, e->stream));
 #else
@@ -308,8 +337,9 @@
   int (*rows_fwd_single)(Engine*, const RealSrc*, real2* S, int nplanes, int kid);
   int (*rows_inv_single)(Engine*, const real2* S, const RealDst*, int nplanes, int kid);
   int (*admm_rows_fwd)(Engine*);
-  int (*admm_rows_fwd_x)(Engine*, const AdmmScalars*, const K1Rows* k1);
-  int (*admm_rows_inv)(Engine*, real* Vout, real* HVout, int skip_hv_outside);
+  int (*admm_rows_fwd_x)(Engine*, const AdmmScalars*, const K1Rows* k1, int a_done);
+  int (*admm_rows_inv)(Engine*, real* Vout, real* HVout, int hv_rows);
+  int (*admm_rows_hv)(Engine*, const AdmmScalars* next);
   int (*gd_rows_mid)(Engine*, const real2* Sin, real2* Sout);
   int (*gd_rows_update)(Engine*, const GdScalars*, const real* alpha);
   int (*gd_rows_update_fwd)(Engine*, const GdScalars*, const real* alpha);
@@ -391,7 +421,7 @@
 int rows_fwd_single(Engine* e, const RealSrc& src, real2* S, int nplanes, int kid);
 int rows_inv_single(Engine* e, const real2* S, const RealDst& dst, int nplanes, int kid);
 int admm_rows_fwd(Engine* e);
-int admm_rows_inv(Engine* e, real* Vout, real* HVout, bool skip_hv_outside = false);
+int admm_rows_inv(Engine* e, real* Vout, real* HVout, int hv_rows = ADMM_HV_ROWS_ALL);
 int cols_passA(Engine* e, real2* S, int nplanes, bool inverse, int zr0, int zr1, int kid, bool crop_rows_only = false,
                real sb_outside_scale = (real)0.);
 int cols_passB_fwd(Engine* e, real2* S, int nplanes, int zr0, int zr1);
diff --git a/lenslesspicam_amd/csrc/lpc_launch.h b/lenslesspicam_amd/csrc/lpc_launch.h
--- a/lenslesspicam_amd/csrc/lpc_launch.h
+++ b/lenslesspicam_amd/csrc/lpc_launch.h
@@ -5,6 +5,9 @@
 
 static inline real2* spec_b(const Engine* e) { return e->S + (size_t)e->P * e->g.cplane; }
 static inline real inv_points(const PlaneGeom& g) { return (real)1.0 / ((real)g.Hp * (real)g.Wp); }
+static inline unsigned admm_rows_inv_grid(const PlaneGeom& g, int hv_rows) {
+  return (unsigned)(hv_rows == ADMM_HV_ROWS_NONE ? g.Hp : hv_rows == ADMM_HV_ROWS_WINDOW ? g.Hp + g.H : 2 * g.Hp);
+}
 static inline PlaneGeom geom_rev(const Engine* e, bool rev) {
   PlaneGeom g = e->g;
   g.rev = rev ? 1 : 0;
@@ -28,11 +31,11 @@
                   e->S, spec_b(e));
 }
 template <int NT, int EM, int SK, class PA>
-static inline int launch_admm_rows_inv_half(Engine* e, const PA& pa, real* Vout, real* HVout, bool skip_hv) {
+static inline int launch_admm_rows_inv_half(Engine* e, const PA& pa, real* Vout, real* HVout, int hv_rows) {
   const PlaneGeom& g = e->g;
-  return launch_k(e, LPC_K_ROW_INV, k_rinv_half<NT, EM, SK, PA>, dim3(skip_hv ? g.Hp + g.H : 2 * g.Hp, e->P), NT,
+  return launch_k(e, LPC_K_ROW_INV, k_rinv_half<NT, EM, SK, PA>, dim3(admm_rows_inv_grid(g, hv_rows), e->P), NT,
                   LPC_ROW_SMEM_BYTES(g.Wp / 2, SK), g, pa, e->planW.tw, (const real2*)e->S, (const real2*)spec_b(e),
-                  Vout, HVout, skip_hv ? 1 : 0);
+                  Vout, HVout, hv_rows);
 }
 
 template <int NT, int EM, int SK, bool R2, int SL, class PA>
diff --git a/lenslesspicam_amd/csrc/lpc_module.cpp b/lenslesspicam_amd/csrc/lpc_module.cpp
--- a/lenslesspicam_amd/csrc/lpc_module.cpp
+++ b/lenslesspicam_amd/csrc/lpc_module.cpp
@@ -45,25 +45,42 @@
 static constexpr int V2SK = LPC_MOD_V2_SK;
 static const size_t kV2Smem = LPC_ROW_SMEM_BYTES(RowP::n, V2SK);
 static int m_admm_rows_fwd(Engine* e) { return launch_admm_rows_fwd_half<RNT, REM, RSK>(e, row_arg(e)); }
-static int m_admm_rows_inv(Engine* e, real* Vout, real* HVout, int skip_hv_outside) {
+static int m_admm_rows_inv(Engine* e, real* Vout, real* HVout, int hv_rows) {
 #ifndef LPC_DOUBLE
   if constexpr (GdV2<RowP>::ok) {
     if (e->plan.admm_rows_v2 & 2) {
       const PlaneGeom& g = e->g;
       constexpr int NB = GdV2<RowP>::NB;
-      return launch_k(e, LPC_K_ROW_INV, k_rinv_half_v2<NB, V2SK, RowPA>, dim3(skip_hv_outside ? g.Hp + g.H : 2 * g.Hp, e->P), NB,
+      return launch_k(e, LPC_K_ROW_INV, k_rinv_half_v2<NB, V2SK, RowPA>, dim3(admm_rows_inv_grid(g, hv_rows), e->P), NB,
                       kV2Smem, g, row_arg(e), (const real2*)e->planW.tw, (const real2*)e->S, (const real2*)spec_b(e), Vout,
-                      HVout, skip_hv_outside ? 1 : 0);
-    }
-  }
-#endif
-  return launch_admm_rows_inv_half<RNT, REM, RSK>(e, row_arg(e), Vout, HVout, skip_hv_outside != 0);
-}
-#if LPC_MOD_ROW_X
-static int m_admm_rows_fwd_x(Engine* e, const AdmmScalars* sc, const K1Rows* k1) {
+                      HVout, hv_rows);
+    }
+  }
+#endif
+  return launch_admm_rows_inv_half<RNT, REM, RSK>(e, row_arg(e), Vout, HVout, hv_rows);
+}
+#if LPC_MOD_ROW_X && !defined(LPC_DOUBLE)
+static int m_admm_rows_hv(Engine* e, const AdmmScalars* next) {
+  if constexpr (GdV2<RowP>::ok) {
+    constexpr int NB = GdV2<RowP>::NB;
+    return launch_k(e, LPC_K_ROW_INV, k_hv_rows_v2<NB, V2SK, RowPA>, dim3(e->g.H, e->P), NB, kV2Smem, e->g, *next, row_arg(e),
+                    (const real2*)e->planW.tw, spec_b(e), e->admm.xi, (const real*)e->Y, make_fastdiv((unsigned)e->g.DC),
+                    make_fastdiv((unsigned)e->g.C));
+  }
+  return fail("internal: this module's rows have no second form");
+}
+#endif
+#if LPC_MOD_ROW_X
+static int m_admm_rows_fwd_x(Engine* e, const AdmmScalars* sc, const K1Rows* k1, int a_done) {
   if (k1) return fail("internal: half-length rows do not hold the TV / W half");
 #ifndef LPC_DOUBLE
   if constexpr (GdV2<RowP>::ok) {
+    if (a_done) {
+      constexpr int NB = GdV2<RowP>::NB;
+      return launch_k(e, LPC_K_ROW_FWD, k_rfwd_half_x_v2<NB, V2SK, RowPA, true>, dim3(e->g.Hp, e->P), NB, kV2Smem, e->g, *sc,
+                      row_arg(e), (const real2*)e->planW.tw, (const real*)e->admm.Rsp, (const real*)nullptr, (real*)nullptr,
+                      (const real*)nullptr, e->S, spec_b(e), make_fastdiv((unsigned)e->g.DC), make_fastdiv((unsigned)e->g.C));
+    }
     if ((e->plan.admm_rows_v2 & 1) && !sc->first && sc->xi_in && sc->xi_out && !(sc->xiw && sc->xi_store)) {
       constexpr int NB = GdV2<RowP>::NB;
       return launch_k(e, LPC_K_ROW_FWD, k_rfwd_half_x_v2<NB, V2SK, RowPA>, dim3(2 * e->g.Hp, e->P), NB, kV2Smem, e->g, *sc,
@@ -142,7 +159,8 @@
 #if LPC_MOD_ROW_X
 constexpr int kK1Quads = (RowP::n >> 2) <= RNT ? 1 : ((RowP::n >> 2) <= 2 * RNT ? 2 : 0);
 constexpr bool kK1Rows = kK1Quads != 0;
-static int m_admm_rows_fwd_x(Engine* e, const AdmmScalars* sc, const K1Rows* k1) {
+static int m_admm_rows_fwd_x(Engine* e, const AdmmScalars* sc, const K1Rows* k1, int a_done) {
+  if (a_done) return fail("internal: paired rows always transform `a`");
   real2 *SA = e->S, *SB = spec_b(e);
   const int xrows = paired_rows_grid(e->g, sc->skipa != 0);
   if (k1) {
@@ -207,6 +225,9 @@
   m->admm_rows_inv = m_admm_rows_inv;
 #if LPC_MOD_ROW_KIND == LPC_ROWS_HALF && !defined(LPC_DOUBLE)
   m->admm_rows_v2 = GdV2<RowP>::ok ? 1 : 0;
+#if LPC_MOD_ROW_X
+  if (GdV2<RowP>::ok && GdV2<RowP>::R == 16) m->admm_rows_hv = m_admm_rows_hv;
+#endif
 #endif
 #if LPC_MOD_ROW_X
   m->admm_rows_fwd_x = m_admm_rows_fwd_x;
diff --git a/lenslesspicam_amd/csrc/lpc_plan.h b/lenslesspicam_amd/csrc/lpc_plan.h
--- a/lenslesspicam_amd/csrc/lpc_plan.h
+++ b/lenslesspicam_amd/csrc/lpc_plan.h
@@ -119,6 +119,7 @@
   int rho_rsp = 1;
   int xi_half = 1;
   int admm_rows_v2 = 1;
+  int hv_fuse = 1;
   int rev_order = 9;
   int gd_rev = -1;
   int gd_no_fuse_fwd = 0;
@@ -177,6 +178,7 @@
       else if (k == "rho_rsp") o.rho_rsp = (int)iv;
       else if (k == "xi_half") o.xi_half = (int)iv;
       else if (k == "admm_rows_v2") o.admm_rows_v2 = (int)iv;
+      else if (k == "hv_fuse") o.hv_fuse = (int)iv;
       else if (k == "mid_pc") o.mid_pc = (int)iv;
       else if (k == "rev_order") o.rev_order = (int)iv;
       else if (k == "gd_rev") o.gd_rev = (int)iv;
diff --git a/lenslesspicam_amd/csrc/lpc_planner.cpp b/lenslesspicam_amd/csrc/lpc_planner.cpp
--- a/lenslesspicam_amd/csrc/lpc_planner.cpp
+++ b/lenslesspicam_amd/csrc/lpc_planner.cpp
@@ -228,6 +228,8 @@
   pl.k1_xcd_order = cu != 256 ? 0 : (long)paired_rows_grid(g, false) * P <= 8192 ? -1 : std::max(0, o.k1_group);
   pl.xi_window = pl.xhalf_rows && !o.xi_full;
   pl.hv_skip = pl.xi_window && !o.hv_full && mod->admm_rows_inv && (split || mod->admm_mid);
+  pl.hv_fuse = ((pl.admm_rows_v2 & 1) && pl.hv_skip && pl.xi_half && mod->admm_rows_hv && pl.k1 == ADMM_K1_TV_W) ? (o.hv_fuse & 3) : 0;
+  if (pl.hv_fuse == 3) pl.hv_fuse = 1;
   const long mid_pts = (long)pl.N2 * pl.T * 2;
   pl.admm_mid = split && sizeof(real) == 4 && pl.N2 == 24 ? ADMM_MID_REG24
                 : mod && mod->admm_mid ? ADMM_MID_MODULE
diff --git a/lenslesspicam_amd/csrc/lpc_row_kernels.h b/lenslesspicam_amd/csrc/lpc_row_kernels.h
--- a/lenslesspicam_amd/csrc/lpc_row_kernels.h
+++ b/lenslesspicam_amd/csrc/lpc_row_kernels.h
@@ -235,7 +235,10 @@
   const unsigned bx = LPC_BX(g);
   int row = bx >> 1, arr = (bx ^ (bx >> 3)) & 1;
   const long pl = LPC_BY(g);
-  if (skip_b_outside) {
+  if (skip_b_outside == 2) {
+    row = (int)bx;
+    arr = 0;
+  } else if (skip_b_outside) {
     if ((int)bx < 2 * g.H) row += g.sh;
     else {
       const int q = (int)bx - 2 * g.H;
diff --git a/lenslesspicam_amd/csrc/lpc_rows.cpp b/lenslesspicam_amd/csrc/lpc_rows.cpp
--- a/lenslesspicam_amd/csrc/lpc_rows.cpp
+++ b/lenslesspicam_amd/csrc/lpc_rows.cpp
@@ -45,14 +45,14 @@
   });
 }
 
-int admm_rows_inv(Engine* e, real* Vout, real* HVout, bool skip_hv_outside) {
-  if (e->mod && e->mod->admm_rows_inv) return e->mod->admm_rows_inv(e, Vout, HVout, skip_hv_outside ? 1 : 0);
-  if (skip_hv_outside) return fail("internal: skipping H V rows needs the plan module's row kernels");
+int admm_rows_inv(Engine* e, real* Vout, real* HVout, int hv_rows) {
+  if (e->mod && e->mod->admm_rows_inv) return e->mod->admm_rows_inv(e, Vout, HVout, hv_rows);
+  if (hv_rows != ADMM_HV_ROWS_ALL) return fail("internal: skipping H V rows needs the plan module's row kernels");
   const PlaneGeom& g = e->g;
   const Fft1dPlan& pinv = e->rows_r2 ? e->planWi : e->planW;
   if (e->plan.rows_half)
     return dispatch_row(g.Wp / 2, e->planWh.skew_ok, false, [&](auto NT, auto EM, auto SK, auto) {
-      return launch_admm_rows_inv_half<NT.value, EM.value, SK.value>(e, e->planWh, Vout, HVout, false);
+      return launch_admm_rows_inv_half<NT.value, EM.value, SK.value>(e, e->planWh, Vout, HVout, ADMM_HV_ROWS_ALL);
     });
   return dispatch_row(g.Wp, pinv.skew_ok, e->rows_r2, [&](auto NT, auto EM, auto SK, auto R2) {
     return launch_admm_rows_inv_paired<NT.value, EM.value, SK.value, R2.value, 0>(e, pinv, Vout, HVout, false);
diff --git a/lenslesspicam_amd/csrc/lpc_rt.h b/lenslesspicam_amd/csrc/lpc_rt.h
--- a/lenslesspicam_amd/csrc/lpc_rt.h
+++ b/lenslesspicam_amd/csrc/lpc_rt.h
@@ -47,6 +47,7 @@
 static inline lpc_rsrc lpc_make_rsrc(const void* base, unsigned bytes) { lpc_rsrc r; r.base = (char*)base; r.bytes = bytes; return r; }
 static inline int lpc_opaque(int x) { return x; }
 static inline float lpc_opaque_f(float x) { return x; }
+template <class T2> static inline T2 lpc_opaque_v2(T2 x) { return x; }
 #define LPC_SCHED_FENCE() ((void)0)
 
 typedef void* lpcStream_t;
@@ -128,6 +129,12 @@
 }
 static __device__ __forceinline__ int lpc_opaque(int x) { asm volatile("" : "+v"(x)); return x; }
 static __device__ __forceinline__ float lpc_opaque_f(float x) { asm volatile("" : "+s"(x)); return x; }
+static __device__ __forceinline__ float2 lpc_opaque_v2(float2 x) {
+  typedef float lpc_f2v __attribute__((ext_vector_type(2)));
+  lpc_f2v t = {x.x, x.y};
+  asm("" : "+v"(t));
+  return make_float2(t.x, t.y);
+}
 #define LPC_SCHED_FENCE() __builtin_amdgcn_sched_barrier(0)
 typedef hipStream_t lpcStream_t;
 typedef hipError_t lpcError_t;
```

New measurement: 344.3 iterations/s (median of 6 runs). 3.0% higher.
